# silverlight6/Ultrasound_Modeling

Measured on AMD Instinct MI355X. Metric: segmentation training images/sec at 256x256, higher is better.
Workload: dtype bf16

## Files before the change

### include/usseg.h

```cpp
#ifndef USSEG_H
#define USSEG_H

#include <stddef.h>
#include <stdint.h>

#ifdef __cplusplus
extern "C" {
#endif

typedef void* usseg_stream_t;

typedef enum UssegStatus {
  USSEG_OK = 0,
  USSEG_ERR_BAD_ARG = -1,
  USSEG_ERR_UNSUPPORTED = -2,
  USSEG_ERR_LAUNCH = -3
} UssegStatus;

typedef enum UssegAct { USSEG_ACT_NONE = 0, USSEG_ACT_LRELU = 1, USSEG_ACT_RELU = 2, USSEG_ACT_ELU = 3, USSEG_ACT_GELU = 4 } UssegAct;

enum {
  USSEG_OUT_F32 = 1,
  USSEG_ACCUMULATE = 2
};

typedef struct UssegConvDesc {
  int32_t B, H, W;
  int32_t Cin, Cout;
  int32_t ldx, ldy;
  int32_t ksize;
  int32_t dilation;
  int32_t act;
  float alpha;
  int32_t flags;
} UssegConvDesc;

const char* usseg_last_error(void);
int usseg_version(void);

int usseg_conv2d_fwd(const UssegConvDesc* d, const void* x, const void* wp_fwd, const float* bias,
                     const void* residual, int32_t ldr, void* y, usseg_stream_t stream);
int usseg_conv2d_fwd_affine(const UssegConvDesc* d, const void* x, const void* wp_fwd, const float* scale, const float* shift,
                            const void* residual, int32_t ldr, void* y, usseg_stream_t stream);
typedef struct UssegBnFoldJob {
  const float *gamma, *beta, *mean, *var;
  const float* bias;
  float *scale, *shift;
  int32_t C, Cp;
  float eps;
  int32_t reserved;
} UssegBnFoldJob;
int usseg_bn_fold_batched(const UssegBnFoldJob* jobs_dev, int32_t njobs, usseg_stream_t stream);
int usseg_conv2d_dgrad(const UssegConvDesc* d, const void* dy, const void* wp_dgrad, const void* residual,
                       int32_t ldr, void* dx, usseg_stream_t stream);
int usseg_conv2d_wgrad(const UssegConvDesc* d, const void* x, const void* dy, float* dw_scratch, float* ws,
                       int64_t ws_floats, usseg_stream_t stream);

int usseg_conv2d_dgrad_branches(const UssegConvDesc* d, int32_t nbranches, const int32_t* ksize, const int32_t* dilation,
                                const int32_t* ch_off, int32_t Cb, const void* dy, const void* wp_cat, const void* residual,
                                int32_t ldr, void* dx, usseg_stream_t stream);

typedef struct UssegWgradBlock {
  float* dst;
  int64_t sT, sI, sO;
  int32_t i_off, o_off, ni, no;
} UssegWgradBlock;
typedef struct UssegWgradDst {
  int32_t nblocks;
  int32_t reserved;
  UssegWgradBlock blk[4];
} UssegWgradDst;
int usseg_conv2d_wgrad_mapped(const UssegConvDesc* d, const void* x, const void* dy, const UssegWgradDst* dst, float* ws,
                              int64_t ws_floats, usseg_stream_t stream);
int usseg_tconv2d_wgrad_mapped(const UssegConvDesc* d, const void* x, const void* dy, const UssegWgradDst* dst, float* ws,
                               int64_t ws_floats, usseg_stream_t stream);

typedef struct UssegWgradJob {
  UssegConvDesc desc;
  const void* x;
  const void* dy;
  float* dw;
  const UssegWgradDst* dst;
} UssegWgradJob;
int usseg_conv2d_wgrad_multi(int32_t njobs, const UssegWgradJob* jobs, float* ws, int64_t ws_floats, usseg_stream_t stream);

int usseg_defer_begin(usseg_stream_t stream, float* reduce_ws, int64_t reduce_floats, float* wgrad_ws, int64_t wgrad_floats);
int usseg_defer_flush(usseg_stream_t stream);
int usseg_defer_end(usseg_stream_t stream);

typedef struct UssegConvJob {
  UssegConvDesc desc;
  const void* x;
  const void* wp;
  const float* bias;
  const void* residual;
  int32_t ldr;
  int32_t reserved;
  void* y;
  const float* scale;
} UssegConvJob;
int usseg_conv2d_fwd_multi(int32_t njobs, const UssegConvJob* jobs, usseg_stream_t stream);
int usseg_conv2d_dgrad_multi(int32_t njobs, const UssegConvJob* jobs, usseg_stream_t stream);

int usseg_tconv2d_fwd(const UssegConvDesc* d, const void* x, const void* wp_fwd, const float* bias, void* y,
                      usseg_stream_t stream);
int usseg_tconv2d_dgrad(const UssegConvDesc* d, const void* dy, const void* wp_dgrad, const void* residual,
                        int32_t ldr, void* dx, usseg_stream_t stream);
int usseg_tconv2d_wgrad(const UssegConvDesc* d, const void* x, const void* dy, float* dw_scratch,
                        usseg_stream_t stream);

int usseg_pack_weight(const float* src, int64_t sT, int64_t sN, int64_t sK, int32_t T, int32_t Nn, int32_t Kk,
                      void* dst, int32_t Kw, int32_t tap_stride, int32_t n_off, int32_t k_off,
                      usseg_stream_t stream);
typedef struct UssegPackJob {
  const float* src;
  void* dst;
  int64_t sT, sN, sK;
  int32_t T, Nn, Kk, Kw, tap_stride, n_off, k_off, reserved;
  const float* nscale;
} UssegPackJob;
int usseg_pack_weights_batched(const UssegPackJob* jobs_dev, int32_t njobs, usseg_stream_t stream);
int usseg_pack_weights_flat(const UssegPackJob* jobs_dev, const int32_t* tilemap_dev, int32_t nblocks, usseg_stream_t stream);
int usseg_unpack_wgrad(const float* scratch, int32_t Mrows, int32_t Ncols, int32_t T, int32_t Nn, int32_t Kk,
                       int32_t n_off, int32_t k_off, float* dst, int64_t sT, int64_t sN, int64_t sK,
                       float scale, int32_t accumulate, usseg_stream_t stream);
typedef struct UssegUnpackJob {
  const float* scratch;
  float* dst;
  int64_t sT, sN, sK;
  int32_t Mrows, Ncols, T, Nn, Kk, n_off, k_off, accumulate;
  float scale;
  int32_t reserved;
} UssegUnpackJob;
int usseg_unpack_wgrad_batched(const UssegUnpackJob* jobs_dev, int32_t njobs, int32_t max_elems, usseg_stream_t stream);

typedef struct UssegNormDesc {
  int64_t M;
  int32_t C, Cphys;
  int32_t ldx, ldy;
  int32_t G;
  int32_t mode;
  float eps;
  int32_t act;
  float alpha;
  int32_t lddx;
} UssegNormDesc;
int usseg_norm_act_fwd(const UssegNormDesc* d, const void* x, const float* gamma, const float* beta,
                       const float* mean, const float* var, const void* mask, int32_t ldm, void* y, usseg_stream_t stream);
int usseg_dropout_mask(void* mask, int64_t M, int32_t C, int32_t ld, uint64_t seed, float rate, usseg_stream_t stream);
int usseg_dropout_mask_step(void* mask, int64_t M, int32_t C, int32_t ld, uint64_t seed, const int32_t* step_dev, float rate,
                            usseg_stream_t stream);
int usseg_counter_add(int32_t* counter, int32_t inc, usseg_stream_t stream);
int usseg_norm_act_bwd(const UssegNormDesc* d, const void* x, const void* dy, const float* gamma, const float* beta,
                       const float* mean, const float* var, const void* mask, int32_t ldm, void* dx, float* dgamma,
                       float* dbeta, float* dbias, float* ws, usseg_stream_t stream);
int usseg_norm_act_bwd_res(const UssegNormDesc* d, const void* x, const void* dy, const float* gamma, const float* beta,
                           const void* dres, int32_t lddres, void* dx, float* dgamma, float* dbeta, float* dbias, float* ws,
                           usseg_stream_t stream);
int usseg_norm_act_fwd_gap(const UssegNormDesc* d, const void* x, const float* gamma, const float* beta, const float* mean,
                           const float* var, void* y, int32_t B, int32_t nb, float* gap_rows, usseg_stream_t stream);
int usseg_norm_act_bwd_sa(const UssegNormDesc* d, const void* x, const void* dout, const float* gamma, const float* beta,
                          const float* mean, const float* var, int32_t B, const float* sa_s, const float* sa_dg, float sa_mult,
                          void* dx, float* dgamma, float* dbeta, float* dbias, float* ws, usseg_stream_t stream);
int usseg_norm_act_bwd_pair(const UssegNormDesc* da, const void* xa, const void* dya, const float* gamma_a, const float* beta_a, void* dxa,
                            float* dgamma_a, float* dbeta_a, float* dbias_a, const UssegNormDesc* db, const void* xb, const void* doutb,
                            const float* gamma_b, const float* beta_b, int32_t B, const float* sa_s, const float* sa_dg, float sa_mult, void* dxb,
                            float* dgamma_b, float* dbeta_b, float* dbias_b, float* ws, usseg_stream_t stream);
int usseg_stem_fwd(int32_t B, int32_t H, int32_t W, const void* x, int32_t ldx, const void* w1, const float* b1, const void* w2, const float* b2,
                   const void* w3, const float* b3, const float* gamma, const float* beta, const float* mean, const float* var, float eps,
                   float alpha, void* y1, void* t1, void* c2, void* pooled, usseg_stream_t stream);
int usseg_stem_fwd_infer(int32_t B, int32_t H, int32_t W, const void* x, int32_t ldx, const void* w1, const float* b1, const void* w2,
                         const float* b2, const void* w3, const float* b3, const float* gamma, const float* beta, const float* mean,
                         const float* var, float eps, float alpha, void* pooled, usseg_stream_t stream);
int usseg_conv3_dgrad_actbwd(int32_t B, int32_t H, int32_t W, const void* dy, int32_t lddy, const void* wd, int32_t Co, const void* yact, int32_t ldy,
                             int32_t mode, const float* gamma, const float* beta, const float* var, float eps, float alpha, void* dx,
                             int32_t lddx, float* dgamma, float* dbeta, float* dbias, float* ws, usseg_stream_t stream);
typedef struct UssegCardinalDesc {
  int32_t B, H, W;
  int32_t Cin;
  int32_t P, cv11, cvkk;
  int32_t Up, Vp, Oc;
  int32_t ldx, ldu, ldv, ldsc;
  float eps, alpha;
} UssegCardinalDesc;
int32_t usseg_cardinal_supported(const UssegCardinalDesc* d);
int usseg_cardinal_fwd(const UssegCardinalDesc* d, const void* x, const void* w1, const float* b1, const float* g1, const float* be1,
                       const void* w2, const float* b2, const float* g2, const float* be2, const void* wsc, const float* bsc,
                       const float* gsc, const float* besc, void* u_raw, void* u, void* v_raw, void* y, float* gap_rows, void* sc_raw,
                       void* sc, usseg_stream_t stream);
int usseg_cardinal_fwd_infer(const UssegCardinalDesc* d, const void* x, const void* w1, const float* b1, const float* g1, const float* be1,
                             const void* w2, const float* b2, const float* g2, const float* be2, const void* wsc, const float* bsc,
                             const float* gsc, const float* besc, void* y, float* gap_rows, void* sc, usseg_stream_t stream);
int usseg_cardinal_bwd(const UssegCardinalDesc* d, const void* dout, int32_t ldo, const void* dsc, int32_t lddsc, const void* v_raw,
                       const void* u_raw, const void* sc_raw, const void* w2d, const float* g2, const float* be2, const float* g1,
                       const float* be1, const float* gsc, const float* besc, const float* sa_s, const float* sa_dg, float sa_mult, void* dv,
                       void* dcat, int32_t ldc, float* dg2, float* dbe2, float* db2, float* dg1, float* dbe1, float* db1, float* dgsc,
                       float* dbesc, float* dbsc, float* ws, usseg_stream_t stream);
int usseg_bn_act_pool_fwd(const void* x, int32_t B, int32_t H, int32_t W, int32_t C, int32_t Cphys, int32_t ldx, const float* gamma,
                          const float* beta, const float* mean, const float* var, float eps, int32_t act, float alpha, void* y,
                          int32_t ldy, usseg_stream_t stream);
int usseg_bn_act_pool_bwd(const void* x, const void* dy, int32_t B, int32_t H, int32_t W, int32_t C, int32_t Cphys, int32_t ldx,
                          int32_t lddy, const float* gamma, const float* beta, const float* mean, const float* var, float eps,
                          int32_t act, float alpha, void* dx, int32_t lddx, float* dgamma, float* dbeta, float* dbias, float* ws,
                          usseg_stream_t stream);
int64_t usseg_reduce_ws_floats(void);
int usseg_channel_stats(const void* x, int64_t M, int32_t C, int32_t ldx, float* sum, float* sumsq, float* ws,
                        usseg_stream_t stream);

int usseg_bn_finalize_stats(const float* sum, const float* sumsq, int64_t M, int32_t C, float momentum, float* mean, float* var,
                            float* moving_mean, float* moving_var, usseg_stream_t stream);
int usseg_bn_batch_stats(const void* x, int64_t M, int32_t C, int32_t ldx, float momentum, float* mean, float* var, float* moving_mean,
                         float* moving_var, float* ws, usseg_stream_t stream);
int usseg_bn_train_bwd_fix(const void* x, void* dx, int64_t M, int32_t C, int32_t Cphys, int32_t ldx, int32_t lddx, const float* gamma,
                           const float* mean, const float* var, float eps, const float* tg, const float* tb, usseg_stream_t stream);

int usseg_act_fwd(const void* x, int64_t M, int32_t C, int32_t ldx, int32_t ldy, int32_t act, float alpha, void* y,
                  usseg_stream_t stream);
int usseg_act_bwd(const void* x, const void* dy, int64_t M, int32_t C, int32_t ldx, int32_t lddy, int32_t lddx,
                  int32_t act, float alpha, void* dx, usseg_stream_t stream);
int usseg_act_bwd_colsum(const void* x, const void* dy, int64_t M, int32_t C, int32_t ldx, int32_t lddy, int32_t lddx, int32_t act,
                         float alpha, void* dx, float* db, float* ws, usseg_stream_t stream);

int usseg_avgpool2_fwd(const void* x, int32_t B, int32_t H, int32_t W, int32_t C, int32_t ldx, int32_t ldy, void* y,
                       usseg_stream_t stream);
int usseg_avgpool2_bwd(const void* dy, int32_t B, int32_t H, int32_t W, int32_t C, int32_t lddy, int32_t lddx,
                       const void* add, int32_t ldadd, void* dx, usseg_stream_t stream);
int usseg_avgpool2_bwd_colsum(const void* dy, int32_t B, int32_t H, int32_t W, int32_t C, int32_t lddy, int32_t lddx, const void* add,
                              int32_t ldadd, void* dx, float* db, float* ws, usseg_stream_t stream);

int usseg_copy_channels(const void* src, int64_t M, int32_t C, int32_t lds, void* dst, int32_t ldd, int32_t accumulate,
                        usseg_stream_t stream);
int usseg_cast_input(const void* src, int32_t src_is_f64, int64_t M, int32_t C, void* dst, int32_t Cphys,
                     usseg_stream_t stream);
int usseg_cast_bf16_to_f32(const void* src, int64_t M, int32_t C, int32_t lds, float* dst, usseg_stream_t stream);

typedef struct UssegSplitAttnDesc {
  int32_t B, HW;
  int32_t P, R, Cg, Hd;
  int32_t ldy, ldo;
  int32_t Cy_phys, Co_phys;
  float mult;
  int32_t norm_mode;
  float eps;
  int32_t act;
  float alpha;
  int32_t use_sigmoid;
} UssegSplitAttnDesc;
typedef struct UssegSplitAttnParams {
  const float *w1, *b1, *gamma, *beta, *mean, *var, *w2, *b2;
} UssegSplitAttnParams;
typedef struct UssegSplitAttnGrads {
  float *w1, *b1, *gamma, *beta, *w2, *b2;
} UssegSplitAttnGrads;
int usseg_splitattn_gap(const UssegSplitAttnDesc* d, const void* y, float* g, float* ws, usseg_stream_t stream);
int64_t usseg_splitattn_ws_floats(const UssegSplitAttnDesc* d);
int usseg_splitattn_mlp_fwd(const UssegSplitAttnDesc* d, const float* g, int32_t g_rows, int32_t g_stride,
                            const UssegSplitAttnParams* p, float* s, float* ws, usseg_stream_t stream);
int usseg_splitattn_apply_fwd(const UssegSplitAttnDesc* d, const void* y, const float* s, void* out,
                              usseg_stream_t stream);
int usseg_splitattn_apply_bwd_reduce(const UssegSplitAttnDesc* d, const void* y, const void* dout, int32_t lddo,
                                     float* ds, float* ws, usseg_stream_t stream);
int64_t usseg_splitattn_mlp_bwd_ws_floats(const UssegSplitAttnDesc* d);
int usseg_splitattn_mlp_bwd(const UssegSplitAttnDesc* d, const float* g, int32_t g_rows, int32_t g_stride,
                            const UssegSplitAttnParams* p, const float* s, const float* ws, const float* ds, float* dg,
                            const UssegSplitAttnGrads* grads, float* grad_ws, usseg_stream_t stream);
int usseg_splitattn_bwd_fused(const UssegSplitAttnDesc* d, const void* y, const void* dout, int32_t lddo, const float* g, int32_t g_rows,
                              int32_t g_stride, const UssegSplitAttnParams* p, const float* s, const float* ws, float* dg,
                              const UssegSplitAttnGrads* grads, float* reduce_ws, float* grad_ws, usseg_stream_t stream);
int usseg_splitattn_apply_bwd_dy(const UssegSplitAttnDesc* d, const void* dout, int32_t lddo, const float* s,
                                 const float* dg, void* dy, int32_t lddy, usseg_stream_t stream);

typedef struct UssegLossDesc {
  int64_t M;
  int32_t HW;
  int32_t C, ldl, lddl;
  int32_t loss_kind;
  float label_smoothing;
  float clip_eps;
  float inv_global_batch;
  int32_t quad_w;
} UssegLossDesc;
#define USSEG_ACC_FLOATS 2050
int usseg_softmax_loss_fwd_bwd(const UssegLossDesc* d, const float* logits, const float* y_true, const float* scale,
                               float* probs, float* loss, void* dlogits, usseg_stream_t stream);
int usseg_head_quad_softmax_loss(const void* x, int32_t B, int32_t h, int32_t w, int32_t Cin_phys, int32_t ldx, const void* wq, const float* bias, int32_t C,
                                 const float* y_true, float* probs, float* loss, void* dlogits, float label_smoothing, float clip_eps,
                                 float inv_global_batch, usseg_stream_t stream);
int usseg_accuracy(const float* probs, const float* y_true, int64_t M, int32_t C, float* acc, usseg_stream_t stream);
typedef struct UssegSegCountDesc {
  int32_t B, H, W, C;
  int32_t num_classes;
  int32_t round;
} UssegSegCountDesc;
#define USSEG_SEG_COUNTS 23
int usseg_seg_counts(const UssegSegCountDesc* d, const float* y_true, const float* y_pred, uint64_t* counts, usseg_stream_t stream);
int usseg_cascade_gate(const float* probs, int32_t C_mask, int64_t M, const void* x, int32_t ldx, void* x_gated, uint8_t* mask,
                       usseg_stream_t stream);
int usseg_cascade_maps(const float* probs, int32_t C, int64_t M, float* prob_map, float* bleed_prob, usseg_stream_t stream);
int usseg_loss_from_probs(const UssegLossDesc* d, const float* probs, const float* y_true, const float* scale, float* loss,
                          usseg_stream_t stream);
typedef struct UssegClassLoss {
  float w[8];
  float gamma;
  float factor;
} UssegClassLoss;
int usseg_softmax_loss_fwd_bwd_cl(const UssegLossDesc* d, const UssegClassLoss* cl, const float* logits, const float* y_true, float* probs,
                                  float* loss, void* dlogits, usseg_stream_t stream);
int usseg_head_quad_softmax_loss_cl(const void* x, int32_t B, int32_t h, int32_t w, int32_t Cin_phys, int32_t ldx, const void* wq, const float* bias,
                                    int32_t C, const float* y_true, float* probs, float* loss, void* dlogits, float label_smoothing, float clip_eps,
                                    float inv_global_batch, const UssegClassLoss* cl, usseg_stream_t stream);
int usseg_loss_from_probs_cl(const UssegLossDesc* d, const UssegClassLoss* cl, const float* probs, const float* y_true, float* loss,
                             int32_t as_map, usseg_stream_t stream);
typedef struct UssegOverlapLoss {
  float w[8];
  float alpha;
  float beta;
  float smooth;
  float power;
  float ov_weight;
  float ce_weight;
} UssegOverlapLoss;
#define USSEG_OVERLAP_ACC_FLOATS 8224
int usseg_overlap_loss_grid(int64_t M);
int usseg_overlap_loss_sums(const UssegLossDesc* d, const UssegOverlapLoss* ol, float ov_scale, const float* probs, const float* y_true,
                            float* acc, int64_t acc_floats, usseg_stream_t stream);
int usseg_overlap_loss_bwd(const UssegLossDesc* d, const UssegOverlapLoss* ol, const float* probs, const float* y_true, const float* acc,
                           int64_t acc_floats, void* dlogits, usseg_stream_t stream);
int64_t usseg_sdf_ws_bytes(int32_t B, int32_t H, int32_t W, int32_t C);
int usseg_sdf_labels(const float* y_true, int32_t B, int32_t H, int32_t W, int32_t C, float thr, float* phi, void* ws, int64_t ws_bytes,
                     usseg_stream_t stream);
int64_t usseg_surface_ws_bytes(int32_t N, int32_t H, int32_t W);
int usseg_surface_dist(const uint8_t* a, const uint8_t* b, int32_t N, int32_t H, int32_t W, int64_t* counters, double* sums, void* ws,
                       int64_t ws_bytes, usseg_stream_t stream);
int64_t usseg_surface_stats_ws_bytes(int32_t N, int32_t H, int32_t W);
int usseg_surface_stats(const uint8_t* a, const uint8_t* b, int32_t N, int32_t H, int32_t W, const double* quant, int32_t P, const int32_t* tol2,
                        int32_t T, int64_t* counters, double* sums, int32_t* sel, int64_t* within, void* ws, int64_t ws_bytes,
                        usseg_stream_t stream);
int64_t usseg_components_ws_bytes(int32_t N, int32_t H, int32_t W);
int usseg_label_components(const uint8_t* mask, int32_t N, int32_t H, int32_t W, int32_t connectivity, int32_t* labels, int32_t* count, void* ws,
                           int64_t ws_bytes, usseg_stream_t stream);
int usseg_component_stats(const int32_t* labels, const float* prob, int32_t N, int32_t H, int32_t W, int32_t cap, int64_t* stats,
                          usseg_stream_t stream);
int usseg_clean_mask(const uint8_t* mask, const float* prob, int32_t N, int32_t H, int32_t W, int32_t connectivity, int32_t min_area,
                     float min_peak, uint8_t* out, void* ws, int64_t ws_bytes, usseg_stream_t stream);
int usseg_component_overlap(const int32_t* labels_a, const int32_t* labels_b, int32_t N, int32_t H, int32_t W, int32_t cap_a, int32_t cap_b,
                            int32_t* hit_a, int32_t* hit_b, usseg_stream_t stream);
typedef struct UssegBoundaryLoss {
  float u[8];
} UssegBoundaryLoss;
int usseg_overlap_boundary_loss_sums(const UssegLossDesc* d, const UssegOverlapLoss* ol, float ov_scale, const float* probs, const float* y_true,
                                     const float* phi, const UssegBoundaryLoss* bl, const float* wb, float* acc, int64_t acc_floats,
                                     usseg_stream_t stream);
int usseg_overlap_boundary_loss_bwd(const UssegLossDesc* d, const UssegOverlapLoss* ol, const float* probs, const float* y_true, const float* phi,
                                    const UssegBoundaryLoss* bl, const float* acc, int64_t acc_floats, void* dlogits, usseg_stream_t stream);
#define USSEG_SORT_TILE 2048
#define USSEG_SORT_DIGIT_BITS 8
int64_t usseg_sort_ws_bytes(int32_t S, int64_t n);
int usseg_sort_pairs_u32(const uint32_t* keys_in, const uint32_t* vals_in, int32_t S, int64_t n, int32_t key_bits, uint32_t* keys_out,
                         uint32_t* vals_out, void* ws, int64_t ws_bytes, usseg_stream_t stream);
typedef struct UssegLovaszLoss {
  float w[8];
  float lv_weight;
  float ce_weight;
  float threshold;
  int32_t all_classes;
} UssegLovaszLoss;
int64_t usseg_lovasz_ws_bytes(int64_t M, int32_t C);
int usseg_lovasz_coeffs(const UssegLossDesc* d, UssegLovaszLoss ll, const float* probs, const float* y_true, float* g, int32_t* counts, void* ws,
                        int64_t ws_bytes, usseg_stream_t stream);
int usseg_lovasz_loss_sums(const UssegLossDesc* d, UssegLovaszLoss ll, float ov_scale, const float* probs, const float* y_true, const float* g,
                           const int32_t* counts, float* acc, int64_t acc_floats, usseg_stream_t stream);
int usseg_lovasz_loss_bwd(const UssegLossDesc* d, UssegLovaszLoss ll, const float* probs, const float* y_true, const float* g, const float* acc,
                          int64_t acc_floats, void* dlogits, usseg_stream_t stream);
int usseg_quad_bias_expand(const float* bias, int32_t C, int32_t Np, float* out , usseg_stream_t stream);
int usseg_quad_bias_fold(const float* d16 , int32_t C, float* dbias, usseg_stream_t stream);
int usseg_tconv_quad_unpack(const float* dq, int32_t Cin_phys, int32_t Cin, int32_t Cout, int32_t Np, int32_t ksize, float* grad,
                            usseg_stream_t stream);
int usseg_quad_head_fold(const float* dq, int32_t Cin_phys, int32_t Cin, int32_t Cout, int32_t Np, int32_t ksize, float* grad, const float* d16,
                         float* dbias, usseg_stream_t stream);
int usseg_space_to_depth2(const void* full, int32_t B, int32_t H, int32_t W, int32_t C, int32_t ld_full, void* quad, int32_t Np,
                          int32_t ld_quad, int32_t to_quad, usseg_stream_t stream);
int usseg_tconv_quad_fwd(const UssegConvDesc* d, int32_t ksize, int32_t Np, const void* x, const void* wq_f, const float* bias_q, void* y4,
                         usseg_stream_t stream);
int usseg_tconv_quad_dgrad(const UssegConvDesc* d, int32_t ksize, int32_t Np, const void* dy4, const void* wq_d, void* dx, usseg_stream_t stream);
int usseg_tconv_quad_wgrad(const UssegConvDesc* d, int32_t ksize, int32_t Np, const void* x, const void* dy4, float* dq, float* ws,
                           int64_t ws_floats, usseg_stream_t stream);

int usseg_loss_cat_scale(const float* y_true, int32_t B, int32_t HW, int32_t C, float* scale, usseg_stream_t stream);

int usseg_label2vec(const float* label, int64_t M, int32_t num_classes, float* out, usseg_stream_t stream);
typedef struct UssegAugSample {
  int32_t do_reduc, nclip;
  int32_t clip[2][4];
  int32_t do_shift, shift_r, shift_c, shift_dir;
  int32_t do_noise, do_flip;
  uint64_t seed;
} UssegAugSample;
typedef struct UssegAugDesc {
  int32_t B, H, W, C;
  int32_t Cphys;
  int32_t num_classes;
} UssegAugDesc;
int usseg_augment(const UssegAugDesc* d, const UssegAugSample* samples_dev, const void* x, int32_t x_is_f64, const float* y,
                  const float* noise, void* x_out_bf16, float* x_out_f32, float* y_out, float* y_vec, usseg_stream_t stream);

int usseg_reinject_hidden(void* hidden, int64_t numel, int32_t n, void* const* bufs, const int32_t* c0, const int32_t* ld,
                          int32_t backward, usseg_stream_t stream);

int usseg_patchify(const void* x, int32_t x_is_f64, int32_t B, int32_t H, int32_t W, int32_t C, int32_t patch, void* out, int32_t Cp,
                   usseg_stream_t stream);
int usseg_patch_merge(void* full, int32_t B, int32_t H, int32_t W, int32_t C, int32_t ldf, void* merged, int32_t ldm, int32_t backward,
                      usseg_stream_t stream);
int usseg_ln_wide_fwd(const void* x, int64_t M, int32_t C, int32_t ldx, const float* gamma, const float* beta, float eps, void* y,
                      int32_t ldy, usseg_stream_t stream);
int usseg_ln_wide_bwd(const void* x, const void* dy, int64_t M, int32_t C, int32_t ldx, int32_t lddy, const float* gamma, float eps,
                      void* dx, int32_t lddx, float* dgamma, float* dbeta, float* ws, int64_t ws_floats, usseg_stream_t stream);
int usseg_window_attn_fwd(const void* qkv, int32_t ldq, const float* table, int32_t B, int32_t H, int32_t W, int32_t C, int32_t heads,
                          int32_t ws, int32_t shift, void* out, int32_t ldo, usseg_stream_t stream);
int64_t usseg_window_attn_bwd_ws_floats(int32_t B, int32_t H, int32_t W, int32_t heads, int32_t ws);
int usseg_window_attn_bwd(const void* qkv, int32_t ldq, const void* dout, int32_t ldo, const float* table, int32_t B, int32_t H, int32_t W,
                          int32_t C, int32_t heads, int32_t ws, int32_t shift, void* dqkv, float* dtable, float* ws_rows,
                          usseg_stream_t stream);
int usseg_token_mean_fwd(const void* x, int32_t B, int32_t L, int32_t C, int32_t ld, float* out, usseg_stream_t stream);
int usseg_token_mean_bwd(const float* dy, int32_t B, int32_t L, int32_t C, int32_t ld, void* dx, usseg_stream_t stream);

int usseg_colsum(const void* dy, int64_t M, int32_t C, int32_t ld, float* db, float* ws, usseg_stream_t stream);

int usseg_sumsq(const float* g, int64_t n, float* out, usseg_stream_t stream);
int usseg_sum_f32(const float* x, int64_t n, float* out, usseg_stream_t stream);
int usseg_sumsq_advance(const float* g, int64_t n, float* out, int32_t* step, float* lr_t_dev, float lr, float beta1, float beta2,
                        usseg_stream_t stream);
int usseg_adam_clip_step(float* p, const float* g, float* m, float* v, int64_t n, const float* sumsq, float clip_norm,
                         const float* lr_t_dev, float beta1, float beta2, float eps, usseg_stream_t stream);
int usseg_adam_advance(int32_t* step, float* lr_t_dev, float lr, float beta1, float beta2, usseg_stream_t stream);
int usseg_fill_f32(float* p, int64_t n, float value, usseg_stream_t stream);
int usseg_scale_f32(float* p, int64_t n, const float* sumsq, float clip_norm, usseg_stream_t stream);

#define USSEG_SCHED_MAX_PIECES 16
typedef struct UssegLrSchedule {
  int32_t n;
  int32_t boundary[USSEG_SCHED_MAX_PIECES - 1];
  float lr[USSEG_SCHED_MAX_PIECES];
  float wd[USSEG_SCHED_MAX_PIECES];
} UssegLrSchedule;
int usseg_sched_advance(int32_t* step, const UssegLrSchedule* sched_dev, float* lr_t_dev, float* wd_t_dev, float beta1, float beta2,
                        usseg_stream_t stream);
int usseg_sumsq_sched_advance(const float* g, int64_t n, float* out, int32_t* step, const UssegLrSchedule* sched_dev, float* lr_t_dev,
                              float* wd_t_dev, float beta1, float beta2, usseg_stream_t stream);
int usseg_adamw_step(float* p, const float* g, float* m, float* v, int64_t n, const float* sumsq, float clip_norm, const float* lr_t_dev,
                     const float* wd_t_dev, const uint8_t* decay_mask, float beta1, float beta2, float eps, usseg_stream_t stream);

typedef struct UssegGemmDesc {
  int32_t M, N, K;
  int32_t ldx, ldw, ldy;
  int32_t nb1, nb2;
  int64_t xs1, xs2, ws1, ws2, ys1, ys2;
  int32_t flags;
} UssegGemmDesc;
int usseg_gemm_nt_batched(const UssegGemmDesc* d, const void* x, const void* w, void* y, usseg_stream_t stream);
int usseg_gemm_tn_batched(const UssegGemmDesc* d, const void* a, const void* b, float* out, usseg_stream_t stream);
int usseg_softmax_rows_fwd(const float* s, int64_t rows, int32_t n, float scale, float* p32, void* pbf, usseg_stream_t stream);
int usseg_softmax_rows_bwd(const float* p32, const float* dp, int64_t rows, int32_t n, float scale, void* ds_bf, usseg_stream_t stream);
int usseg_transpose_batched(const void* src, int32_t R, int32_t C, int32_t lds, int32_t nb1, int32_t nb2, int64_t ss1, int64_t ss2,
                            void* dst, usseg_stream_t stream);
int usseg_cast_f32_to_bf16_batched(const float* src, int32_t R, int32_t C, int32_t nb1, int32_t nb2, void* dst, int32_t ldd, int64_t ds1,
                                   int64_t ds2, usseg_stream_t stream);

typedef struct UssegFlashDesc {
  int32_t B, N, H, head_dim;
  int32_t ld_qkv, ld_o;
  float scale;
} UssegFlashDesc;
int usseg_flash_attn_fwd(const UssegFlashDesc* d, const void* q, const void* k, const void* v, void* o, float* o32, float* lse,
                         usseg_stream_t stream);
int usseg_flash_attn_bwd(const UssegFlashDesc* d, const void* q, const void* k, const void* v, const void* o, const float* o32,
                         const void* d_o, const float* lse, float* delta, void* dq, void* dk, void* dv, usseg_stream_t stream);

int usseg_prof_enable(int32_t kind_mask, int32_t capacity);
int usseg_prof_read(int32_t kind, double* total_ms, int64_t* launches);
// ... 47 lines not shown
```

### ultrasound_modeling_amd/ResNest.py

```python
from __future__ import annotations

import contextlib
from typing import List

import torch
import torch.nn as nn

from . import knobs
from . import ops
from .layers import (KERAS_LN_EPS, KERAS_LRELU_ALPHA, AveragePooling2D, BatchNormalization, Conv2D, LayerNormalization,
                     LeakyReLU, _Workspace)
from .ops import ACT_LRELU, ACT_NONE, BF16, roundup


_STAGE_LAZY_ENV = knobs.get("USSEG_ENC_LAZY")
_STAGE_LAZY = _STAGE_LAZY_ENV if _STAGE_LAZY_ENV is not None else 12
_FOLD_BN = knobs.get("USSEG_FOLD_BN")
_FUSED_CARDINAL = knobs.get("USSEG_FUSED_CARDINAL")
_FUSED_CARDINAL_BWD = knobs.get("USSEG_FUSED_CARDINAL_BWD")
_CARD_BWD_MAX_PX = knobs.get("USSEG_CARD_BWD_MAX_PX")
_LN_PAIR = knobs.get("USSEG_LN_PAIR")
_FUSED_STEM_BWD = knobs.get("USSEG_FUSED_STEM_BWD")
_STEM_WGRAD_MERGE = knobs.get("USSEG_STEM_WGRAD_MERGE")
_FUSED_STEM = knobs.get("USSEG_FUSED_STEM")
_MERGED_DGRAD = knobs.get("USSEG_MERGED_DGRAD")


def _span(t: torch.Tensor, n: int) -> torch.Tensor:
    return torch.as_strided(t, (n,), (1,))


def _make_norm(kind: str, channels: int):
    assert kind in ("ln", "bn")
    return LayerNormalization(channels) if kind == "ln" else BatchNormalization(channels)


class split_attention(nn.Module):

    def __init__(self, inchannel, radix, atrous=1, wDecay=None, norm="ln"):
        super().__init__()
        self.inchannel, self.radix, self.atrous, self.wDecay = inchannel, radix, atrous, wDecay
        self.dense1 = Conv2D(inchannel, inchannel // 2, 1)
        self.dense1_bn = _make_norm(norm, inchannel // 2)
        self.dense1_act = LeakyReLU()
        self.dense2 = Conv2D(inchannel // 2, inchannel, 1)
        for c in (self.dense1, self.dense2):
            c.on_finalize = lambda device: None

    def forward(self, inputs: List[torch.Tensor]):
        R = len(inputs)
        B, H, W, Cp, _ = ops.geom(inputs[0])
        Cg = self.inchannel
        dev = inputs[0].device
        ycat = ops.new_act(B, H, W, roundup(R * Cg, 8), dev, zero=True)
        stack = torch.cat([ops.to_f32(t, Cg) for t in inputs], dim=3)
        ycat[..., :R * Cg] = stack.to(BF16)
        out = ops.new_act(B, H, W, roundup(Cg, 8), dev)
        bn = isinstance(self.dense1_bn, BatchNormalization)
        d = ops.splitattn_desc(B, H * W, 1, R, Cg, Cg // 2, ycat.shape[3], out.shape[3], ycat.shape[3], out.shape[3], 1.0, 1 if bn else 0,
                               KERAS_LN_EPS, ACT_LRELU, KERAS_LRELU_ALPHA, R == 1)
        w2 = self.dense2.kernel.data.reshape(1, Cg // 2, Cg).repeat(R, 1, 1).contiguous()
        b2 = self.dense2.bias.data.repeat(R).contiguous()
        stats = (self.dense1_bn.moving_mean_p, self.dense1_bn.moving_variance_p) if bn else (None, None)
        params = (self.dense1.kernel.data, self.dense1.bias.data, self.dense1_bn.gamma.data, self.dense1_bn.beta.data) + stats + (w2, b2)
        ops.splitattn_fwd(d, ycat, params, out)
        return out

    def __call__(self, inputs, *args, **kwargs):
        return self.forward(inputs)


class cardinal(nn.Module):

    def __init__(self, ksize, outchannel, radix, kpaths, atrous=1, wDecay=None, in_channels=None, norm="ln"):
        super().__init__()
        self.outchannel, self.ksize, self.radix, self.kpaths, self.atrous, self.wDecay = outchannel, ksize, radix, kpaths, atrous, wDecay
        self.in_channels = in_channels if in_channels is not None else outchannel
        self.cv11 = int(outchannel / radix / kpaths)
        self.cvkk = int(outchannel / kpaths)
        self.conv1 = Conv2D(self.in_channels, self.cv11, 1, atrous)
        self.conv1_bn = _make_norm(norm, self.cv11)
        self.conv1_act = LeakyReLU()
        self.conv2 = Conv2D(self.cv11, self.cvkk, ksize, atrous)
        self.conv2_bn = _make_norm(norm, self.cvkk)
        self.conv2_act = LeakyReLU()
        self.split = split_attention(self.cvkk, radix, atrous, wDecay, norm=norm)
        for c in (self.conv1, self.conv2):
            c.on_finalize = lambda device: None
        self._solo = None

    def forward(self, x):
        if self._solo is None:
            self._solo = _CardinalGroup([self], self.radix)
            self._solo.on_finalize(x.device)
        return self._solo.forward(x)

    def backward(self, dy, dx_residual=None):
        return self._solo.backward(dy, dx_residual)

    def __call__(self, x, *args, **kwargs):
        return self.forward(x)


class _CardinalGroup:

    def __init__(self, cards: List[cardinal], radix: int):
        self.cards, self.P, self.radix = cards, len(cards), radix
        c0 = cards[0]
        self.cin, self.cv11, self.cvkk, self.k, self.dil = c0.in_channels, c0.cv11, c0.cvkk, c0.ksize, c0.atrous
        self.hid = self.cvkk // 2
        self.U, self.V = self.P * self.cv11, self.P * self.cvkk
        self.Up, self.Vp = roundup(self.U, 8), roundup(self.V, 8)
        self.cin_p = roundup(self.cin, 8)
        self.bn = isinstance(c0.conv1_bn, BatchNormalization)
        self.nmode, self.ngroups = (1, 1) if self.bn else (0, self.P)
        self.st1 = self.st2 = self.sta = (None, None)

    def adjacent_params(self):
        cs = self.cards
        groups = [[c.conv1.bias for c in cs], [c.conv1_bn.gamma for c in cs], [c.conv1_bn.beta for c in cs],
                  [c.conv2.bias for c in cs], [c.conv2_bn.gamma for c in cs], [c.conv2_bn.beta for c in cs],
                  [c.split.dense1.kernel for c in cs], [c.split.dense1.bias for c in cs],
                  [c.split.dense1_bn.gamma for c in cs], [c.split.dense1_bn.beta for c in cs],
                  [c.split.dense2.kernel for c in cs], [c.split.dense2.bias for c in cs]]
        return [(g, 0) for g in groups]

    def on_finalize(self, device):
        T = self.k * self.k
        self.w1_f = torch.zeros((roundup(self.Up, 16), self.cin_p), dtype=BF16, device=device)
        self.w1_d = torch.zeros((roundup(self.cin_p, 16), self.Up), dtype=BF16, device=device)
        self.w2_f = torch.zeros((roundup(self.Vp, 16), T * self.Up), dtype=BF16, device=device)
        self.w2_d = torch.zeros((roundup(self.Up, 16), T * self.Vp), dtype=BF16, device=device)
        c0 = self.cards[0]
        sp = lambda p, n: (_span(p.data, n), _span(p.grad, n))
        self.b1, self.db1 = sp(c0.conv1.bias, self.Up)
        self.g1, self.dg1 = sp(c0.conv1_bn.gamma, self.U)
        self.be1, self.dbe1 = sp(c0.conv1_bn.beta, self.U)
        self.b2, self.db2 = sp(c0.conv2.bias, self.Vp)
        self.g2, self.dg2 = sp(c0.conv2_bn.gamma, self.V)
        self.be2, self.dbe2 = sp(c0.conv2_bn.beta, self.V)
        s = c0.split
        names = (s.dense1.kernel, s.dense1.bias, s.dense1_bn.gamma, s.dense1_bn.beta, s.dense2.kernel, s.dense2.bias)
        self.mlp_p = tuple(p.data for p in names)
        self.mlp_g = tuple(p.grad for p in names)
        if self.bn:
            self.st1 = self._share_stats([c.conv1_bn for c in self.cards], self.Up, device)
            self.st2 = self._share_stats([c.conv2_bn for c in self.cards], self.Vp, device)
            self.sta = self._share_stats([c.split.dense1_bn for c in self.cards], roundup(self.P * self.hid, 8), device)
        for a, b in zip(self.cards[:-1], self.cards[1:]):
            assert b.conv1.bias.data_ptr() == a.conv1.bias.data_ptr() + 4 * self.cv11, "cardinal params are not adjacent"
            assert b.split.dense2.kernel.data_ptr() == a.split.dense2.kernel.data_ptr() + 4 * self.hid * self.cvkk
        self.repack()

    @staticmethod
    def _share_stats(bns, width, device):
        mean = torch.zeros(width, dtype=torch.float32, device=device)
        var = torch.ones(width, dtype=torch.float32, device=device)
        o = 0
        for bn in bns:
            mean[o:o + bn.C] = bn.moving_mean.to(device)
            var[o:o + bn.C] = bn.moving_variance.to(device)
            bn._buffers["moving_mean_p"], bn._buffers["moving_variance_p"] = mean[o:o + bn.C], var[o:o + bn.C]
            o += bn.C
        return mean, var

    def pack_jobs(self):
        T = self.k * self.k
        jobs = []
        for p, c in enumerate(self.cards):
            k1, k2 = c.conv1.kernel.data, c.conv2.kernel.data
            jobs.append(ops.pack_job(k1, 0, 1, self.cv11, 1, self.cv11, self.cin, self.w1_f, self.cin_p, self.cin_p, p * self.cv11, 0))
            jobs.append(ops.pack_job(k1, 0, self.cv11, 1, 1, self.cin, self.cv11, self.w1_d, self.Up, self.Up, 0, p * self.cv11))
            sT = self.cv11 * self.cvkk
            jobs.append(ops.pack_job(k2, sT, 1, self.cvkk, T, self.cvkk, self.cv11, self.w2_f, T * self.Up, self.Up, p * self.cvkk, p * self.cv11))
            jobs.append(ops.pack_job(k2, sT, self.cvkk, 1, T, self.cv11, self.cvkk, self.w2_d, T * self.Vp, self.Vp, p * self.cv11, p * self.cvkk))
        return jobs

    def repack(self):
        jobs = self.pack_jobs()
        ops.pack_weights_batched(ops.make_pack_table(jobs, self.w1_f.device), len(jobs))

    def _maps(self):
        key = self.cards[0].conv1.kernel.grad.data_ptr()
        if getattr(self, "_wmaps_key", None) != key:
            sT = self.cv11 * self.cvkk
            m1 = ops.wgrad_dst([(c.conv1.kernel.grad, 0, self.cv11, 1, 0, p * self.cv11, self.cin, self.cv11) for p, c in enumerate(self.cards)])
            m2 = ops.wgrad_dst([(c.conv2.kernel.grad, sT, self.cvkk, 1, p * self.cv11, p * self.cvkk, self.cv11, self.cvkk)
                                for p, c in enumerate(self.cards)])
            self._wmaps, self._wmaps_key = (m1, m2), key
        return self._wmaps

    def _sa_desc(self, B, HW):
        use_sigmoid = self.radix == 1
        return ops.splitattn_desc(B, HW, self.P, 1, self.cvkk, self.hid, self.Vp, self.Vp, self.Vp, self.Vp, float(self.radix), self.nmode,
                                  KERAS_LN_EPS, ACT_LRELU, KERAS_LRELU_ALPHA, use_sigmoid)

    def _mlp_params(self):
        return self.mlp_p[:4] + self.sta + self.mlp_p[4:]

    def fused_ok(self, sc_conv) -> bool:
        ok = getattr(self, "_fused_ok", None)
        if ok is None:
            ok = self._fused_ok = (not self.bn and self.k == 3 and self.dil == 1 and sc_conv.k == 1 and sc_conv.cout_p == sc_conv.cout and
                                   ops.cardinal_supported(self.cin_p, self.P, self.cv11, self.cvkk, self.Up, self.Vp, sc_conv.cout))
        return ok and _FUSED_CARDINAL

    def forward_fused(self, x, sc_conv, sc_norm, out=None, stash=True):
        B, H, W, _, _ = ops.geom(x)
        a = KERAS_LRELU_ALPHA
        if not stash:
            y, gap, sc = ops.cardinal_fwd_infer(x, self.w1_f, self.b1, self.g1, self.be1, self.w2_f, self.b2, self.g2, self.be2, sc_conv.wp_f,
                                                sc_conv.bias.data, sc_norm.gamma.data, sc_norm.beta.data, self.P, self.cv11, self.cvkk,
                                                self.Up, self.Vp, sc_conv.cout, KERAS_LN_EPS, a)
            out = out if out is not None else ops.new_act(B, H, W, self.Vp, x.device)
            ops.splitattn_fwd(self._sa_desc(B, H * W), y, self._mlp_params(), out, gap=gap)
            self._saved = None
            sc_conv._x = sc_norm._x = None
            return out, sc
        u_raw, u, v_raw, y, gap, sc_raw, sc = ops.cardinal_fwd(x, self.w1_f, self.b1, self.g1, self.be1, self.w2_f, self.b2, self.g2, self.be2,
                                                               sc_conv.wp_f, sc_conv.bias.data, sc_norm.gamma.data, sc_norm.beta.data,
                                                               self.P, self.cv11, self.cvkk, self.Up, self.Vp, sc_conv.cout, KERAS_LN_EPS, a)
        out = out if out is not None else ops.new_act(B, H, W, self.Vp, x.device)
        _, g, s, ws = ops.splitattn_fwd(self._sa_desc(B, H * W), y, self._mlp_params(), out, gap=gap)
        self._saved = (x, u_raw, u, v_raw, y, g, s, ws)
        sc_conv._x = x
        sc_norm._x, sc_norm._act = sc_raw, (ACT_LRELU, a)
        return out, sc

    def forward(self, x, out=None):
        B, H, W, C, _ = ops.geom(x)
        dev = x.device
        a = KERAS_LRELU_ALPHA
        u_raw = ops.conv2d_fwd(x, self.w1_f, self.b1, 1, 1, ops.new_act(B, H, W, self.Up, dev))
        u = ops.norm_act_fwd(u_raw, self.U, self.g1, self.be1, torch.empty_like(u_raw), self.nmode, self.ngroups, KERAS_LN_EPS, ACT_LRELU, a,
                             *self.st1)
        v_raw = ops.conv2d_fwd(u, self.w2_f, self.b2, self.k, self.dil, ops.new_act(B, H, W, self.Vp, dev))
        y, gap = ops.norm_act_fwd_gap(v_raw, self.V, self.g2, self.be2, torch.empty_like(v_raw), self.nmode, self.ngroups, KERAS_LN_EPS,
                                      ACT_LRELU, a, *self.st2)
        out = out if out is not None else ops.new_act(B, H, W, self.Vp, dev)
        d = self._sa_desc(B, H * W)
        _, g, s, ws = ops.splitattn_fwd(d, y, self._mlp_params(), out, gap=gap)
        self._saved = (x, u_raw, u, v_raw, y, g, s, ws)
        return out

    def backward_fused(self, dout, dsc, sc_conv, sc_norm, dcat):
        x, u_raw, u, v_raw, y, g, s, ws = self._saved
        B, H, W, _, _ = ops.geom(x)
        sa_s, sa_dg = ops.splitattn_bwd(self._sa_desc(B, H * W), y, dout, self._mlp_params(), self.mlp_g, g, s, ws, None)
        dv = torch.empty_like(v_raw)
        grads = (self.dg2, self.dbe2, self.db2, self.dg1, self.dbe1, self.db1, sc_norm.gamma.grad, sc_norm.beta.grad, sc_conv.bias.grad)
        ops.cardinal_bwd(dout, dsc, v_raw, u_raw, sc_norm._x, self.w2_d, self.g2, self.be2, self.g1, self.be1, sc_norm.gamma.data, sc_norm.beta.data,
                         sa_s, sa_dg, float(self.radix), dv, dcat, grads, self.cin_p, self.P, self.cv11, self.cvkk, self.Up, self.Vp, sc_conv.cout,
                         KERAS_LN_EPS, KERAS_LRELU_ALPHA)
        ops.wgrad_later(lambda: ops.conv2d_wgrad_mapped(u, dv, self.k, self.dil, self._maps()[1]), u, dv)

    def backward(self, dout, dx_residual=None, du_raw_out=None, shortcut=None):
        x, u_raw, u, v_raw, y, g, s, ws = self._saved
        B, H, W, _, _ = ops.geom(x)
        dev = x.device
        a = KERAS_LRELU_ALPHA
        T = self.k * self.k
        d = self._sa_desc(B, H * W)
        sa_s, sa_dg = ops.splitattn_bwd(d, y, dout, self._mlp_params(), self.mlp_g, g, s, ws, None)
        dv = torch.empty_like(v_raw)
        paired = False
        if shortcut is not None:
            scn, dsc, dx_sc, dbias_sc = shortcut
            if _LN_PAIR and not self.bn and scn._act == (ACT_LRELU, a):
                paired = ops.norm_act_bwd_pair(scn._x, dsc, scn.C, scn.gamma.data, scn.beta.data, dx_sc, scn.gamma.grad, scn.beta.grad, dbias_sc,
                                               v_raw, dout, self.V, self.ngroups, self.g2, self.be2, dv, self.dg2, self.dbe2, self.db2, sa_s, sa_dg,
                                               float(self.radix), KERAS_LN_EPS, a)
            if not paired:
                scn.backward(dsc, dx=dx_sc, dbias=dbias_sc)
        if not paired:
            ops.norm_act_bwd_sa(v_raw, dout, self.V, self.g2, self.be2, dv, self.dg2, self.dbe2, self.nmode, self.ngroups,
                                KERAS_LN_EPS, ACT_LRELU, a, sa_s, sa_dg, float(self.radix), *self.st2, dbias=self.db2)
        ops.wgrad_later(lambda: ops.conv2d_wgrad_mapped(u, dv, self.k, self.dil, self._maps()[1]), u, dv)
        du = ops.conv2d_dgrad(dv, self.w2_d, self.k, self.dil, torch.empty_like(u))
        du_raw = ops.norm_act_bwd(u_raw, du, self.U, self.g1, self.be1, du_raw_out if du_raw_out is not None else torch.empty_like(u_raw),
                                  self.dg1, self.dbe1, self.nmode, self.ngroups, KERAS_LN_EPS, ACT_LRELU, a, *self.st1, dbias=self.db1)
        if du_raw_out is not None:
            return None
        ops.wgrad_later(lambda: ops.conv2d_wgrad_mapped(x, du_raw, 1, 1, self._maps()[0]), x, du_raw)
        return ops.conv2d_dgrad(du_raw, self.w1_d, 1, 1, ops.new_act(B, H, W, self.cin_p, dev), dx_residual)


class residual_S(nn.Module):

    def __init__(self, ksize, outchannel, radix, kpaths, atrous=1, wDecay=None, in_channels=None, norm="ln"):
        super().__init__()
        self.kpaths, self.atrous, self.ksize, self.outchannel, self.radix, self.wDecay = kpaths, atrous, ksize, outchannel, radix, wDecay
        self.in_channels = in_channels if in_channels is not None else outchannel // 2
        self.cardinal_blocks = nn.ModuleList(
            [cardinal(ksize, outchannel // 2, radix, kpaths, atrous, wDecay, in_channels=self.in_channels, norm=norm) for _ in range(kpaths)])
        cvkk = self.cardinal_blocks[0].cvkk
        self.concats_2 = Conv2D(kpaths * cvkk, outchannel, ksize, atrous)
        self.convtmp_sc = Conv2D(self.in_channels, outchannel, 1, atrous)
        self.convtmp_scbn = _make_norm(norm, outchannel)
        self.convtmp_scact = LeakyReLU()
        self._group = _CardinalGroup(list(self.cardinal_blocks), radix)

    def adjacent_params(self):
        return self._group.adjacent_params()

    def on_finalize(self, device):
        g, sc = self._group, self.convtmp_sc
        self.wcat_d = (torch.zeros((roundup(g.cin_p, 16), g.Up + sc.cout_p), dtype=BF16, device=device)
                       if _MERGED_DGRAD and sc.k == 1 and g.P <= 3 else None)
        g.on_finalize(device)
        self.repack()

    def repack(self):
        jobs = self.pack_jobs()
        ops.pack_weights_batched(ops.make_pack_table(jobs, self._group.w1_f.device), len(jobs))

    def pack_jobs(self):
        g, sc = self._group, self.convtmp_sc
        jobs = g.pack_jobs()
        if self.wcat_d is not None:
            Kc = g.Up + sc.cout_p
            for p, c in enumerate(g.cards):
                jobs.append(ops.pack_job(c.conv1.kernel.data, 0, g.cv11, 1, 1, g.cin, g.cv11, self.wcat_d, Kc, Kc, 0, p * g.cv11))
            sT, sI, sO = sc._strides_tio()
            jobs.append(ops.pack_job(sc.kernel.data, sT, sI, sO, 1, sc.cin, sc.cout, self.wcat_d, Kc, Kc, 0, g.Up))
        return jobs

    def forward(self, x, out=None, stash=True):
        if self._group.fused_ok(self.convtmp_sc):
            concats_1, sc = self._group.forward_fused(x, self.convtmp_sc, self.convtmp_scbn, stash=stash)
            return self.concats_2.forward(concats_1, out=out, residual=sc)
        concats_1 = self._group.forward(x)
        sc_raw = self.convtmp_sc.forward(x)
        sc = self.convtmp_scbn.forward(sc_raw, ACT_LRELU, KERAS_LRELU_ALPHA)
        return self.concats_2.forward(concats_1, out=out, residual=sc)

    def backward(self, dout, need_dx=True, bias_done=False):
        d_c1 = self.concats_2.backward(dout, skip_bias=bias_done)
        if self.wcat_d is not None and need_dx:
            g, sc = self._group, self.convtmp_sc
            x = sc._x
            B, H, W, _, _ = ops.geom(x)
            dcat = ops.new_act(B, H, W, g.Up + sc.cout_p, x.device)
            if _FUSED_CARDINAL_BWD and g.fused_ok(sc) and B * H * W < _CARD_BWD_MAX_PX:
                g.backward_fused(d_c1, dout, sc, self.convtmp_scbn, dcat)
            else:
                g.backward(d_c1, du_raw_out=dcat[..., :g.Up], shortcut=(self.convtmp_scbn, dout, dcat[..., g.Up:], sc.bias.grad))
            ops.wgrad_later(lambda: ops.conv2d_wgrad_mapped(x, dcat, 1, 1, self._wcat_map()), x, dcat)
            return ops.conv2d_dgrad(dcat, self.wcat_d, 1, 1, ops.new_act(B, H, W, g.cin_p, x.device))
        dsc_raw = self.convtmp_scbn.backward(dout, dbias=self.convtmp_sc.bias.grad)
        dx_a = self._group.backward(d_c1)
        return self.convtmp_sc.backward(dsc_raw, need_dx=need_dx, dx_residual=dx_a, skip_bias=True)

    def _wcat_map(self):
        g, sc = self._group, self.convtmp_sc
        key = sc.kernel.grad.data_ptr()
        if getattr(self, "_wcat_key", None) != key:
            blocks = [(c.conv1.kernel.grad, 0, g.cv11, 1, 0, p * g.cv11, g.cin, g.cv11) for p, c in enumerate(g.cards)]
            blocks.append((sc.kernel.grad, 0, sc.cout, 1, 0, g.Up, sc.cin, sc.cout))
            self._wcat_m, self._wcat_key = ops.wgrad_dst(blocks), key
        return self._wcat_m

    def __call__(self, x, *args, **kwargs):
        return self.forward(x)


class ResNest(nn.Module):

    def __init__(self, height, width, channel, ksize, radix=4, kpaths=4, wDecay=None, *, norm="ln", widths=(64, 128, 256, 512)):
        super().__init__()
        self.height, self.width, self.channel = height, width, channel
        self.ksize, self.radix, self.kpaths, self.wDecay = ksize, radix, kpaths, wDecay
        self.conv1 = Conv2D(channel, 16, 3)
        self.conv1_act = LeakyReLU()
        self.convtmp_1 = Conv2D(16, 32, 3)
        self.convtmp_1bn = BatchNormalization(32)
        self.convtmp_1act = LeakyReLU()
        self.convtmp_2 = Conv2D(32, 32, 3)
        self.convtmp_2bn = BatchNormalization(32)
        self.convtmp_2act = LeakyReLU()
        self.conv1_pool = AveragePooling2D()
        self.conv2_pool = AveragePooling2D()
        self.conv3_pool = AveragePooling2D()
        self.conv4_pool = AveragePooling2D()
        w = tuple(widths)
        self.widths = w
        self.conv_1 = residual_S(ksize, w[0], radix, kpaths, wDecay=wDecay, in_channels=32, norm=norm)
        self.conv_2 = residual_S(ksize, w[1], radix, kpaths, wDecay=wDecay, in_channels=w[0], norm=norm)
        self.conv_3 = residual_S(ksize, w[2], radix, kpaths, wDecay=wDecay, in_channels=w[1], norm=norm)
        self.conv_4 = residual_S(ksize, w[3], radix, kpaths, wDecay=wDecay, in_channels=w[2], norm=norm)

    def forward(self, x, outs=None, stash=True):
        o3, o2, o1 = outs if outs is not None else (None, None, None)
        if x.dtype != BF16:
            x = ops.cast_input(x.contiguous(), roundup(self.channel, 8))
        a = KERAS_LRELU_ALPHA
        bn1, bn2 = self.convtmp_1bn, self.convtmp_2bn
        self._fold = self.convtmp_1.fold_scale() is not None
        if (_FUSED_STEM and self._fold and not bn2.training_mode and self.conv1.cin_p == 8 and x.shape[1] % 2 == 0 and x.shape[2] % 2 == 0
                and (self.conv1.cout, self.convtmp_1.cout, self.convtmp_2.cout) == (16, 32, 32)):
            if not stash:
                t = ops.stem_fwd_infer(x, self.conv1.wp_f, self.conv1.bias.data, self.convtmp_1.wp_f, bn1.fold_shift, self.convtmp_2.wp_f,
                                       self.convtmp_2.bias.data, bn2.gamma.data, bn2.beta.data, bn2.moving_mean_p, bn2.moving_variance_p, bn2.eps, a)
                self._y1 = self._t1 = self.conv1._x = self.convtmp_1._x = self.convtmp_2._x = bn2._x = None
                self._pool_fused = self._stem_fused = True
                return self._stages_forward(t, o1, o2, o3, stash=False)
            self._y1, self._t1, c2, t = ops.stem_fwd(x, self.conv1.wp_f, self.conv1.bias.data, self.convtmp_1.wp_f, bn1.fold_shift,
                                                     self.convtmp_2.wp_f, self.convtmp_2.bias.data, bn2.gamma.data, bn2.beta.data,
                                                     bn2.moving_mean_p, bn2.moving_variance_p, bn2.eps, a)
            self.conv1._x, self.convtmp_1._x, self.convtmp_2._x = x, self._y1, self._t1
            bn2._x, bn2._act = c2, (ACT_LRELU, a)
            self._pool_fused = self._stem_fused = True
            return self._stages_forward(t, o1, o2, o3)
        self._stem_fused = False
        self._y1 = self.conv1.forward(x, act=ACT_LRELU, alpha=a)
        self._pool_fused = False
        if self._fold:
            self._t1 = t = self.convtmp_1.forward(self._y1, act=ACT_LRELU, alpha=a, bias=bn1.fold_shift)
        else:
            t = self.convtmp_1.forward(self._y1)
            t = self.convtmp_1bn.forward(t, ACT_LRELU, a)
        t = self.convtmp_2.forward(t)
        self._pool_fused = not bn2.training_mode
        if self._pool_fused:
            t = self.convtmp_2bn.forward_pool(t, ACT_LRELU, a)
        else:
            t = self.conv1_pool.forward(self.convtmp_2bn.forward(t, ACT_LRELU, a))
        return self._stages_forward(t, o1, o2, o3, stash=stash)

    def _stages_forward(self, t, o1, o2, o3, stash=True):
        x_1 = self.conv_1.forward(t, out=o1, stash=stash)
        x_2 = self.conv_2.forward(self.conv2_pool.forward(x_1), out=o2, stash=stash)
        x_3 = self.conv_3.forward(self.conv3_pool.forward(x_2), out=o3, stash=stash)
        x_4 = self.conv_4.forward(self.conv4_pool.forward(x_3), stash=stash)
        return x_4, [x_3, x_2, x_1]

    def backward(self, d_x4, d_feats):
        d_x3, d_x2, d_x1 = d_feats
        mask = getattr(self, "stage_lazy", _STAGE_LAZY)
        lazy = lambda st: ops.lazy_wgrads() if (mask >> (st - 1)) & 1 else contextlib.nullcontext()
        with lazy(4):
            d = self.conv_4.backward(d_x4)
        d = self.conv4_pool.backward(d, add=d_x3, db=self.conv_3.concats_2.bias.grad)
        with lazy(3):
            d = self.conv_3.backward(d, bias_done=True)
        d = self.conv3_pool.backward(d, add=d_x2, db=self.conv_2.concats_2.bias.grad)
        with lazy(2):
            d = self.conv_2.backward(d, bias_done=True)
        d = self.conv2_pool.backward(d, add=d_x1, db=self.conv_1.concats_2.bias.grad)
        with lazy(1):
            d = self.conv_1.backward(d, bias_done=True)
        a = KERAS_LRELU_ALPHA
        if self._pool_fused:
            d = self.convtmp_2bn.backward_pool(d, dbias=self.convtmp_2.bias.grad)
        else:
            d = self.convtmp_2bn.backward(self.conv1_pool.backward(d), dbias=self.convtmp_2.bias.grad)
        bn1, c1, c2 = self.convtmp_1bn, self.convtmp_1, self.convtmp_2
        wjobs = [] if _STEM_WGRAD_MERGE else None
        def wg(conv, dy):
            if wjobs is None:
                conv.backward(dy, need_dx=False, skip_bias=True)
            else:
                wjobs.append(conv.wgrad_job(dy))
        dn = torch.empty_like(self._t1) if (_FUSED_STEM_BWD and self._fold) else None
        if dn is not None and ops.conv3_dgrad_actbwd(d, c2.wp_d, self._t1, dn, 2, a, c1.bias.grad, bn1.gamma.data, bn1.beta.data, bn1.moving_variance_p,
                                                     bn1.eps, bn1.gamma.grad, bn1.beta.grad):
            wg(c2, d)
            d = dn
        else:
            if wjobs is not None:
                wjobs.append(c2.wgrad_job(d))
            d = c2.backward(d, skip_bias=True, skip_wgrad=wjobs is not None)
            if self._fold:
                d = bn1.backward_folded(self._t1, d, ACT_LRELU, a, dbias=c1.bias.grad)
            else:
                d = bn1.backward(d, dbias=c1.bias.grad)
        dn = torch.empty_like(self._y1) if _FUSED_STEM_BWD else None
        if dn is not None and ops.conv3_dgrad_actbwd(d, c1.wp_d, self._y1, dn, 0, KERAS_LRELU_ALPHA, self.conv1.bias.grad):
            wg(c1, d)
            d = dn
        else:
            if wjobs is not None:
                wjobs.append(c1.wgrad_job(d))
            d = c1.backward(d, skip_bias=True, skip_wgrad=wjobs is not None)
            d = ops.act_bwd_colsum(self._y1, d, torch.empty_like(d), ACT_LRELU, KERAS_LRELU_ALPHA, self.conv1.bias.grad, self.conv1.cout)
        wg(self.conv1, d)
        if wjobs:
            keep = [t for job in wjobs for t in job[:2]]
            ops.wgrad_later(lambda: ops.conv2d_wgrad_multi(wjobs), *keep)
        return None

    def bn_fold_jobs(self):
        return [self.convtmp_1bn.fold_job(self.convtmp_1.bias.data), self.convtmp_2bn.fold_job(self.convtmp_2.bias.data)]

    def on_finalize(self, device):
        if getattr(self, "_fold_table", None) is None:
            jobs = self.bn_fold_jobs()
            self._fold_table = (ops.make_bn_fold_table(jobs, device), len(jobs))
        ops.bn_fold_batched(*self._fold_table)
        if _FOLD_BN:
            self.convtmp_1._fold_scale = self.convtmp_1bn.fold_scale
            self.convtmp_1._fold_bns = [self.convtmp_1bn]

    def repack(self):
        for m in self.modules():
            if m is not self and isinstance(m, (Conv2D, residual_S)) and getattr(m, "wp_f", 1) is not None:
                m.repack()
        self.on_finalize(self.conv1.kernel.device)

    def __call__(self, x, *args, **kwargs):
        return self.forward(x)
```

### ultrasound_modeling_amd/_lib.py

```python
from __future__ import annotations

import ctypes as C
import os

import torch
from . import knobs

_HERE = os.path.dirname(os.path.abspath(__file__))
LIB_PATH = knobs.get("USSEG_LIB") or os.path.join(_HERE, "libusseg_hip.so")

c_i32, c_i64, c_f32, c_vp = C.c_int32, C.c_int64, C.c_float, C.c_void_p


class UssegError(RuntimeError):
    pass


class ConvDesc(C.Structure):
    _fields_ = [("B", c_i32), ("H", c_i32), ("W", c_i32), ("Cin", c_i32), ("Cout", c_i32), ("ldx", c_i32),
                ("ldy", c_i32), ("ksize", c_i32), ("dilation", c_i32), ("act", c_i32), ("alpha", c_f32),
                ("flags", c_i32)]


class ConvJob(C.Structure):
    _fields_ = [("desc", ConvDesc), ("x", c_vp), ("wp", c_vp), ("bias", c_vp), ("residual", c_vp), ("ldr", c_i32),
                ("reserved", c_i32), ("y", c_vp), ("scale", c_vp)]


class WgradBlock(C.Structure):
    _fields_ = [("dst", c_vp), ("sT", c_i64), ("sI", c_i64), ("sO", c_i64), ("i_off", c_i32), ("o_off", c_i32), ("ni", c_i32), ("no", c_i32)]


class WgradDst(C.Structure):
    _fields_ = [("nblocks", c_i32), ("reserved", c_i32), ("blk", WgradBlock * 4)]


P_WgradDst = C.POINTER(WgradDst)


class WgradJob(C.Structure):
    _fields_ = [("desc", ConvDesc), ("x", c_vp), ("dy", c_vp), ("dw", c_vp), ("dst", P_WgradDst)]


class AugSample(C.Structure):
    _fields_ = [("do_reduc", c_i32), ("nclip", c_i32), ("clip", (c_i32 * 4) * 2), ("do_shift", c_i32), ("shift_r", c_i32),
                ("shift_c", c_i32), ("shift_dir", c_i32), ("do_noise", c_i32), ("do_flip", c_i32), ("seed", C.c_uint64)]


class AugDesc(C.Structure):
    _fields_ = [("B", c_i32), ("H", c_i32), ("W", c_i32), ("C", c_i32), ("Cphys", c_i32), ("num_classes", c_i32)]


class PrepAugSample(C.Structure):
    _fields_ = [("do_flip", c_i32), ("do_reduc", c_i32), ("do_contrast", c_i32), ("do_clip", c_i32), ("clip", c_i32 * 4), ("do_rotate", c_i32),
                ("rot_slot", c_i32), ("do_shift", c_i32), ("shift_r", c_i32), ("shift_c", c_i32), ("shift_dir", c_i32), ("do_noise", c_i32),
                ("reserved", c_i32), ("seed", C.c_uint64), ("rot", C.c_double * 6)]


class PrepAugDesc(C.Structure):
    _fields_ = [("N", c_i32), ("H", c_i32), ("W", c_i32), ("C", c_i32), ("n_rot", c_i32), ("k_lo", c_i32), ("k_hi", c_i32),
                ("g_lo", C.c_double), ("g_hi", C.c_double), ("zH", C.c_double), ("zW", C.c_double)]


class NormDesc(C.Structure):
    _fields_ = [("M", c_i64), ("C", c_i32), ("Cphys", c_i32), ("ldx", c_i32), ("ldy", c_i32), ("G", c_i32),
                ("mode", c_i32), ("eps", c_f32), ("act", c_i32), ("alpha", c_f32), ("lddx", c_i32)]


class CardinalDesc(C.Structure):
    _fields_ = [("B", c_i32), ("H", c_i32), ("W", c_i32), ("Cin", c_i32), ("P", c_i32), ("cv11", c_i32), ("cvkk", c_i32), ("Up", c_i32),
                ("Vp", c_i32), ("Oc", c_i32), ("ldx", c_i32), ("ldu", c_i32), ("ldv", c_i32), ("ldsc", c_i32), ("eps", c_f32), ("alpha", c_f32)]


class SplitAttnDesc(C.Structure):
    _fields_ = [("B", c_i32), ("HW", c_i32), ("P", c_i32), ("R", c_i32), ("Cg", c_i32), ("Hd", c_i32),
                ("ldy", c_i32), ("ldo", c_i32), ("Cy_phys", c_i32), ("Co_phys", c_i32), ("mult", c_f32),
                ("norm_mode", c_i32), ("eps", c_f32), ("act", c_i32), ("alpha", c_f32), ("use_sigmoid", c_i32)]


class SplitAttnParams(C.Structure):
    _fields_ = [(n, c_vp) for n in ("w1", "b1", "gamma", "beta", "mean", "var", "w2", "b2")]


class SplitAttnGrads(C.Structure):
    _fields_ = [(n, c_vp) for n in ("w1", "b1", "gamma", "beta", "w2", "b2")]


class GemmDesc(C.Structure):
    _fields_ = [("M", c_i32), ("N", c_i32), ("K", c_i32), ("ldx", c_i32), ("ldw", c_i32), ("ldy", c_i32), ("nb1", c_i32), ("nb2", c_i32),
                ("xs1", c_i64), ("xs2", c_i64), ("ws1", c_i64), ("ws2", c_i64), ("ys1", c_i64), ("ys2", c_i64), ("flags", c_i32)]


class ClassLoss(C.Structure):
    _fields_ = [("w", c_f32 * 8), ("gamma", c_f32), ("factor", c_f32)]


class OverlapLoss(C.Structure):
    _fields_ = [("w", c_f32 * 8), ("alpha", c_f32), ("beta", c_f32), ("smooth", c_f32), ("power", c_f32), ("ov_weight", c_f32),
                ("ce_weight", c_f32)]


class LovaszLoss(C.Structure):
    _fields_ = [("w", c_f32 * 8), ("lv_weight", c_f32), ("ce_weight", c_f32), ("threshold", c_f32), ("all_classes", c_i32)]


class BoundaryLoss(C.Structure):
    _fields_ = [("u", c_f32 * 8)]


class FlashDesc(C.Structure):
    _fields_ = [("B", c_i32), ("N", c_i32), ("H", c_i32), ("head_dim", c_i32), ("ld_qkv", c_i32), ("ld_o", c_i32), ("scale", c_f32)]


class LossDesc(C.Structure):
    _fields_ = [("M", c_i64), ("HW", c_i32), ("C", c_i32), ("ldl", c_i32), ("lddl", c_i32), ("loss_kind", c_i32),
                ("label_smoothing", c_f32), ("clip_eps", c_f32), ("inv_global_batch", c_f32), ("quad_w", c_i32)]


class SegCountDesc(C.Structure):
    _fields_ = [("B", c_i32), ("H", c_i32), ("W", c_i32), ("C", c_i32), ("num_classes", c_i32), ("round", c_i32)]


SEG_COUNTS = 23

ACT_NONE, ACT_LRELU, ACT_RELU, ACT_ELU, ACT_GELU = 0, 1, 2, 3, 4
OUT_F32, ACCUMULATE = 1, 2

P = C.POINTER
_PROTOS = {
    "usseg_last_error": (C.c_char_p, []),
    "usseg_version": (C.c_int, []),
    "usseg_conv2d_fwd": (C.c_int, [P(ConvDesc), c_vp, c_vp, c_vp, c_vp, c_i32, c_vp, c_vp]),
    "usseg_conv2d_fwd_affine": (C.c_int, [P(ConvDesc), c_vp, c_vp, c_vp, c_vp, c_vp, c_i32, c_vp, c_vp]),
    "usseg_bn_fold_batched": (C.c_int, [c_vp, c_i32, c_vp]),
    "usseg_conv2d_dgrad": (C.c_int, [P(ConvDesc), c_vp, c_vp, c_vp, c_i32, c_vp, c_vp]),
    "usseg_conv2d_wgrad": (C.c_int, [P(ConvDesc), c_vp, c_vp, c_vp, c_vp, c_i64, c_vp]),
    "usseg_conv2d_wgrad_mapped": (C.c_int, [P(ConvDesc), c_vp, c_vp, P(WgradDst), c_vp, c_i64, c_vp]),
    "usseg_tconv2d_wgrad_mapped": (C.c_int, [P(ConvDesc), c_vp, c_vp, P(WgradDst), c_vp, c_i64, c_vp]),
    "usseg_conv2d_dgrad_branches": (C.c_int, [P(ConvDesc), c_i32, c_vp, c_vp, c_vp, c_i32, c_vp, c_vp, c_vp, c_i32, c_vp, c_vp]),
    "usseg_conv2d_wgrad_multi": (C.c_int, [c_i32, c_vp, c_vp, c_i64, c_vp]),
    "usseg_conv2d_fwd_multi": (C.c_int, [c_i32, c_vp, c_vp]),
    "usseg_conv2d_dgrad_multi": (C.c_int, [c_i32, c_vp, c_vp]),
    "usseg_tconv2d_fwd": (C.c_int, [P(ConvDesc), c_vp, c_vp, c_vp, c_vp, c_vp]),
    "usseg_tconv2d_dgrad": (C.c_int, [P(ConvDesc), c_vp, c_vp, c_vp, c_i32, c_vp, c_vp]),
    "usseg_tconv2d_wgrad": (C.c_int, [P(ConvDesc), c_vp, c_vp, c_vp, c_vp]),
    "usseg_pack_weight": (C.c_int, [c_vp, c_i64, c_i64, c_i64, c_i32, c_i32, c_i32, c_vp, c_i32, c_i32, c_i32, c_i32, c_vp]),
    "usseg_pack_weights_batched": (C.c_int, [c_vp, c_i32, c_vp]),
    "usseg_pack_weights_flat": (C.c_int, [c_vp, c_vp, c_i32, c_vp]),
    "usseg_unpack_wgrad": (C.c_int, [c_vp, c_i32, c_i32, c_i32, c_i32, c_i32, c_i32, c_i32, c_vp, c_i64, c_i64, c_i64,
                                     c_f32, c_i32, c_vp]),
    "usseg_unpack_wgrad_batched": (C.c_int, [c_vp, c_i32, c_i32, c_vp]),
    "usseg_norm_act_fwd": (C.c_int, [P(NormDesc), c_vp, c_vp, c_vp, c_vp, c_vp, c_vp, c_i32, c_vp, c_vp]),
    "usseg_dropout_mask": (C.c_int, [c_vp, c_i64, c_i32, c_i32, C.c_uint64, c_f32, c_vp]),
    "usseg_dropout_mask_step": (C.c_int, [c_vp, c_i64, c_i32, c_i32, C.c_uint64, c_vp, c_f32, c_vp]),
    "usseg_counter_add": (C.c_int, [c_vp, c_i32, c_vp]),
    "usseg_norm_act_bwd": (C.c_int, [P(NormDesc), c_vp, c_vp, c_vp, c_vp, c_vp, c_vp, c_vp, c_i32, c_vp, c_vp, c_vp, c_vp, c_vp, c_vp]),
    "usseg_bn_act_pool_fwd": (C.c_int, [c_vp, c_i32, c_i32, c_i32, c_i32, c_i32, c_i32, c_vp, c_vp, c_vp, c_vp, c_f32, c_i32, c_f32, c_vp, c_i32, c_vp]),
    "usseg_bn_act_pool_bwd": (C.c_int, [c_vp, c_vp, c_i32, c_i32, c_i32, c_i32, c_i32, c_i32, c_i32, c_vp, c_vp, c_vp, c_vp, c_f32, c_i32, c_f32,
                                        c_vp, c_i32, c_vp, c_vp, c_vp, c_vp, c_vp]),
    "usseg_reduce_ws_floats": (c_i64, []),
    "usseg_channel_stats": (C.c_int, [c_vp, c_i64, c_i32, c_i32, c_vp, c_vp, c_vp, c_vp]),
    "usseg_bn_finalize_stats": (C.c_int, [c_vp, c_vp, c_i64, c_i32, c_f32, c_vp, c_vp, c_vp, c_vp, c_vp]),
    "usseg_bn_batch_stats": (C.c_int, [c_vp, c_i64, c_i32, c_i32, c_f32, c_vp, c_vp, c_vp, c_vp, c_vp, c_vp]),
    "usseg_bn_train_bwd_fix": (C.c_int, [c_vp, c_vp, c_i64, c_i32, c_i32, c_i32, c_i32, c_vp, c_vp, c_vp, c_f32, c_vp, c_vp, c_vp]),
    "usseg_act_fwd": (C.c_int, [c_vp, c_i64, c_i32, c_i32, c_i32, c_i32, c_f32, c_vp, c_vp]),
    "usseg_act_bwd": (C.c_int, [c_vp, c_vp, c_i64, c_i32, c_i32, c_i32, c_i32, c_i32, c_f32, c_vp, c_vp]),
    "usseg_act_bwd_colsum": (C.c_int, [c_vp, c_vp, c_i64, c_i32, c_i32, c_i32, c_i32, c_i32, c_f32, c_vp, c_vp, c_vp, c_vp]),
    "usseg_avgpool2_fwd": (C.c_int, [c_vp, c_i32, c_i32, c_i32, c_i32, c_i32, c_i32, c_vp, c_vp]),
    "usseg_avgpool2_bwd": (C.c_int, [c_vp, c_i32, c_i32, c_i32, c_i32, c_i32, c_i32, c_vp, c_i32, c_vp, c_vp]),
    "usseg_avgpool2_bwd_colsum": (C.c_int, [c_vp, c_i32, c_i32, c_i32, c_i32, c_i32, c_i32, c_vp, c_i32, c_vp, c_vp, c_vp, c_vp]),
    "usseg_copy_channels": (C.c_int, [c_vp, c_i64, c_i32, c_i32, c_vp, c_i32, c_i32, c_vp]),
    "usseg_cast_input": (C.c_int, [c_vp, c_i32, c_i64, c_i32, c_vp, c_i32, c_vp]),
    "usseg_cast_bf16_to_f32": (C.c_int, [c_vp, c_i64, c_i32, c_i32, c_vp, c_vp]),
    "usseg_splitattn_gap": (C.c_int, [P(SplitAttnDesc), c_vp, c_vp, c_vp, c_vp]),
    "usseg_splitattn_ws_floats": (c_i64, [P(SplitAttnDesc)]),
    "usseg_splitattn_mlp_fwd": (C.c_int, [P(SplitAttnDesc), c_vp, c_i32, c_i32, P(SplitAttnParams), c_vp, c_vp, c_vp]),
    "usseg_norm_act_fwd_gap": (C.c_int, [P(NormDesc), c_vp, c_vp, c_vp, c_vp, c_vp, c_vp, c_i32, c_i32, c_vp, c_vp]),
    "usseg_stem_fwd": (C.c_int, [c_i32, c_i32, c_i32, c_vp, c_i32, c_vp, c_vp, c_vp, c_vp, c_vp, c_vp, c_vp, c_vp, c_vp, c_vp, c_f32, c_f32,
                                 c_vp, c_vp, c_vp, c_vp, c_vp]),
    "usseg_stem_fwd_infer": (C.c_int, [c_i32, c_i32, c_i32, c_vp, c_i32, c_vp, c_vp, c_vp, c_vp, c_vp, c_vp, c_vp, c_vp, c_vp, c_vp, c_f32, c_f32,
                                       c_vp, c_vp]),
    "usseg_conv3_dgrad_actbwd": (C.c_int, [c_i32, c_i32, c_i32, c_vp, c_i32, c_vp, c_i32, c_vp, c_i32, c_i32, c_vp, c_vp, c_vp, c_f32, c_f32, c_vp, c_i32,
                                           c_vp, c_vp, c_vp, c_vp, c_vp]),
    "usseg_cardinal_supported": (c_i32, [P(CardinalDesc)]),
    "usseg_cardinal_fwd": (C.c_int, [P(CardinalDesc)] + [c_vp] * 21),
    "usseg_cardinal_fwd_infer": (C.c_int, [P(CardinalDesc)] + [c_vp] * 17),
    "usseg_cardinal_bwd": (C.c_int, [P(CardinalDesc), c_vp, c_i32, c_vp, c_i32] + [c_vp] * 12 + [c_f32, c_vp, c_vp, c_i32] + [c_vp] * 11),
    "usseg_accuracy": (C.c_int, [c_vp, c_vp, c_i64, c_i32, c_vp, c_vp]),
    "usseg_seg_counts": (C.c_int, [P(SegCountDesc), c_vp, c_vp, c_vp, c_vp]),
    "usseg_cascade_gate": (C.c_int, [c_vp, c_i32, c_i64, c_vp, c_i32, c_vp, c_vp, c_vp]),
    "usseg_cascade_maps": (C.c_int, [c_vp, c_i32, c_i64, c_vp, c_vp, c_vp]),
    "usseg_norm_act_bwd_res": (C.c_int, [P(NormDesc), c_vp, c_vp, c_vp, c_vp, c_vp, c_i32, c_vp, c_vp, c_vp, c_vp, c_vp, c_vp]),
    "usseg_norm_act_bwd_sa": (C.c_int, [P(NormDesc), c_vp, c_vp, c_vp, c_vp, c_vp, c_vp, c_i32, c_vp, c_vp, c_f32, c_vp, c_vp, c_vp, c_vp, c_vp, c_vp]),
    "usseg_norm_act_bwd_pair": (C.c_int, [P(NormDesc)] + [c_vp] * 8 + [P(NormDesc)] + [c_vp] * 4 + [c_i32, c_vp, c_vp, c_f32] + [c_vp] * 6),
    "usseg_splitattn_apply_fwd": (C.c_int, [P(SplitAttnDesc), c_vp, c_vp, c_vp, c_vp]),
    "usseg_splitattn_apply_bwd_reduce": (C.c_int, [P(SplitAttnDesc), c_vp, c_vp, c_i32, c_vp, c_vp, c_vp]),
    "usseg_splitattn_mlp_bwd_ws_floats": (c_i64, [P(SplitAttnDesc)]),
    "usseg_splitattn_bwd_fused": (C.c_int, [P(SplitAttnDesc), c_vp, c_vp, c_i32, c_vp, c_i32, c_i32, P(SplitAttnParams), c_vp, c_vp, c_vp,
                                            P(SplitAttnGrads), c_vp, c_vp, c_vp]),
    "usseg_splitattn_mlp_bwd": (C.c_int, [P(SplitAttnDesc), c_vp, c_i32, c_i32, P(SplitAttnParams), c_vp, c_vp, c_vp, c_vp,
                                          P(SplitAttnGrads), c_vp, c_vp]),
    "usseg_splitattn_apply_bwd_dy": (C.c_int, [P(SplitAttnDesc), c_vp, c_i32, c_vp, c_vp, c_vp, c_i32, c_vp]),
    "usseg_softmax_loss_fwd_bwd": (C.c_int, [P(LossDesc), c_vp, c_vp, c_vp, c_vp, c_vp, c_vp, c_vp]),
    "usseg_head_quad_softmax_loss": (C.c_int, [c_vp, c_i32, c_i32, c_i32, c_i32, c_i32, c_vp, c_vp, c_i32, c_vp, c_vp, c_vp, c_vp, c_f32, c_f32, c_f32, c_vp]),
    "usseg_loss_from_probs": (C.c_int, [P(LossDesc), c_vp, c_vp, c_vp, c_vp, c_vp]),
    "usseg_softmax_loss_fwd_bwd_cl": (C.c_int, [P(LossDesc), P(ClassLoss), c_vp, c_vp, c_vp, c_vp, c_vp, c_vp]),
    "usseg_head_quad_softmax_loss_cl": (C.c_int, [c_vp, c_i32, c_i32, c_i32, c_i32, c_i32, c_vp, c_vp, c_i32, c_vp, c_vp, c_vp, c_vp, c_f32, c_f32, c_f32,
                                                  P(ClassLoss), c_vp]),
    "usseg_loss_from_probs_cl": (C.c_int, [P(LossDesc), P(ClassLoss), c_vp, c_vp, c_vp, c_i32, c_vp]),
    "usseg_overlap_loss_grid": (C.c_int, [c_i64]),
    "usseg_overlap_loss_sums": (C.c_int, [P(LossDesc), P(OverlapLoss), c_f32, c_vp, c_vp, c_vp, c_i64, c_vp]),
    "usseg_overlap_loss_bwd": (C.c_int, [P(LossDesc), P(OverlapLoss), c_vp, c_vp, c_vp, c_i64, c_vp, c_vp]),
    "usseg_sdf_ws_bytes": (c_i64, [c_i32, c_i32, c_i32, c_i32]),
    "usseg_sdf_labels": (C.c_int, [c_vp, c_i32, c_i32, c_i32, c_i32, c_f32, c_vp, c_vp, c_i64, c_vp]),
    "usseg_surface_ws_bytes": (c_i64, [c_i32, c_i32, c_i32]),
    "usseg_surface_dist": (C.c_int, [c_vp, c_vp, c_i32, c_i32, c_i32, c_vp, c_vp, c_vp, c_i64, c_vp]),
    "usseg_surface_stats_ws_bytes": (c_i64, [c_i32, c_i32, c_i32]),
    "usseg_surface_stats": (C.c_int, [c_vp, c_vp, c_i32, c_i32, c_i32, c_vp, c_i32, c_vp, c_i32, c_vp, c_vp, c_vp, c_vp, c_vp, c_i64, c_vp]),
    "usseg_components_ws_bytes": (c_i64, [c_i32, c_i32, c_i32]),
    "usseg_label_components": (C.c_int, [c_vp, c_i32, c_i32, c_i32, c_i32, c_vp, c_vp, c_vp, c_i64, c_vp]),
    "usseg_component_stats": (C.c_int, [c_vp, c_vp, c_i32, c_i32, c_i32, c_i32, c_vp, c_vp]),
    "usseg_clean_mask": (C.c_int, [c_vp, c_vp, c_i32, c_i32, c_i32, c_i32, c_i32, c_f32, c_vp, c_vp, c_i64, c_vp]),
    "usseg_component_overlap": (C.c_int, [c_vp, c_vp, c_i32, c_i32, c_i32, c_i32, c_i32, c_vp, c_vp, c_vp]),
    "usseg_overlap_boundary_loss_sums": (C.c_int, [P(LossDesc), P(OverlapLoss), c_f32, c_vp, c_vp, c_vp, P(BoundaryLoss), c_vp, c_vp, c_i64, c_vp]),
    "usseg_overlap_boundary_loss_bwd": (C.c_int, [P(LossDesc), P(OverlapLoss), c_vp, c_vp, c_vp, P(BoundaryLoss), c_vp, c_i64, c_vp, c_vp]),
    "usseg_sort_ws_bytes": (c_i64, [c_i32, c_i64]),
    "usseg_sort_pairs_u32": (C.c_int, [c_vp, c_vp, c_i32, c_i64, c_i32, c_vp, c_vp, c_vp, c_i64, c_vp]),
    "usseg_lovasz_ws_bytes": (c_i64, [c_i64, c_i32]),
    "usseg_lovasz_coeffs": (C.c_int, [P(LossDesc), LovaszLoss, c_vp, c_vp, c_vp, c_vp, c_vp, c_i64, c_vp]),
    "usseg_lovasz_loss_sums": (C.c_int, [P(LossDesc), LovaszLoss, c_f32, c_vp, c_vp, c_vp, c_vp, c_vp, c_i64, c_vp]),
    "usseg_lovasz_loss_bwd": (C.c_int, [P(LossDesc), LovaszLoss, c_vp, c_vp, c_vp, c_vp, c_i64, c_vp, c_vp]),
    "usseg_quad_bias_expand": (C.c_int, [c_vp, c_i32, c_i32, c_vp, c_vp]),
    "usseg_space_to_depth2": (C.c_int, [c_vp, c_i32, c_i32, c_i32, c_i32, c_i32, c_vp, c_i32, c_i32, c_i32, c_vp]),
    "usseg_tconv_quad_fwd": (C.c_int, [P(ConvDesc), c_i32, c_i32, c_vp, c_vp, c_vp, c_vp, c_vp]),
    "usseg_tconv_quad_dgrad": (C.c_int, [P(ConvDesc), c_i32, c_i32, c_vp, c_vp, c_vp, c_vp]),
    "usseg_tconv_quad_wgrad": (C.c_int, [P(ConvDesc), c_i32, c_i32, c_vp, c_vp, c_vp, c_vp, c_i64, c_vp]),
    "usseg_quad_bias_fold": (C.c_int, [c_vp, c_i32, c_vp, c_vp]),
    "usseg_tconv_quad_unpack": (C.c_int, [c_vp, c_i32, c_i32, c_i32, c_i32, c_i32, c_vp, c_vp]),
    "usseg_quad_head_fold": (C.c_int, [c_vp, c_i32, c_i32, c_i32, c_i32, c_i32, c_vp, c_vp, c_vp, c_vp]),
    "usseg_label2vec": (C.c_int, [c_vp, c_i64, c_i32, c_vp, c_vp]),
    "usseg_augment": (C.c_int, [P(AugDesc), c_vp, c_vp, c_i32, c_vp, c_vp, c_vp, c_vp, c_vp, c_vp, c_vp]),
    "usseg_loss_cat_scale": (C.c_int, [c_vp, c_i32, c_i32, c_i32, c_vp, c_vp]),
    "usseg_patchify": (C.c_int, [c_vp, c_i32, c_i32, c_i32, c_i32, c_i32, c_i32, c_vp, c_i32, c_vp]),
    "usseg_patch_merge": (C.c_int, [c_vp, c_i32, c_i32, c_i32, c_i32, c_i32, c_vp, c_i32, c_i32, c_vp]),
    "usseg_ln_wide_fwd": (C.c_int, [c_vp, c_i64, c_i32, c_i32, c_vp, c_vp, c_f32, c_vp, c_i32, c_vp]),
    "usseg_ln_wide_bwd": (C.c_int, [c_vp, c_vp, c_i64, c_i32, c_i32, c_i32, c_vp, c_f32, c_vp, c_i32, c_vp, c_vp, c_vp, c_i64, c_vp]),
    "usseg_window_attn_fwd": (C.c_int, [c_vp, c_i32, c_vp, c_i32, c_i32, c_i32, c_i32, c_i32, c_i32, c_i32, c_vp, c_i32, c_vp]),
    "usseg_window_attn_bwd_ws_floats": (c_i64, [c_i32, c_i32, c_i32, c_i32, c_i32]),
    "usseg_window_attn_bwd": (C.c_int, [c_vp, c_i32, c_vp, c_i32, c_vp, c_i32, c_i32, c_i32, c_i32, c_i32, c_i32, c_i32, c_vp, c_vp, c_vp, c_vp]),
    "usseg_token_mean_fwd": (C.c_int, [c_vp, c_i32, c_i32, c_i32, c_i32, c_vp, c_vp]),
    "usseg_token_mean_bwd": (C.c_int, [c_vp, c_i32, c_i32, c_i32, c_i32, c_vp, c_vp]),
    "usseg_colsum": (C.c_int, [c_vp, c_i64, c_i32, c_i32, c_vp, c_vp, c_vp]),
    "usseg_sumsq": (C.c_int, [c_vp, c_i64, c_vp, c_vp]),
    "usseg_sum_f32": (C.c_int, [c_vp, c_i64, c_vp, c_vp]),
    "usseg_sumsq_advance": (C.c_int, [c_vp, c_i64, c_vp, c_vp, c_vp, c_f32, c_f32, c_f32, c_vp]),
    "usseg_reinject_hidden": (C.c_int, [c_vp, c_i64, c_i32, c_vp, c_vp, c_vp, c_i32, c_vp]),
    "usseg_adam_clip_step": (C.c_int, [c_vp, c_vp, c_vp, c_vp, c_i64, c_vp, c_f32, c_vp, c_f32, c_f32, c_f32, c_vp]),
    "usseg_adam_advance": (C.c_int, [c_vp, c_vp, c_f32, c_f32, c_f32, c_vp]),
    "usseg_fill_f32": (C.c_int, [c_vp, c_i64, c_f32, c_vp]),
    "usseg_scale_f32": (C.c_int, [c_vp, c_i64, c_vp, c_f32, c_vp]),
    "usseg_sched_advance": (C.c_int, [c_vp, c_vp, c_vp, c_vp, c_f32, c_f32, c_vp]),
    "usseg_sumsq_sched_advance": (C.c_int, [c_vp, c_i64, c_vp, c_vp, c_vp, c_vp, c_vp, c_f32, c_f32, c_vp]),
    "usseg_adamw_step": (C.c_int, [c_vp, c_vp, c_vp, c_vp, c_i64, c_vp, c_f32, c_vp, c_vp, c_vp, c_f32, c_f32, c_f32, c_vp]),
    "usseg_gemm_nt_batched": (C.c_int, [P(GemmDesc), c_vp, c_vp, c_vp, c_vp]),
    "usseg_gemm_tn_batched": (C.c_int, [P(GemmDesc), c_vp, c_vp, c_vp, c_vp]),
    "usseg_flash_attn_fwd": (C.c_int, [P(FlashDesc), c_vp, c_vp, c_vp, c_vp, c_vp, c_vp, c_vp]),
    "usseg_flash_attn_bwd": (C.c_int, [P(FlashDesc), c_vp, c_vp, c_vp, c_vp, c_vp, c_vp, c_vp, c_vp, c_vp, c_vp, c_vp, c_vp]),
    "usseg_softmax_rows_fwd": (C.c_int, [c_vp, c_i64, c_i32, c_f32, c_vp, c_vp, c_vp]),
    "usseg_softmax_rows_bwd": (C.c_int, [c_vp, c_vp, c_i64, c_i32, c_f32, c_vp, c_vp]),
    "usseg_transpose_batched": (C.c_int, [c_vp, c_i32, c_i32, c_i32, c_i32, c_i32, c_i64, c_i64, c_vp, c_vp]),
    "usseg_cast_f32_to_bf16_batched": (C.c_int, [c_vp, c_i32, c_i32, c_i32, c_i32, c_vp, c_i32, c_i64, c_i64, c_vp]),
    "usseg_defer_begin": (C.c_int, [c_vp, c_vp, c_i64, c_vp, c_i64]),
    "usseg_defer_flush": (C.c_int, [c_vp]),
    "usseg_defer_end": (C.c_int, [c_vp]),
    "usseg_prof_enable": (C.c_int, [c_i32, c_i32]),
    "usseg_prof_read": (C.c_int, [c_i32, P(C.c_double), P(c_i64)]),
    "usseg_prof_disable": (C.c_int, []),
    "usseg_prep_cycle_stats": (C.c_int, [c_vp, c_i32, c_i32, c_i32, c_vp, c_vp, c_vp]),
    "usseg_prep_label": (C.c_int, [c_vp, c_i32, c_i32, c_vp, c_vp, c_i32, c_i32, c_i32, c_vp, c_vp, c_vp, c_vp]),
    "usseg_prep_label_thick": (C.c_int, [c_vp, c_i32, c_i32, c_vp, c_i32, c_i32, c_i32, c_vp, c_vp, c_vp]),
    "usseg_prep_assemble": (C.c_int, [c_vp, c_vp, c_i32, c_i32, c_i32, c_vp, c_i32, c_i32, c_i32, c_vp, c_vp, c_i32, c_vp, c_vp]),
    "usseg_select_ranks_f64": (C.c_int, [c_vp, c_i32, c_i64, P(c_i32), c_i32, c_vp, c_vp, c_vp]),
    "usseg_prep_aug_ws_doubles": (c_i64, [c_i32, c_i32, c_i32, c_i32, c_i32]),
    "usseg_prep_aug": (C.c_int, [P(PrepAugDesc), c_vp, c_vp, c_vp, c_vp, c_vp, c_i64, c_vp, c_vp, c_vp]),
    "usseg_cone_index": (C.c_int, [c_vp, c_vp, c_i32, c_i32, C.c_double, C.c_double, C.c_double, c_i32, c_i32, c_vp, c_vp]),
    "usseg_cone_range": (C.c_int, [c_vp, c_i32, c_i32, c_vp, c_vp, c_vp]),
    "usseg_cone_render": (C.c_int, [c_vp, c_i32, c_i32, c_i32, c_vp, c_vp, c_vp, c_vp, c_i32, c_i32, c_i32, P(C.c_double), c_vp, c_vp, c_vp,
                                    c_vp]),
}
EXPORTED_SYMBOLS = tuple(_PROTOS)

_lib = None


def load() -> C.CDLL:
    global _lib
    if _lib is not None:
        return _lib
    if not os.path.exists(LIB_PATH):
        raise UssegError(f"{LIB_PATH} not found: build the HIP extension first (python -c 'import __graft_entry__ as g; "
                         f"g.build()'). There is no CPU fallback.")
    lib = C.CDLL(LIB_PATH)
    for name, (res, args) in _PROTOS.items():
        fn = getattr(lib, name)
        fn.restype = res
        fn.argtypes = args
    _lib = lib
    return lib


def check(rc: int, what: str = "") -> None:
    if rc != 0:
        msg = load().usseg_last_error().decode("utf-8", "replace")
        raise UssegError(f"{what}: usseg error {rc}: {msg}")
```

### ultrasound_modeling_amd/csrc/stem.hip

```cpp
#include "common.h"

namespace {

struct StemFwd {
  const bf16_t* x;
  const bf16_t *w1, *w2, *w3;
  const float *b1, *b2, *b3, *gamma, *beta, *mean, *var;
  bf16_t *y1, *t1, *c2, *pooled;
  int32_t B, H, W, ldx, tiles_x, ntiles;
  float alpha, eps;
};

#ifndef STEM_TH
#define STEM_TH 16
#endif
constexpr int T = 16, TH = STEM_TH;
constexpr int XW = T + 6, Y1W = T + 4, T1W = T + 2;
constexpr int XH = TH + 6, Y1H = TH + 4, T1H = TH + 2;
constexpr int XS = 8, Y1S = 16 + 8, T1S = 32 + 8, C2S = 32 + 8;
constexpr int XS_B = XW * XH * XS * 2, Y1_B = Y1W * Y1H * Y1S * 2, T1_B = T1W * T1H * T1S * 2;
constexpr int LDS_B = XS_B + Y1_B + T1_B;
static_assert(T * TH * C2S * 2 <= XS_B + Y1_B, "staging tile must fit the dead x / y1 region");
static_assert(XW * XH <= 512 && (T / 2) * (TH / 2) * 4 <= 256, "thread mappings");

__device__ __forceinline__ bf16x8_t zfrag() {
  bf16x8_t z;
#pragma unroll
  for (int i = 0; i < 8; ++i) z[i] = (__bf16)0.f;
  return z;
}

template <int CPT, int NT>
struct WFrag {
  static constexpr int NCH = 9 * CPT, KS = (NCH + 3) / 4;
  bf16x8_t a[KS][NT];
  __device__ __forceinline__ void load(const bf16_t* w, int r, int q) {
#pragma unroll
    for (int ks = 0; ks < KS; ++ks)
#pragma unroll
      for (int nt = 0; nt < NT; ++nt) {
        const int chunk = 4 * ks + q;
        const bf16x8_t v = *reinterpret_cast<const bf16x8_t*>(w + (int64_t)(nt * 16 + r) * (NCH * 8) + (chunk < NCH ? chunk : 0) * 8);
        a[ks][nt] = chunk < NCH ? v : zfrag();
      }
  }
};

template <int CPT, int NT, int OW, int OH, int SRC_S, int DST_S, bool LRELU, bool ZERO_OUT>
__device__ __forceinline__ void conv_phase(const bf16_t* src, bf16_t* dst, const WFrag<CPT, NT>& wf, const float* bias, float alpha, int gy0, int gx0,
                                           int H, int W, int wv, int r, int q) {
  constexpr int IW = OW + 2, NPIX = OW * OH, MT = (NPIX + 15) / 16, NCH = 9 * CPT, KS = (NCH + 3) / 4;
  float4 bb[NT];
#pragma unroll
  for (int nt = 0; nt < NT; ++nt) bb[nt] = *reinterpret_cast<const float4*>(bias + nt * 16 + 4 * q);
  int toff[KS];
#pragma unroll
  for (int ks = 0; ks < KS; ++ks) {
    const int chunk = 4 * ks + q;
    const int cc = chunk < NCH ? chunk : 0;
    const int tap = cc / CPT, choff = cc - tap * CPT;
    const int dy = tap / 3, dx = tap - dy * 3;
    toff[ks] = (dy * IW + dx) * SRC_S + choff * 8;
  }
  for (int mt = wv; mt < MT; mt += 4) {
    const int pp = mt * 16 + r;
    const int pc = pp < NPIX ? pp : NPIX - 1;
    const int py = pc / OW, px = pc - py * OW;
    const int base = (py * IW + px) * SRC_S;
    f32x4_t acc[NT];
#pragma unroll
    for (int nt = 0; nt < NT; ++nt) acc[nt] = f32x4_t{0.f, 0.f, 0.f, 0.f};
#pragma unroll
    for (int ks = 0; ks < KS; ++ks) {
      const bf16x8_t b = *reinterpret_cast<const bf16x8_t*>(src + base + toff[ks]);
#pragma unroll
      for (int nt = 0; nt < NT; ++nt) acc[nt] = __builtin_amdgcn_mfma_f32_16x16x32_bf16(wf.a[ks][nt], b, acc[nt], 0, 0, 0);
    }
    if (pp < NPIX) {
      const int gy = gy0 + py, gx = gx0 + px;
      const bool in = !ZERO_OUT || (gy >= 0 && gy < H && gx >= 0 && gx < W);
#pragma unroll
      for (int nt = 0; nt < NT; ++nt) {
        float v0 = acc[nt][0] + bb[nt].x, v1 = acc[nt][1] + bb[nt].y, v2 = acc[nt][2] + bb[nt].z, v3 = acc[nt][3] + bb[nt].w;
        if (LRELU) {
          v0 = v0 >= 0.f ? v0 : alpha * v0; v1 = v1 >= 0.f ? v1 : alpha * v1;
          v2 = v2 >= 0.f ? v2 : alpha * v2; v3 = v3 >= 0.f ? v3 : alpha * v3;
        }
        uint2 o;
        o.x = in ? pack2bf(v0, v1) : 0u;
        o.y = in ? pack2bf(v2, v3) : 0u;
        *reinterpret_cast<uint2*>(dst + pp * DST_S + nt * 16 + 4 * q) = o;
      }
    }
  }
}

template <int GW, int OFF, int NCHK, int S>
__device__ __forceinline__ void store_interior(const bf16_t* tile, bf16_t* out, int64_t img, int ld, int ty0, int tx0, int H, int W, int tid) {
  for (int it = tid; it < T * TH * NCHK; it += 256) {
    const int pp = it / NCHK, c = it - pp * NCHK;
    const int iy = pp / T, ix = pp - iy * T;
    const int gy = ty0 + iy, gx = tx0 + ix;
    if (gy < H && gx < W)
      *reinterpret_cast<uint4*>(out + (img + (int64_t)gy * W + gx) * ld + c * 8) =
          *reinterpret_cast<const uint4*>(tile + ((iy + OFF) * GW + ix + OFF) * S + c * 8);
  }
}

__global__ __launch_bounds__(256) void stem_fwd_kernel(const StemFwd p) {
  constexpr bool STASH = true;
#include "stem_fwd_body.inc"
}

__global__ __launch_bounds__(256) void stem_fwd_infer_kernel(const StemFwd p) {
  constexpr bool STASH = false;
#include "stem_fwd_body.inc"
}

struct DgAct {
  const bf16_t *dy, *wd, *yact;
  bf16_t* dx;
  const float *gamma, *beta, *var;
  float* ws;
  int32_t B, H, W, lddy, ldy, lddx, tiles_x, ntiles;
  float eps, alpha;
};
[[maybe_unused]] constexpr int DG_S = 40;

template <int CO, int MODE>
__global__ __launch_bounds__(256, 2) void dgrad_actbwd_kernel(const DgAct p) {
#if defined(__HIP_DEVICE_COMPILE__)
  constexpr int TW = 16, HWD = TW + 2, NT = CO / 16, NIT = (HWD * HWD * 4 + 255) / 256, CL = 4 * NT;
  __shared__ __attribute__((aligned(16))) bf16_t DT[2][HWD * HWD * DG_S];
  __shared__ float RED[4][4][NT * 4 * 3];
  const int tid = threadIdx.x, lane = tid & 63, wv = tid >> 6, r = lane & 15, q = lane >> 4;
  constexpr bool WREG = NT == 1;
  __shared__ __attribute__((aligned(16))) bf16_t WL[WREG ? 8 : 9 * NT * 64 * 8];
  __shared__ __attribute__((aligned(16))) float CST[3][CO];
  auto wrow = [&](int t, int nt) { return p.wd + (int64_t)(CL * (r >> 2) + 4 * nt + (r & 3)) * 288 + (8 - t) * 32 + q * 8; };
  bf16x8_t a[WREG ? 9 : 1][NT];
  if constexpr (WREG) {
#pragma unroll
    for (int t = 0; t < 9; ++t) a[t][0] = *reinterpret_cast<const bf16x8_t*>(wrow(t, 0));
  } else if (wv == 0) {
#pragma unroll
    for (int t = 0; t < 9; ++t)
#pragma unroll
      for (int nt = 0; nt < NT; ++nt) *reinterpret_cast<bf16x8_t*>(WL + ((t * NT + nt) * 64 + lane) * 8) = *reinterpret_cast<const bf16x8_t*>(wrow(t, nt));
  }
  if (MODE == 2 && tid < CO) {
    const float g = p.gamma[tid];
    CST[0][tid] = g * rsqrtf(p.var[tid] + p.eps);
    CST[1][tid] = p.beta[tid];
    CST[2][tid] = fabsf(g) > 1e-20f ? 1.f / g : 0.f;
  }
  const float inv_neg = p.alpha != 0.f ? 1.f / p.alpha : 1.f;
  float sga[NT][4], sbe[NT][4], sbi[NT][4];
#pragma unroll
  for (int nt = 0; nt < NT; ++nt)
#pragma unroll
    for (int j = 0; j < 4; ++j) sga[nt][j] = sbe[nt][j] = sbi[nt][j] = 0.f;
  const int tiles_img = p.tiles_x * ((p.H + TW - 1) / TW);
  uint4 dv[NIT];
  auto load_dy = [&](int t) -> uint32_t {
    const int b = t / tiles_img, tile = t - b * tiles_img;
    const int tyi = tile / p.tiles_x, txi = tile - tyi * p.tiles_x;
    const int64_t img = (int64_t)b * p.H * p.W;
    uint32_t m = 0;
#pragma unroll
    for (int i = 0; i < NIT; ++i) {
      const int it = tid + i * 256;
      const int hp = min(it >> 2, HWD * HWD - 1), c = it & 3;
      const int hy = hp / HWD, hx = hp - hy * HWD;
      const int gy = tyi * TW - 1 + hy, gx = txi * TW - 1 + hx;
      m |= (uint32_t)(gy >= 0 && gy < p.H && gx >= 0 && gx < p.W) << i;
      const int cy = min(max(gy, 0), p.H - 1), cx = min(max(gx, 0), p.W - 1);
      dv[i] = *reinterpret_cast<const uint4*>(p.dy + (img + (int64_t)cy * p.W + cx) * p.lddy + c * 8);
    }
    return m;
  };
  auto stage = [&](int buf, uint32_t m) {
#pragma unroll
    for (int i = 0; i < NIT; ++i) {
      const int it = tid + i * 256;
      const uint4 v = (m >> i) & 1u ? dv[i] : make_uint4(0, 0, 0, 0);
      if (it < HWD * HWD * 4) *reinterpret_cast<uint4*>(DT[buf] + (it >> 2) * DG_S + (it & 3) * 8) = v;
    }
  };
  int t = blockIdx.x, buf = 0;
  if (t < p.ntiles) {
    const uint32_t m = load_dy(t);
    stage(0, m);
  }
  __syncthreads();
  for (; t < p.ntiles; t += gridDim.x) {
    const int b = t / tiles_img, tile = t - b * tiles_img;
    const int tyi = tile / p.tiles_x, txi = tile - tyi * p.tiles_x;
    const int ty0 = tyi * TW, tx0 = txi * TW;
    const int64_t img = (int64_t)b * p.H * p.W;
    uint32_t yv[4][CL / 2];
#pragma unroll
    for (int i = 0; i < 4; ++i) {
      const int gy = min(ty0 + wv + 4 * i, p.H - 1), gx = min(tx0 + r, p.W - 1);
      const bf16_t* yp = p.yact + (img + (int64_t)gy * p.W + gx) * p.ldy + CL * q;
      if constexpr (NT == 2) {
        const uint4 v = *reinterpret_cast<const uint4*>(yp);
        yv[i][0] = v.x; yv[i][1] = v.y; yv[i][CL / 2 - 2] = v.z; yv[i][CL / 2 - 1] = v.w;
      } else {
        const uint2 v = *reinterpret_cast<const uint2*>(yp);
        yv[i][0] = v.x; yv[i][1] = v.y;
      }
    }
    const int tn = t + (int)gridDim.x;
    const uint32_t mnext = load_dy(tn < p.ntiles ? tn : t);
    f32x4_t acc[4][NT];
#pragma unroll
    for (int i = 0; i < 4; ++i)
#pragma unroll
      for (int nt = 0; nt < NT; ++nt) acc[i][nt] = f32x4_t{0.f, 0.f, 0.f, 0.f};
#pragma unroll
    for (int tp = 0; tp < 9; ++tp) {
      const int ty = tp / 3, tx = tp - ty * 3;
      bf16x8_t at[NT];
#pragma unroll
      for (int nt = 0; nt < NT; ++nt) {
        if constexpr (WREG) at[nt] = a[tp][nt];
        else at[nt] = *reinterpret_cast<const bf16x8_t*>(WL + ((tp * NT + nt) * 64 + lane) * 8);
      }
#pragma unroll
      for (int i = 0; i < 4; ++i) {
        const bf16x8_t bx = *reinterpret_cast<const bf16x8_t*>(DT[buf] + ((wv + 4 * i + ty) * HWD + (r + tx)) * DG_S + q * 8);
#pragma unroll
        for (int nt = 0; nt < NT; ++nt) acc[i][nt] = __builtin_amdgcn_mfma_f32_16x16x32_bf16(at[nt], bx, acc[i][nt], 0, 0, 0);
      }
    }
#pragma unroll
    for (int i = 0; i < 4; ++i) {
      const int gy = ty0 + wv + 4 * i, gx = tx0 + r;
      const bool ok = gy < p.H && gx < p.W;
      uint32_t o2[CL / 2];
#pragma unroll
      for (int nt = 0; nt < NT; ++nt) {
        const uint32_t y01 = yv[i][2 * nt], y23 = yv[i][2 * nt + 1];
        const float y[4] = {__uint_as_float(y01 << 16), __uint_as_float(y01 & 0xffff0000u), __uint_as_float(y23 << 16), __uint_as_float(y23 & 0xffff0000u)};
        float o[4];
        float4 gr = make_float4(1.f, 1.f, 1.f, 1.f), be = gr, ig = gr;
        if (MODE == 2) {
          gr = *reinterpret_cast<const float4*>(&CST[0][CL * q + 4 * nt]);
          be = *reinterpret_cast<const float4*>(&CST[1][CL * q + 4 * nt]);
          ig = *reinterpret_cast<const float4*>(&CST[2][CL * q + 4 * nt]);
        }
        const float grj[4] = {gr.x, gr.y, gr.z, gr.w}, bej[4] = {be.x, be.y, be.z, be.w}, igj[4] = {ig.x, ig.y, ig.z, ig.w};
#pragma unroll
        for (int j = 0; j < 4; ++j) {
          const float d = ok ? acc[i][nt][j] : 0.f;
          if (MODE == 2) {
            const float xh = ((y[j] >= 0.f ? y[j] : y[j] * inv_neg) - bej[j]) * igj[j];
            const float dh = d * (y[j] > 0.f ? 1.f : p.alpha);
            sga[nt][j] = fmaf(dh, xh, sga[nt][j]);
            sbe[nt][j] += dh;
            o[j] = dh * grj[j];
            sbi[nt][j] += o[j];
          } else {
            o[j] = d * (y[j] >= 0.f ? 1.f : p.alpha);
          }
        }
        o2[2 * nt] = pack2bf(o[0], o[1]); o2[2 * nt + 1] = pack2bf(o[2], o[3]);
        if (MODE == 0) {
          sbi[nt][0] += __uint_as_float(o2[2 * nt] << 16); sbi[nt][1] += __uint_as_float(o2[2 * nt] & 0xffff0000u);
          sbi[nt][2] += __uint_as_float(o2[2 * nt + 1] << 16); sbi[nt][3] += __uint_as_float(o2[2 * nt + 1] & 0xffff0000u);
        }
      }
      if (ok) {
        bf16_t* xp = p.dx + (img + (int64_t)gy * p.W + gx) * p.lddx + CL * q;
        if constexpr (NT == 2) *reinterpret_cast<uint4*>(xp) = make_uint4(o2[0], o2[1], o2[CL / 2 - 2], o2[CL / 2 - 1]);
        else *reinterpret_cast<uint2*>(xp) = make_uint2(o2[0], o2[1]);
      }
    }
    stage(buf ^ 1, mnext);
    __syncthreads();
    buf ^= 1;
  }
#pragma unroll
  for (int nt = 0; nt < NT; ++nt)
#pragma unroll
    for (int j = 0; j < 4; ++j) {
      float v0 = sga[nt][j], v1 = sbe[nt][j], v2 = sbi[nt][j];
#pragma unroll
      for (int msk = 1; msk < 16; msk <<= 1) {
        v0 += __shfl_xor(v0, msk, 64); v1 += __shfl_xor(v1, msk, 64); v2 += __shfl_xor(v2, msk, 64);
      }
      if (r == 0) { RED[wv][q][(nt * 4 + j) * 3 + 0] = v0; RED[wv][q][(nt * 4 + j) * 3 + 1] = v1; RED[wv][q][(nt * 4 + j) * 3 + 2] = v2; }
    }
  __syncthreads();
  if (tid < CO * 3) {
    const int k = tid / CO, c = tid - k * CO;
    const int qq = c / CL, nt = (c % CL) >> 2, j = c & 3;
    float s = 0.f;
#pragma unroll
    for (int w = 0; w < 4; ++w) s += RED[w][qq][(nt * 4 + j) * 3 + k];
    p.ws[((int64_t)blockIdx.x * 3 + k) * CO + c] = s;
  }
#endif
}

}

extern "C" int usseg_stem_fwd(int32_t B, int32_t H, int32_t W, const void* x, int32_t ldx, const void* w1, const float* b1, const void* w2,
                              const float* b2, const void* w3, const float* b3, const float* gamma, const float* beta, const float* mean,
                              const float* var, float eps, float alpha, void* y1, void* t1, void* c2, void* pooled, usseg_stream_t stream) {
  USSEG_CHECK_ARG(x && w1 && b1 && w2 && b2 && w3 && b3 && gamma && beta && mean && var && y1 && t1 && c2 && pooled, "stem_fwd: null pointer");
  USSEG_CHECK_ARG(B > 0 && H > 0 && W > 0 && H % 2 == 0 && W % 2 == 0 && ldx >= 8 && ldx % 8 == 0, "stem_fwd: bad geometry (H, W even; 8 physical input channels)");
  USSEG_CHECK_ARG(((((uintptr_t)b1) | ((uintptr_t)b2) | ((uintptr_t)b3) | ((uintptr_t)gamma) | ((uintptr_t)beta) | ((uintptr_t)mean) | ((uintptr_t)var)) & 15) == 0,
                  "stem_fwd: per-channel vectors must be 16-byte aligned");
  StemFwd p = {};
  p.x = (const bf16_t*)x; p.w1 = (const bf16_t*)w1; p.w2 = (const bf16_t*)w2; p.w3 = (const bf16_t*)w3;
  p.b1 = b1; p.b2 = b2; p.b3 = b3; p.gamma = gamma; p.beta = beta; p.mean = mean; p.var = var;
  p.y1 = (bf16_t*)y1; p.t1 = (bf16_t*)t1; p.c2 = (bf16_t*)c2; p.pooled = (bf16_t*)pooled;
  p.B = B; p.H = H; p.W = W; p.ldx = ldx; p.alpha = alpha; p.eps = eps;
  p.tiles_x = (W + T - 1) / T;
  p.ntiles = p.tiles_x * ((H + TH - 1) / TH);
  if (usseg_lds_opt_in((const void*)stem_fwd_kernel, LDS_B)) return usseg_check_launch("stem_fwd");
  hipStream_t s = (hipStream_t)stream;
  const int slot = usseg_prof_start(4, s);
  hipLaunchKernelGGL(stem_fwd_kernel, dim3(p.ntiles, B), dim3(256), LDS_B, s, p);
  usseg_prof_stop(4, slot, s);
  return usseg_check_launch("stem_fwd");
}

extern "C" int usseg_stem_fwd_infer(int32_t B, int32_t H, int32_t W, const void* x, int32_t ldx, const void* w1, const float* b1, const void* w2,
                                    const float* b2, const void* w3, const float* b3, const float* gamma, const float* beta, const float* mean,
                                    const float* var, float eps, float alpha, void* pooled, usseg_stream_t stream) {
  USSEG_CHECK_ARG(x && w1 && b1 && w2 && b2 && w3 && b3 && gamma && beta && mean && var && pooled, "stem_fwd_infer: null pointer");
  USSEG_CHECK_ARG(B > 0 && H > 0 && W > 0 && H % 2 == 0 && W % 2 == 0 && ldx >= 8 && ldx % 8 == 0, "stem_fwd_infer: bad geometry (H, W even; 8 physical input channels)");
  USSEG_CHECK_ARG(((((uintptr_t)b1) | ((uintptr_t)b2) | ((uintptr_t)b3) | ((uintptr_t)gamma) | ((uintptr_t)beta) | ((uintptr_t)mean) | ((uintptr_t)var)) & 15) == 0,
                  "stem_fwd_infer: per-channel vectors must be 16-byte aligned");
  StemFwd p = {};
  p.x = (const bf16_t*)x; p.w1 = (const bf16_t*)w1; p.w2 = (const bf16_t*)w2; p.w3 = (const bf16_t*)w3;
  p.b1 = b1; p.b2 = b2; p.b3 = b3; p.gamma = gamma; p.beta = beta; p.mean = mean; p.var = var;
  p.pooled = (bf16_t*)pooled;
  p.B = B; p.H = H; p.W = W; p.ldx = ldx; p.alpha = alpha; p.eps = eps;
  p.tiles_x = (W + T - 1) / T;
  p.ntiles = p.tiles_x * ((H + TH - 1) / TH);
  if (usseg_lds_opt_in((const void*)stem_fwd_infer_kernel, LDS_B)) return usseg_check_launch("stem_fwd_infer");
  hipStream_t s = (hipStream_t)stream;
  const int slot = usseg_prof_start(4, s);
  hipLaunchKernelGGL(stem_fwd_infer_kernel, dim3(p.ntiles, B), dim3(256), LDS_B, s, p);
  usseg_prof_stop(4, slot, s);
  return usseg_check_launch("stem_fwd_infer");
}

extern "C" int usseg_conv3_dgrad_actbwd(int32_t B, int32_t H, int32_t W, const void* dy, int32_t lddy, const void* wd, int32_t Co, const void* yact,
                                        int32_t ldy, int32_t mode, const float* gamma, const float* beta, const float* var, float eps, float alpha,
                                        void* dx, int32_t lddx, float* dgamma, float* dbeta, float* dbias, float* ws, usseg_stream_t stream) {
  USSEG_CHECK_ARG(dy && wd && yact && dx && dbias && ws && B > 0 && H > 0 && W > 0, "conv3_dgrad_actbwd: null pointer / bad geometry");
  USSEG_CHECK_ARG(lddy >= 32 && lddy % 8 == 0 && ldy >= Co && ldy % 4 == 0 && lddx >= Co && lddx % 4 == 0, "conv3_dgrad_actbwd: bad strides");
  USSEG_CHECK_ARG(mode == 0 || (mode == 2 && gamma && beta && var && dgamma && dbeta), "conv3_dgrad_actbwd: mode 0 (activation) or 2 (folded BatchNorm)");
  if (!((Co == 32 && mode == 2) || (Co == 16 && mode == 0))) {
    usseg_set_error("conv3_dgrad_actbwd: no fused kernel for %d channels / mode %d", Co, mode);
    return USSEG_ERR_UNSUPPORTED;
  }
  DgAct p = {};
  p.dy = (const bf16_t*)dy; p.wd = (const bf16_t*)wd; p.yact = (const bf16_t*)yact; p.dx = (bf16_t*)dx;
  p.gamma = gamma; p.beta = beta; p.var = var;
  p.B = B; p.H = H; p.W = W; p.lddy = lddy; p.ldy = ldy; p.lddx = lddx; p.eps = eps; p.alpha = alpha;
  p.tiles_x = (W + 15) / 16;
  const int64_t total = (int64_t)p.tiles_x * ((H + 15) / 16) * B;
  USSEG_CHECK_ARG(total < (1ll << 31), "conv3_dgrad_actbwd: too many tiles");
  p.ntiles = (int)total;
  constexpr int DG_GRID = 512;
  static_assert(DG_GRID <= USSEG_REDUCE_MAX_BLOCKS, "one partial row per workgroup");
  const int grid = p.ntiles < DG_GRID ? p.ntiles : DG_GRID;
  hipStream_t s = (hipStream_t)stream;
  p.ws = usseg_defer_reduce_ws(s, ws, (int64_t)grid * 3 * Co);
  const int slot = usseg_prof_start(4, s);
  if (mode == 2) hipLaunchKernelGGL((dgrad_actbwd_kernel<32, 2>), dim3(grid), dim3(256), 0, s, p);
  else hipLaunchKernelGGL((dgrad_actbwd_kernel<16, 0>), dim3(grid), dim3(256), 0, s, p);
  usseg_prof_stop(4, slot, s);
  if (mode == 2) usseg_launch_reduce_finish(p.ws, 1, grid, 3, Co, Co, 1.f, dgamma, dbeta, dbias, s, 0);
  else usseg_launch_reduce_finish(p.ws + 2 * Co, 1, grid, 1, 3 * Co, Co, 1.f, dbias, nullptr, nullptr, s, 0);
  return usseg_check_launch("conv3_dgrad_actbwd");
}
```

### ultrasound_modeling_amd/csrc/stem_fwd_body.inc

```
#if defined(__HIP_DEVICE_COMPILE__)
  extern __shared__ __attribute__((aligned(16))) char lds[];
  bf16_t* const XT = reinterpret_cast<bf16_t*>(lds);
  bf16_t* const Y1T = reinterpret_cast<bf16_t*>(lds + XS_B);
  bf16_t* const T1T = reinterpret_cast<bf16_t*>(lds + XS_B + Y1_B);
  bf16_t* const C2T = reinterpret_cast<bf16_t*>(lds);
  const int tid = threadIdx.x, lane = tid & 63, wv = __builtin_amdgcn_readfirstlane(tid >> 6);
  const int r = lane & 15, q = lane >> 4;
  WFrag<1, 1> wf1;
  WFrag<2, 2> wf2;
  wf1.load(p.w1, r, q);
  wf2.load(p.w2, r, q);
  {
  const int b = blockIdx.y, tile = blockIdx.x;
  const int tyi = tile / p.tiles_x, txi = tile - tyi * p.tiles_x;
  const int ty0 = tyi * TH, tx0 = txi * T;
  const int64_t img = (int64_t)b * p.H * p.W;
  {
    uint4 v[2];
#pragma unroll
    for (int i = 0; i < 2; ++i) {
      const int hp = tid + 256 * i;
      const int hy = hp / XW, hx = hp - hy * XW;
      const int gy = ty0 - 3 + hy, gx = tx0 - 3 + hx;
      v[i] = (hp < XW * XH && gy >= 0 && gy < p.H && gx >= 0 && gx < p.W)
                 ? *reinterpret_cast<const uint4*>(p.x + (img + (int64_t)gy * p.W + gx) * p.ldx) : make_uint4(0, 0, 0, 0);
    }
#pragma unroll
    for (int i = 0; i < 2; ++i) {
      const int hp = tid + 256 * i;
      if (hp < XW * XH) *reinterpret_cast<uint4*>(XT + hp * XS) = v[i];
    }
  }
  __syncthreads();
  conv_phase<1, 1, Y1W, Y1H, XS, Y1S, true, true>(XT, Y1T, wf1, p.b1, p.alpha, ty0 - 2, tx0 - 2, p.H, p.W, wv, r, q);
  WFrag<4, 2> wf3;
  wf3.load(p.w3, r, q);
  __syncthreads();
  if constexpr (STASH) store_interior<Y1W, 2, 2, Y1S>(Y1T, p.y1, img, 16, ty0, tx0, p.H, p.W, tid);
  conv_phase<2, 2, T1W, T1H, Y1S, T1S, true, true>(Y1T, T1T, wf2, p.b2, p.alpha, ty0 - 1, tx0 - 1, p.H, p.W, wv, r, q);
  __syncthreads();
  if constexpr (STASH) store_interior<T1W, 1, 4, T1S>(T1T, p.t1, img, 32, ty0, tx0, p.H, p.W, tid);
  conv_phase<4, 2, T, TH, T1S, C2S, false, false>(T1T, C2T, wf3, p.b3, 0.f, ty0, tx0, p.H, p.W, wv, r, q);
  __syncthreads();
  if constexpr (STASH) store_interior<T, 0, 4, C2S>(C2T, p.c2, img, 32, ty0, tx0, p.H, p.W, tid);
  if (tid < (T / 2) * (TH / 2) * 4) {
    const int pp = tid >> 2, c = tid & 3;
    const int oy = pp >> 3, ox = pp & 7;
    const int gy = (ty0 >> 1) + oy, gx = (tx0 >> 1) + ox;
    float ga[8], be[8], mu[8], rs[8];
    *reinterpret_cast<float4*>(ga) = *reinterpret_cast<const float4*>(p.gamma + c * 8);
    *reinterpret_cast<float4*>(ga + 4) = *reinterpret_cast<const float4*>(p.gamma + c * 8 + 4);
    *reinterpret_cast<float4*>(be) = *reinterpret_cast<const float4*>(p.beta + c * 8);
    *reinterpret_cast<float4*>(be + 4) = *reinterpret_cast<const float4*>(p.beta + c * 8 + 4);
    *reinterpret_cast<float4*>(mu) = *reinterpret_cast<const float4*>(p.mean + c * 8);
    *reinterpret_cast<float4*>(mu + 4) = *reinterpret_cast<const float4*>(p.mean + c * 8 + 4);
    *reinterpret_cast<float4*>(rs) = *reinterpret_cast<const float4*>(p.var + c * 8);
    *reinterpret_cast<float4*>(rs + 4) = *reinterpret_cast<const float4*>(p.var + c * 8 + 4);
#pragma unroll
    for (int j = 0; j < 8; ++j) rs[j] = rsqrtf(rs[j] + p.eps);
    float acc[8];
#pragma unroll
    for (int j = 0; j < 8; ++j) acc[j] = 0.f;
#pragma unroll
    for (int s = 0; s < 4; ++s) {
      const int iy = 2 * oy + (s >> 1), ix = 2 * ox + (s & 1);
      float xv[8], o[8], r8[8];
      unpack8(*reinterpret_cast<const uint4*>(C2T + (iy * T + ix) * C2S + c * 8), xv);
#pragma unroll
      for (int j = 0; j < 8; ++j) {
        const float v = ga[j] * ((xv[j] - mu[j]) * rs[j]) + be[j];
        o[j] = v >= 0.f ? v : p.alpha * v;
      }
      unpack8(pack8(o), r8);
#pragma unroll
      for (int j = 0; j < 8; ++j) acc[j] += r8[j];
    }
#pragma unroll
    for (int j = 0; j < 8; ++j) acc[j] *= 0.25f;
    if (gy < (p.H >> 1) && gx < (p.W >> 1))
      *reinterpret_cast<uint4*>(p.pooled + ((int64_t)b * (p.H >> 1) * (p.W >> 1) + (int64_t)gy * (p.W >> 1) + gx) * 32 + c * 8) = pack8(acc);
  }
  }
#endif
```

### ultrasound_modeling_amd/knobs.py

```python
from __future__ import annotations

import os

KNOBS = {
    "USSEG_LIB":                ("str",    None,  "path of a diagnostic build of the same sources to load instead of the in-tree library"),
    "USSEG_SIDE_STREAM":        ("flag",   0,     "weight gradients fork to a side stream per launch inside an overlap region"),
    "USSEG_DEFER":              ("flag",   1,     "defer the finishing reductions to the end of the region (0: finish after each producer)"),
    "USSEG_LAZY_WGRAD":         ("flag",   1,     "lazy weight gradients: queued and run on the side stream beside the backward-data chain"),
    "USSEG_FUSE_LN_RES":        ("flag",   1,     "LayerNorm backward + residual add in one pass (transformer blocks)"),
    "USSEG_ENC_LAZY":           ("optint", None,  "bit mask of the ResNest stages whose weight gradients are lazy (unset: 12, or 0 in front of a ViT)"),
    "USSEG_FOLD_BN":            ("flag",   1,     "inference BatchNorm folded into the producing conv's packed weights"),
    "USSEG_FUSED_CARDINAL":     ("flag",   1,     "cardinal group + shortcut of a stage as one launch"),
    "USSEG_FUSED_CARDINAL_BWD": ("flag",   1,     "its backward chain + the shortcut norm's backward as one launch"),
    "USSEG_CARD_BWD_MAX_PX":    ("int",    32768, "most pixels of a stage for the fused cardinal backward"),
    "USSEG_LN_PAIR":            ("flag",   1,     "shortcut norm backward + conv2_bn backward of the large stages in one launch"),
    "USSEG_FUSED_STEM_BWD":     ("flag",   1,     "stem backward-data fused with the norm / activation backward in front"),
    "USSEG_STEM_WGRAD_MERGE":   ("flag",   1,     "the stem's three weight gradients in one multi-job launch"),
    "USSEG_FUSED_STEM":         ("flag",   1,     "the stem (three convs, two norms, pool) as one launch"),
    "USSEG_MERGED_DGRAD":       ("flag",   1,     "one backward-data GEMM for a stage's grouped 1x1 and shortcut 1x1"),
    "USSEG_FUSED_DGRAD":        ("flag",   1,     "the DecoderBlock's four branch backward-data passes as one launch"),
    "USSEG_BRANCH4":            ("flag",   1,     "the DecoderBlock's 1x1 branch as a fourth job of the dilated branches' launch"),
    "USSEG_QUAD_UP":            ("flag",   0,     "the decoder's transposed convs in quad (parity-class) form"),
    "USSEG_QUAD_HEAD":          ("flag",   1,     "the <= 4-class head's transposed conv in quad form (read at construction)"),
    "USSEG_QUAD_TCONV":         ("flag",   0,     "Arch A's inner transposed convs in quad form (read at construction)"),
    "USSEG_STAGE_LAZY":         ("flag",   1,     "Arch A: per-stage lazy weight gradients"),
    "USSEG_FUSED_HEAD":         ("flag",   1,     "head conv + softmax + loss as one launch"),
    "USSEG_VIT_LAZY":           ("str",    "enc", "lazy weight gradients of the ViT: whole encoder (enc), per block (block), or 0"),
    "USSEG_FUSED_ATTN":         ("flag",   1,     "train-step attention on the fused kernels (head size 128)"),
    "USSEG_SWIN_LAZY":          ("flag",   1,     "Swin: per-block lazy weight gradients"),
    "USSEG_DIST_BACKEND":       ("str",    None,  "torch.distributed backend (unset: nccl with a GPU, else gloo)"),
    "USSEG_DP_CHUNKS":          ("int",    0,     "chunks of the pipelined gradient exchange (0 or 1: one exchange)"),
}


def get(name: str):
    rule, default, _ = KNOBS[name]
    v = os.environ.get(name)
    if rule == "flag":
        return bool(default) if v is None else v != "0"
    if v is None:
        return default
    return v if rule == "str" else int(v)
```

### ultrasound_modeling_amd/ops.py

```python
from __future__ import annotations

import contextlib
import ctypes as C
import math
import os
from typing import Optional, Tuple

import torch

from . import _lib as L
from . import knobs
from ._lib import (ACCUMULATE, ACT_ELU, ACT_GELU, ACT_LRELU, ACT_NONE, ACT_RELU, OUT_F32, CardinalDesc, ConvDesc, GemmDesc, LossDesc, NormDesc,
                   SplitAttnDesc, SplitAttnGrads, SplitAttnParams)

BF16 = torch.bfloat16
ACC_FLOATS = 2050


def roundup(a: int, b: int) -> int:
    return (a + b - 1) // b * b


def _stream() -> int:
    return torch.cuda.current_stream().cuda_stream
# ... 446 lines not shown
    B, H, W, Cphys, _ = geom(x)
    d = _norm_desc(x, C_logical, geom(out)[4], G, mode, eps, act, alpha)
    gamma, beta, mean, var = (_readable(t, Cphys) for t in (gamma, beta, mean, var))
    nb = max(1, min(32, (H * W) // 32))
    rows = torch.empty((B, nb, Cphys), dtype=torch.float32, device=x.device)
    L.check(L.load().usseg_norm_act_fwd_gap(C.byref(d), x.data_ptr(), gamma.data_ptr(), beta.data_ptr(), _ptr(mean), _ptr(var), out.data_ptr(),
                                            B, nb, rows.data_ptr(), _stream()), "norm_act_fwd_gap")
    return out, (rows, nb, Cphys)


def norm_act_bwd_sa(x, dout, C_logical, gamma, beta, dx, dgamma, dbeta, mode, G, eps, act, alpha, sa_s, sa_dg, sa_mult, mean=None, var=None,
                    dbias=None):
    B, H, W, Cphys, ldx = geom(x)
    d = NormDesc(B * H * W, C_logical, Cphys, ldx, geom(dout)[4], G, mode, eps, act, alpha, geom(dx)[4])
    gamma, beta, mean, var = (_readable(t, Cphys) for t in (gamma, beta, mean, var))
    L.check(L.load().usseg_norm_act_bwd_sa(C.byref(d), x.data_ptr(), dout.data_ptr(), gamma.data_ptr(), beta.data_ptr(), _ptr(mean), _ptr(var), B,
                                           sa_s.data_ptr(), sa_dg.data_ptr(), sa_mult, dx.data_ptr(), dgamma.data_ptr(), dbeta.data_ptr(),
                                           _ptr(dbias), reduce_ws(x.device).data_ptr(), _stream()), "norm_act_bwd_sa")
    return dx


def norm_act_bwd_pair(xa, dya, Ca, gamma_a, beta_a, dxa, dgamma_a, dbeta_a, dbias_a, xb, doutb, Cb, Gb, gamma_b, beta_b, dxb, dgamma_b, dbeta_b,
                      dbias_b, sa_s, sa_dg, sa_mult, eps, alpha) -> bool:
    Ba, Ha, Wa, Cpa, ldxa = geom(xa)
    Bb, Hb, Wb, Cpb, ldxb = geom(xb)
    da = NormDesc(Ba * Ha * Wa, Ca, Cpa, ldxa, geom(dya)[4], 1, 0, eps, ACT_LRELU, alpha, geom(dxa)[4])
    db = NormDesc(Bb * Hb * Wb, Cb, Cpb, ldxb, geom(doutb)[4], Gb, 0, eps, ACT_LRELU, alpha, geom(dxb)[4])
    gamma_a, beta_a, gamma_b, beta_b = (_readable(t, n) for t, n in ((gamma_a, Cpa), (beta_a, Cpa), (gamma_b, Cpb), (beta_b, Cpb)))
    rc = L.load().usseg_norm_act_bwd_pair(C.byref(da), xa.data_ptr(), dya.data_ptr(), gamma_a.data_ptr(), beta_a.data_ptr(), dxa.data_ptr(),
                                          dgamma_a.data_ptr(), dbeta_a.data_ptr(), dbias_a.data_ptr(), C.byref(db), xb.data_ptr(), doutb.data_ptr(),
                                          gamma_b.data_ptr(), beta_b.data_ptr(), Bb, sa_s.data_ptr(), sa_dg.data_ptr(), float(sa_mult), dxb.data_ptr(),
                                          dgamma_b.data_ptr(), dbeta_b.data_ptr(), dbias_b.data_ptr(), reduce_ws(xa.device).data_ptr(), _stream())
    if rc == -2:
        return False
    L.check(rc, "norm_act_bwd_pair")
    return True


def norm_act_bwd(x, dy, C_logical, gamma, beta, dx, dgamma, dbeta, mode, G=1, eps=1e-3, act=ACT_NONE, alpha=0.0, mean=None,
                 var=None, dbias=None, mask=None):
    B, H, W, Cphys, ldx = geom(x)
    lddy = geom(dy)[4]
    d = NormDesc(B * H * W, C_logical, Cphys, ldx, lddy, G, mode, eps, act, alpha, geom(dx)[4])
    gamma, beta, mean, var = (_readable(t, Cphys) for t in (gamma, beta, mean, var))
    ldm = geom(mask)[4] if mask is not None else 0
    L.check(L.load().usseg_norm_act_bwd(C.byref(d), x.data_ptr(), dy.data_ptr(), gamma.data_ptr(), beta.data_ptr(), _ptr(mean),
                                        _ptr(var), _ptr(mask), ldm, dx.data_ptr(), dgamma.data_ptr(), dbeta.data_ptr(), _ptr(dbias),
                                        reduce_ws(x.device).data_ptr(), _stream()), "norm_act_bwd")
    return dx


def accuracy(probs, y_true, acc):
    assert acc.numel() >= ACC_FLOATS and probs.is_contiguous() and y_true.is_contiguous() and probs.dtype == y_true.dtype == torch.float32
    C_ = probs.shape[-1]
    L.check(L.load().usseg_accuracy(probs.data_ptr(), y_true.data_ptr(), probs.numel() // C_, C_, acc.data_ptr(), _stream()), "accuracy")
    return acc[0]


def seg_counts(y_true, probs, counts, round=True, num_classes=3):
    assert y_true.shape == probs.shape and y_true.dim() == 4, (tuple(y_true.shape), tuple(probs.shape))
    assert y_true.dtype == probs.dtype == torch.float32 and y_true.is_contiguous() and probs.is_contiguous()
    assert counts.dtype == torch.int64 and counts.is_contiguous() and counts.numel() >= L.SEG_COUNTS
    if not (y_true.is_cuda and probs.is_cuda and counts.is_cuda):
        raise RuntimeError("seg_counts: device tensors only (there is no CPU fallback)")
    B, H, W, C_ = y_true.shape
    d = L.SegCountDesc(B, H, W, C_, int(num_classes), int(bool(round)))
    L.check(L.load().usseg_seg_counts(C.byref(d), y_true.data_ptr(), probs.data_ptr(), counts.data_ptr(), _stream()), "seg_counts")
    return counts


def cascade_gate(probs, x, out=None, mask=None):
    B, H, W, Cm = probs.shape
    assert probs.dtype == torch.float32 and probs.is_contiguous() and probs.is_cuda
    assert x.dtype == BF16 and x.is_contiguous() and tuple(x.shape[:3]) == (B, H, W), (tuple(x.shape), tuple(probs.shape))
    out = torch.empty_like(x) if out is None else out
    assert out.dtype == BF16 and out.is_contiguous() and out.shape == x.shape
    if mask is not None:
        assert mask.dtype == torch.uint8 and mask.is_contiguous() and tuple(mask.shape) == (B, H, W)
    L.check(L.load().usseg_cascade_gate(probs.data_ptr(), Cm, B * H * W, x.data_ptr(), x.shape[3], out.data_ptr(), _ptr(mask), _stream()),
            "cascade_gate")
    return out


def cascade_maps(probs, prob_map=None, bleed_prob=None):
    B, H, W, Cc = probs.shape
    assert probs.dtype == torch.float32 and probs.is_contiguous() and probs.is_cuda
    prob_map = torch.empty((B, H, W), dtype=torch.float32, device=probs.device) if prob_map is None else prob_map
    bleed_prob = torch.empty((B, H, W), dtype=torch.float32, device=probs.device) if bleed_prob is None else bleed_prob
    for t in (prob_map, bleed_prob):
        assert t.dtype == torch.float32 and t.is_contiguous() and tuple(t.shape) == (B, H, W)
    L.check(L.load().usseg_cascade_maps(probs.data_ptr(), Cc, B * H * W, prob_map.data_ptr(), bleed_prob.data_ptr(), _stream()),
            "cascade_maps")
    return prob_map, bleed_prob


def norm_act_bwd_res(x, dy, C_logical, gamma, beta, dres, dx, dgamma, dbeta, eps, dbias=None):
    B, H, W, Cphys, ldx = geom(x)
    d = NormDesc(B * H * W, C_logical, Cphys, ldx, geom(dy)[4], 1, 0, eps, ACT_NONE, 0.0, geom(dx)[4])
    L.check(L.load().usseg_norm_act_bwd_res(C.byref(d), x.data_ptr(), dy.data_ptr(), gamma.data_ptr(), beta.data_ptr(), dres.data_ptr(),
                                            geom(dres)[4], dx.data_ptr(), dgamma.data_ptr(), dbeta.data_ptr(), _ptr(dbias),
                                            reduce_ws(x.device).data_ptr(), _stream()), "norm_act_bwd_res")
    return dx


def bn_act_pool_fwd(x, C_logical, gamma, beta, mean, var, eps, act, alpha, out=None):
    B, H, W, Cp, ldx = geom(x)
    out = out if out is not None else new_act(B, H // 2, W // 2, Cp, x.device)
    L.check(L.load().usseg_bn_act_pool_fwd(x.data_ptr(), B, H, W, C_logical, Cp, ldx, gamma.data_ptr(), beta.data_ptr(), mean.data_ptr(), var.data_ptr(),
                                           eps, act, alpha, out.data_ptr(), geom(out)[4], _stream()), "bn_act_pool_fwd")
    return out


def bn_act_pool_bwd(x, dy, C_logical, gamma, beta, mean, var, eps, act, alpha, dx, dgamma, dbeta, dbias=None):
    B, H, W, Cp, ldx = geom(x)
    L.check(L.load().usseg_bn_act_pool_bwd(x.data_ptr(), dy.data_ptr(), B, H, W, C_logical, Cp, ldx, geom(dy)[4], gamma.data_ptr(), beta.data_ptr(),
                                           mean.data_ptr(), var.data_ptr(), eps, act, alpha, dx.data_ptr(), geom(dx)[4], dgamma.data_ptr(),
                                           dbeta.data_ptr(), _ptr(dbias), reduce_ws(x.device).data_ptr(), _stream()), "bn_act_pool_bwd")
    return dx


def dropout_mask(mask, seed: int, rate: float, step_dev=None):
    B, H, W, Cc, ld = geom(mask)
    if step_dev is not None:
        L.check(L.load().usseg_dropout_mask_step(mask.data_ptr(), B * H * W, Cc, ld, seed, step_dev.data_ptr(), rate, _stream()), "dropout_mask_step")
        return mask
    L.check(L.load().usseg_dropout_mask(mask.data_ptr(), B * H * W, Cc, ld, seed, rate, _stream()), "dropout_mask")
    return mask


def counter_add(counter, inc: int = 1):
    assert counter.dtype == torch.int32
    L.check(L.load().usseg_counter_add(counter.data_ptr(), inc, _stream()), "counter_add")


def channel_stats(x, C_logical, s, s2):
    B, H, W, _, ldx = geom(x)
    L.check(L.load().usseg_channel_stats(x.data_ptr(), B * H * W, C_logical, ldx, s.data_ptr(), s2.data_ptr(),
                                         reduce_ws(x.device).data_ptr(), _stream()), "channel_stats")


def bn_finalize_stats(s, s2, M, C_logical, momentum, mean, var, moving_mean=None, moving_var=None):
    L.check(L.load().usseg_bn_finalize_stats(s.data_ptr(), s2.data_ptr(), M, C_logical, momentum, mean.data_ptr(), var.data_ptr(),
                                             _ptr(moving_mean), _ptr(moving_var), _stream()), "bn_finalize_stats")


def bn_batch_stats(x, C_logical, momentum, mean, var, moving_mean=None, moving_var=None):
    B, H, W, _, ldx = geom(x)
    L.check(L.load().usseg_bn_batch_stats(x.data_ptr(), B * H * W, C_logical, ldx, momentum, mean.data_ptr(), var.data_ptr(), _ptr(moving_mean),
                                          _ptr(moving_var), reduce_ws(x.device).data_ptr(), _stream()), "bn_batch_stats")


def bn_train_bwd_fix(x, dx, C_logical, gamma, mean, var, eps, tg, tb):
    B, H, W, Cphys, ldx = geom(x)
    L.check(L.load().usseg_bn_train_bwd_fix(x.data_ptr(), dx.data_ptr(), B * H * W, C_logical, Cphys, ldx, geom(dx)[4], gamma.data_ptr(),
                                            mean.data_ptr(), var.data_ptr(), eps, tg.data_ptr(), tb.data_ptr(), _stream()), "bn_train_bwd_fix")


def act_fwd(x, out, act, alpha):
    B, H, W, Cc, ldx = geom(x)
    L.check(L.load().usseg_act_fwd(x.data_ptr(), B * H * W, Cc, ldx, geom(out)[4], act, alpha, out.data_ptr(), _stream()), "act_fwd")
    return out


def act_bwd(x, dy, dx, act, alpha):
    B, H, W, Cc, ldx = geom(x)
    L.check(L.load().usseg_act_bwd(x.data_ptr(), dy.data_ptr(), B * H * W, Cc, ldx, geom(dy)[4], geom(dx)[4], act, alpha,
                                   dx.data_ptr(), _stream()), "act_bwd")
    return dx


def act_bwd_colsum(x, dy, dx, act, alpha, db, C_logical):
    B, H, W, Cc, ldx = geom(x)
    L.check(L.load().usseg_act_bwd_colsum(x.data_ptr(), dy.data_ptr(), B * H * W, C_logical, ldx, geom(dy)[4], geom(dx)[4], act, alpha, dx.data_ptr(),
                                          db.data_ptr(), reduce_ws(x.device).data_ptr(), _stream()), "act_bwd_colsum")
    return dx


def avgpool2_fwd(x, out):
    B, H, W, Cc, ldx = geom(x)
    L.check(L.load().usseg_avgpool2_fwd(x.data_ptr(), B, H, W, Cc, ldx, geom(out)[4], out.data_ptr(), _stream()), "avgpool2_fwd")
    return out


def avgpool2_bwd(dy, dx, add=None, db=None):
    B, H, W, Cc, lddx = geom(dx)
    ldadd = geom(add)[4] if add is not None else 0
    if db is not None and Cc <= 512:
        L.check(L.load().usseg_avgpool2_bwd_colsum(dy.data_ptr(), B, H, W, Cc, geom(dy)[4], lddx, _ptr(add), ldadd, dx.data_ptr(), db.data_ptr(),
                                                   reduce_ws(dx.device).data_ptr(), _stream()), "avgpool2_bwd_colsum")
        return dx
    L.check(L.load().usseg_avgpool2_bwd(dy.data_ptr(), B, H, W, Cc, geom(dy)[4], lddx, _ptr(add), ldadd, dx.data_ptr(),
                                        _stream()), "avgpool2_bwd")
    if db is not None:
        colsum(dx, db)
    return dx


def copy_channels(src, dst, accumulate=False):
    B, H, W, Cc, lds = geom(src)
    Bd, Hd, Wd, Cd, ldd = geom(dst)
    assert B * H * W == Bd * Hd * Wd and Cc == Cd
    L.check(L.load().usseg_copy_channels(src.data_ptr(), B * H * W, Cc, lds, dst.data_ptr(), ldd, 1 if accumulate else 0,
                                         _stream()), "copy_channels")
    return dst


def cast_input(x: torch.Tensor, Cphys: int) -> torch.Tensor:
    assert x.is_cuda and x.is_contiguous() and x.dtype in (torch.float32, torch.float64)
    B, H, W, Cc = x.shape
    out = new_act(B, H, W, Cphys, x.device)
    L.check(L.load().usseg_cast_input(x.data_ptr(), 1 if x.dtype == torch.float64 else 0, B * H * W, Cc, out.data_ptr(), Cphys,
                                      _stream()), "cast_input")
    return out


def to_f32(x: torch.Tensor, C_logical: Optional[int] = None) -> torch.Tensor:
    B, H, W, Cc, ld = geom(x)
    Cl = C_logical or Cc
    out = torch.empty((B, H, W, Cl), dtype=torch.float32, device=x.device)
    L.check(L.load().usseg_cast_bf16_to_f32(x.data_ptr(), B * H * W, Cl, ld, out.data_ptr(), _stream()), "cast_bf16_to_f32")
    return out


def colsum(dy, db: torch.Tensor, C_logical: Optional[int] = None):
    B, H, W, Cc, ld = geom(dy)
    L.check(L.load().usseg_colsum(dy.data_ptr(), B * H * W, C_logical or Cc, ld, db.data_ptr(), reduce_ws(dy.device).data_ptr(),
                                  _stream()), "colsum")


def fill_f32(t: torch.Tensor, value: float = 0.0):
    assert t.dtype == torch.float32 and t.is_contiguous()
    L.check(L.load().usseg_fill_f32(t.data_ptr(), t.numel(), value, _stream()), "fill_f32")


def sumsq(g: torch.Tensor, out: torch.Tensor):
    assert out.numel() >= ACC_FLOATS, "sumsq accumulates through a USSEG_ACC_FLOATS buffer"
    L.check(L.load().usseg_sumsq(g.data_ptr(), g.numel(), out.data_ptr(), _stream()), "sumsq")


def sum_f32(x: torch.Tensor, out: torch.Tensor):
    assert out.numel() >= ACC_FLOATS and x.dtype == torch.float32 and x.is_contiguous()
    L.check(L.load().usseg_sum_f32(x.data_ptr(), x.numel(), out.data_ptr(), _stream()), "sum_f32")
    return out[0]


def sumsq_advance(g: torch.Tensor, out: torch.Tensor, step_dev, lr_t_dev, lr, b1, b2):
    assert out.numel() >= ACC_FLOATS
    L.check(L.load().usseg_sumsq_advance(g.data_ptr(), g.numel(), out.data_ptr(), step_dev.data_ptr(), lr_t_dev.data_ptr(), lr, b1, b2, _stream()),
            "sumsq_advance")


def reinject_hidden(hidden: torch.Tensor, views, backward: bool):
    assert hidden.is_contiguous() and hidden.dtype == BF16 and 1 <= len(views) <= 4
    n = len(views)
    bufs = (C.c_void_p * n)(*[v.data_ptr() for v in views])
    c0 = (C.c_int32 * n)(*[v.shape[3] for v in views])
    ld = (C.c_int32 * n)(*[geom(v)[4] for v in views])
    for v in views:
        assert v.numel() == hidden.numel()
    L.check(L.load().usseg_reinject_hidden(hidden.data_ptr(), hidden.numel(), n, bufs, c0, ld, 1 if backward else 0, _stream()), "reinject_hidden")


def scale_by_clip(g: torch.Tensor, sumsq_t: torch.Tensor, clip_norm: float):
    L.check(L.load().usseg_scale_f32(g.data_ptr(), g.numel(), sumsq_t.data_ptr(), clip_norm, _stream()), "scale_f32")


def adam_clip_step(p, g, m, v, sumsq_t, clip_norm, lr_t_dev, b1, b2, eps):
    L.check(L.load().usseg_adam_clip_step(p.data_ptr(), g.data_ptr(), m.data_ptr(), v.data_ptr(), p.numel(), _ptr(sumsq_t),
                                          clip_norm, lr_t_dev.data_ptr(), b1, b2, eps, _stream()), "adam_clip_step")


def adam_advance(step_dev, lr_t_dev, lr, b1, b2):
    L.check(L.load().usseg_adam_advance(step_dev.data_ptr(), lr_t_dev.data_ptr(), lr, b1, b2, _stream()), "adam_advance")


def sched_advance(step_dev, sched_dev, lr_t_dev, wd_t_dev, b1, b2):
    L.check(L.load().usseg_sched_advance(step_dev.data_ptr(), sched_dev.data_ptr(), lr_t_dev.data_ptr(), wd_t_dev.data_ptr(), b1, b2, _stream()),
            "sched_advance")


def sumsq_sched_advance(g: torch.Tensor, out: torch.Tensor, step_dev, sched_dev, lr_t_dev, wd_t_dev, b1, b2):
    assert out.numel() >= ACC_FLOATS
    L.check(L.load().usseg_sumsq_sched_advance(g.data_ptr(), g.numel(), out.data_ptr(), step_dev.data_ptr(), sched_dev.data_ptr(), lr_t_dev.data_ptr(),
                                               wd_t_dev.data_ptr(), b1, b2, _stream()), "sumsq_sched_advance")


def adamw_step(p, g, m, v, sumsq_t, clip_norm, lr_t_dev, wd_t_dev, decay_mask, b1, b2, eps):
    L.check(L.load().usseg_adamw_step(p.data_ptr(), g.data_ptr(), m.data_ptr(), v.data_ptr(), p.numel(), _ptr(sumsq_t), clip_norm,
                                      lr_t_dev.data_ptr(), wd_t_dev.data_ptr(), _ptr(decay_mask), b1, b2, eps, _stream()), "adamw_step")


def stem_fwd(x, w1, b1, w2, b2, w3, b3, gamma, beta, mean, var, eps, alpha):
    B, H, W, Cin, ldx = geom(x)
    assert Cin == 8 and x.dtype == BF16
    dev = x.device
    y1, t1, c2 = new_act(B, H, W, 16, dev), new_act(B, H, W, 32, dev), new_act(B, H, W, 32, dev)
    pooled = new_act(B, H // 2, W // 2, 32, dev)
    L.check(L.load().usseg_stem_fwd(B, H, W, x.data_ptr(), ldx, w1.data_ptr(), b1.data_ptr(), w2.data_ptr(), b2.data_ptr(), w3.data_ptr(),
                                    b3.data_ptr(), gamma.data_ptr(), beta.data_ptr(), mean.data_ptr(), var.data_ptr(), eps, alpha,
                                    y1.data_ptr(), t1.data_ptr(), c2.data_ptr(), pooled.data_ptr(), _stream()), "stem_fwd")
    return y1, t1, c2, pooled


def stem_fwd_infer(x, w1, b1, w2, b2, w3, b3, gamma, beta, mean, var, eps, alpha):
    B, H, W, Cin, ldx = geom(x)
    assert Cin == 8 and x.dtype == BF16
    pooled = new_act(B, H // 2, W // 2, 32, x.device)
    L.check(L.load().usseg_stem_fwd_infer(B, H, W, x.data_ptr(), ldx, w1.data_ptr(), b1.data_ptr(), w2.data_ptr(), b2.data_ptr(), w3.data_ptr(),
                                          b3.data_ptr(), gamma.data_ptr(), beta.data_ptr(), mean.data_ptr(), var.data_ptr(), eps, alpha,
                                          pooled.data_ptr(), _stream()), "stem_fwd_infer")
    return pooled


def conv3_dgrad_actbwd(dy, wd, yact, dx, mode, alpha, dbias, gamma=None, beta=None, var=None, eps=1e-3, dgamma=None, dbeta=None) -> bool:
    B, H, W, Cdy, lddy = geom(dy)
    Co = yact.shape[-1]
    if Cdy != 32 or tuple(wd.shape) != (roundup(Co, 16), 9 * 32):
        return False
    rc = L.load().usseg_conv3_dgrad_actbwd(B, H, W, dy.data_ptr(), lddy, wd.data_ptr(), Co, yact.data_ptr(), geom(yact)[4], mode, _ptr(gamma), _ptr(beta),
                                           _ptr(var), eps, alpha, dx.data_ptr(), geom(dx)[4], _ptr(dgamma), _ptr(dbeta), dbias.data_ptr(),
                                           reduce_ws(dy.device).data_ptr(), _stream())
    if rc == -2:
        return False
    L.check(rc, "conv3_dgrad_actbwd")
    return True


def cardinal_desc(B, H, W, Cin, P, cv11, cvkk, Up, Vp, Oc, ldx, ldu, ldv, ldsc, eps, alpha) -> CardinalDesc:
    return CardinalDesc(B, H, W, Cin, P, cv11, cvkk, Up, Vp, Oc, ldx, ldu, ldv, ldsc, eps, alpha)


def cardinal_supported(Cin, P, cv11, cvkk, Up, Vp, Oc) -> bool:
    d = cardinal_desc(1, 8, 8, Cin, P, cv11, cvkk, Up, Vp, Oc, Cin, Up, Vp, Oc, 1e-3, 0.3)
    return bool(L.load().usseg_cardinal_supported(C.byref(d)))


def cardinal_fwd(x, w1, b1, g1, be1, w2, b2, g2, be2, wsc, bsc, gsc, besc, P, cv11, cvkk, Up, Vp, Oc, eps, alpha):
    B, H, W, Cin, ldx = geom(x)
    dev = x.device
    u_raw, u = new_act(B, H, W, Up, dev), new_act(B, H, W, Up, dev)
    v_raw, y = new_act(B, H, W, Vp, dev), new_act(B, H, W, Vp, dev)
    sc_raw, sc = new_act(B, H, W, Oc, dev), new_act(B, H, W, Oc, dev)
    tiles = ((H + 7) // 8) * ((W + 7) // 8)
    rows = torch.empty((B, tiles, Vp), dtype=torch.float32, device=dev)
    d = cardinal_desc(B, H, W, Cin, P, cv11, cvkk, Up, Vp, Oc, ldx, Up, Vp, Oc, eps, alpha)
    g1, be1, g2, be2, gsc, besc = (_readable(t, n) for t, n in ((g1, P * cv11), (be1, P * cv11), (g2, P * cvkk), (be2, P * cvkk), (gsc, Oc), (besc, Oc)))
    L.check(L.load().usseg_cardinal_fwd(C.byref(d), x.data_ptr(), w1.data_ptr(), b1.data_ptr(), g1.data_ptr(), be1.data_ptr(), w2.data_ptr(),
                                        b2.data_ptr(), g2.data_ptr(), be2.data_ptr(), wsc.data_ptr(), bsc.data_ptr(), gsc.data_ptr(), besc.data_ptr(),
                                        u_raw.data_ptr(), u.data_ptr(), v_raw.data_ptr(), y.data_ptr(), rows.data_ptr(), sc_raw.data_ptr(),
                                        sc.data_ptr(), _stream()), "cardinal_fwd")
    return u_raw, u, v_raw, y, (rows, tiles, Vp), sc_raw, sc


def cardinal_fwd_infer(x, w1, b1, g1, be1, w2, b2, g2, be2, wsc, bsc, gsc, besc, P, cv11, cvkk, Up, Vp, Oc, eps, alpha):
    B, H, W, Cin, ldx = geom(x)
    dev = x.device
    y, sc = new_act(B, H, W, Vp, dev), new_act(B, H, W, Oc, dev)
    tiles = ((H + 7) // 8) * ((W + 7) // 8)
    rows = torch.empty((B, tiles, Vp), dtype=torch.float32, device=dev)
    d = cardinal_desc(B, H, W, Cin, P, cv11, cvkk, Up, Vp, Oc, ldx, Up, Vp, Oc, eps, alpha)
    g1, be1, g2, be2, gsc, besc = (_readable(t, n) for t, n in ((g1, P * cv11), (be1, P * cv11), (g2, P * cvkk), (be2, P * cvkk), (gsc, Oc), (besc, Oc)))
    L.check(L.load().usseg_cardinal_fwd_infer(C.byref(d), x.data_ptr(), w1.data_ptr(), b1.data_ptr(), g1.data_ptr(), be1.data_ptr(), w2.data_ptr(),
                                              b2.data_ptr(), g2.data_ptr(), be2.data_ptr(), wsc.data_ptr(), bsc.data_ptr(), gsc.data_ptr(),
                                              besc.data_ptr(), y.data_ptr(), rows.data_ptr(), sc.data_ptr(), _stream()), "cardinal_fwd_infer")
    return y, (rows, tiles, Vp), sc


def cardinal_bwd(dout, dsc, v_raw, u_raw, sc_raw, w2d, g2, be2, g1, be1, gsc, besc, sa_s, sa_dg, sa_mult, dv, dcat, grads, Cin, P, cv11, cvkk, Up,
                 Vp, Oc, eps, alpha):
    B, H, W, _, ldo = geom(dout)
    d = cardinal_desc(B, H, W, Cin, P, cv11, cvkk, Up, Vp, Oc, Cin, geom(u_raw)[4], geom(v_raw)[4], geom(sc_raw)[4], eps, alpha)
    assert geom(dv)[4] == d.ldv and dcat.shape[-1] >= Up + Oc
    g2, be2, g1, be1, gsc, besc = (_readable(t, n) for t, n in ((g2, P * cvkk), (be2, P * cvkk), (g1, P * cv11), (be1, P * cv11), (gsc, Oc), (besc, Oc)))
    L.check(L.load().usseg_cardinal_bwd(C.byref(d), dout.data_ptr(), ldo, dsc.data_ptr(), geom(dsc)[4], v_raw.data_ptr(), u_raw.data_ptr(),
                                        sc_raw.data_ptr(), w2d.data_ptr(), g2.data_ptr(), be2.data_ptr(), g1.data_ptr(), be1.data_ptr(),
                                        gsc.data_ptr(), besc.data_ptr(), sa_s.data_ptr(), sa_dg.data_ptr(), float(sa_mult), dv.data_ptr(),
                                        dcat.data_ptr(), geom(dcat)[4], *[t.data_ptr() for t in grads], reduce_ws(dout.device).data_ptr(),
                                        _stream()), "cardinal_bwd")
    return dv, dcat


def splitattn_desc(B, HW, P, R, Cg, Hd, ldy, ldo, Cy_phys, Co_phys, mult, norm_mode, eps, act, alpha, use_sigmoid) -> SplitAttnDesc:
    return SplitAttnDesc(B, HW, P, R, Cg, Hd, ldy, ldo, Cy_phys, Co_phys, mult, norm_mode, eps, act, alpha, 1 if use_sigmoid else 0)


def _sa_params(w1, b1, gamma, beta, mean, var, w2, b2) -> SplitAttnParams:
    return SplitAttnParams(_ptr(w1), _ptr(b1), _ptr(gamma), _ptr(beta), _ptr(mean), _ptr(var), _ptr(w2), _ptr(b2))


def splitattn_fwd(d: SplitAttnDesc, y, params, out, gap=None):
    dev = y.device
    Cy = d.P * d.R * d.Cg
    s = torch.empty((d.B, Cy), dtype=torch.float32, device=dev)
    ws = torch.empty(d.B * d.P * (d.Cg + 2 * d.Hd), dtype=torch.float32, device=dev)
    lib = L.load()
    if gap is None:
        g = torch.empty((d.B, Cy), dtype=torch.float32, device=dev)
        L.check(lib.usseg_splitattn_gap(C.byref(d), y.data_ptr(), g.data_ptr(), reduce_ws(dev).data_ptr(), _stream()), "splitattn_gap")
        gap = (g, 1, Cy)
    sp = _sa_params(*params)
    L.check(lib.usseg_splitattn_mlp_fwd(C.byref(d), gap[0].data_ptr(), gap[1], gap[2], C.byref(sp), s.data_ptr(), ws.data_ptr(), _stream()),
            "splitattn_mlp_fwd")
    L.check(lib.usseg_splitattn_apply_fwd(C.byref(d), y.data_ptr(), s.data_ptr(), out.data_ptr(), _stream()), "splitattn_apply_fwd")
    return out, gap, s, ws


def splitattn_bwd(d: SplitAttnDesc, y, dout, params, grads, g, s, ws, dy):
    dev = y.device
    Cy = d.P * d.R * d.Cg
    dg = torch.empty((d.B, Cy), dtype=torch.float32, device=dev)
    lib = L.load()
    lddo = geom(dout)[4]
    if not isinstance(g, tuple):
        g = (g, 1, Cy)
    sp = _sa_params(*params)
    sg = SplitAttnGrads(*[_ptr(t) for t in grads])
    gws = torch.empty(int(lib.usseg_splitattn_mlp_bwd_ws_floats(C.byref(d))), dtype=torch.float32, device=dev)
    L.check(lib.usseg_splitattn_bwd_fused(C.byref(d), y.data_ptr(), dout.data_ptr(), lddo, g[0].data_ptr(), g[1], g[2], C.byref(sp), s.data_ptr(),
                                          ws.data_ptr(), dg.data_ptr(), C.byref(sg), reduce_ws(dev).data_ptr(), gws.data_ptr(), _stream()),
            "splitattn_bwd_fused")
    if dy is None:
        assert d.R == 1, "the fused re-weighting backward needs identical radix branches (R == 1)"
        return s, dg
    L.check(lib.usseg_splitattn_apply_bwd_dy(C.byref(d), dout.data_ptr(), lddo, s.data_ptr(), dg.data_ptr(), dy.data_ptr(), geom(dy)[4],
                                             _stream()), "splitattn_apply_bwd_dy")
    return dy


def class_loss(w, gamma=0.0, factor=1.0) -> L.ClassLoss:
    w = [float(v) for v in w]
    gamma, factor = float(gamma), float(factor)
    if not 1 <= len(w) <= 8:
        raise ValueError(f"class loss: 1 to 8 class weights, got {len(w)}")
    if not (gamma == 0.0 or 1.0 <= gamma <= 8.0):
        raise ValueError(f"class loss: gamma must be 0 or lie in [1, 8], got {gamma}")
    if not all(math.isfinite(v) and v >= 0.0 for v in w + [factor]):
        raise ValueError(f"class loss: weights and factor must be finite and >= 0, got {w}, {factor}")
    return L.ClassLoss((L.c_f32 * 8)(*w), gamma, factor)


def softmax_loss(logits, y_true, probs, loss, dlogits, *, HW, C_classes, loss_kind=0, label_smoothing=0.1, clip_eps=1e-7,
                 inv_global_batch=1.0, scale=None, quad_w=0, class_loss=None):
    M = probs.numel() // C_classes
    ldl = logits.shape[-1]
    if class_loss is not None:
        assert scale is None and (loss is None or loss.numel() >= ACC_FLOATS)
        d = LossDesc(M, HW, C_classes, ldl, 16 if quad_w else 8, 2, label_smoothing, clip_eps, inv_global_batch, quad_w)
        L.check(L.load().usseg_softmax_loss_fwd_bwd_cl(C.byref(d), C.byref(class_loss), logits.data_ptr(), _ptr(y_true), probs.data_ptr(), _ptr(loss),
                                                       _ptr(dlogits), _stream()), "softmax_loss_cl")
        return
    assert loss is None or loss_kind == 1 or loss.numel() >= ACC_FLOATS, "the scalar loss accumulates through a USSEG_ACC_FLOATS buffer"
    d = LossDesc(M, HW, C_classes, ldl, 16 if quad_w else 8, loss_kind, label_smoothing, clip_eps, inv_global_batch, quad_w)
    L.check(L.load().usseg_softmax_loss_fwd_bwd(C.byref(d), logits.data_ptr(), _ptr(y_true), _ptr(scale), probs.data_ptr(), _ptr(loss),
                                                _ptr(dlogits), _stream()), "softmax_loss")


def head_quad_softmax_loss(x, wq, bias, C_classes, y_true, probs, loss, dlogits, *, label_smoothing=0.1, clip_eps=1e-7, inv_global_batch=1.0,
                           class_loss=None) -> bool:
    B, h, w, Cx, ldx = geom(x)
    assert tuple(wq.shape) == (16, 9 * Cx) and (loss is None or loss.numel() >= ACC_FLOATS)
    if class_loss is not None:
        rc = L.load().usseg_head_quad_softmax_loss_cl(x.data_ptr(), B, h, w, Cx, ldx, wq.data_ptr(), bias.data_ptr(), C_classes, _ptr(y_true),
                                                      probs.data_ptr(), _ptr(loss), _ptr(dlogits), label_smoothing, clip_eps, inv_global_batch,
                                                      C.byref(class_loss), _stream())
    else:
        rc = L.load().usseg_head_quad_softmax_loss(x.data_ptr(), B, h, w, Cx, ldx, wq.data_ptr(), bias.data_ptr(), C_classes, _ptr(y_true), probs.data_ptr(),
                                                   _ptr(loss), _ptr(dlogits), label_smoothing, clip_eps, inv_global_batch, _stream())
    if rc == -2:
        return False
    L.check(rc, "head_quad_softmax_loss")
    return True


def loss_from_probs(probs, y_true, loss, *, HW, C_classes, loss_kind=0, label_smoothing=0.1, clip_eps=1e-7, inv_global_batch=1.0, scale=None,
                    class_loss=None, as_map=False):
    assert probs.dtype == torch.float32 and y_true.dtype == torch.float32 and probs.is_contiguous() and y_true.is_contiguous()
    M = probs.numel() // C_classes
    if class_loss is not None:
        assert scale is None and loss.numel() >= (HW if as_map else ACC_FLOATS)
        d = LossDesc(M, HW, C_classes, C_classes, 8, 2, label_smoothing, clip_eps, inv_global_batch, 0)
        L.check(L.load().usseg_loss_from_probs_cl(C.byref(d), C.byref(class_loss), probs.data_ptr(), y_true.data_ptr(), loss.data_ptr(), int(as_map),
                                                  _stream()), "loss_from_probs_cl")
        return
    assert loss_kind == 1 or loss.numel() >= ACC_FLOATS
    d = LossDesc(M, HW, C_classes, C_classes, 8, loss_kind, label_smoothing, clip_eps, inv_global_batch, 0)
    L.check(L.load().usseg_loss_from_probs(C.byref(d), probs.data_ptr(), y_true.data_ptr(), _ptr(scale), loss.data_ptr(), _stream()),
            "loss_from_probs")


OVERLAP_ACC_FLOATS = 8224
OVERLAP_KEYS = ("alpha", "beta", "smooth", "power", "class_weight", "ce_weight", "ov_weight")


def overlap_loss(class_weight, alpha=0.5, beta=0.5, smooth=1.0, power=1.0, ov_weight=1.0, ce_weight=0.0) -> L.OverlapLoss:
    w = [float(v) for v in class_weight]
    alpha, beta, smooth, power, ov_weight, ce_weight = (float(v) for v in (alpha, beta, smooth, power, ov_weight, ce_weight))
    if not 1 <= len(w) <= 4:
        raise ValueError(f"overlap loss: 1 to 4 class weights, got {len(w)}")
    if not 1.0 <= power <= 4.0:
        raise ValueError(f"overlap loss: power must lie in [1, 4], got {power}")
    if not (math.isfinite(smooth) and smooth > 0.0):
        raise ValueError(f"overlap loss: smooth must be finite and > 0, got {smooth}")
    if not all(math.isfinite(v) and v >= 0.0 for v in w + [alpha, beta, ov_weight, ce_weight]):
        raise ValueError(f"overlap loss: weights, alpha and beta must be finite and >= 0, got {w}, {alpha}, {beta}, {ov_weight}, {ce_weight}")
    if ov_weight == 0.0 and ce_weight == 0.0:
        raise ValueError("overlap loss: ov_weight and ce_weight are both zero")
    return L.OverlapLoss((L.c_f32 * 8)(*w), alpha, beta, smooth, power, ov_weight, ce_weight)


def overlap_loss_grid(M: int) -> int:
    return int(L.load().usseg_overlap_loss_grid(int(M)))


def _overlap_desc(probs, y_true, HW, C_classes, lddl, label_smoothing, clip_eps, inv_global_batch, quad_w):
    assert probs.dtype == torch.float32 and y_true.dtype == torch.float32 and probs.is_contiguous() and y_true.is_contiguous()
    assert probs.shape == y_true.shape
    return LossDesc(probs.numel() // C_classes, HW, C_classes, C_classes, lddl, 0, label_smoothing, clip_eps, inv_global_batch, quad_w)


def overlap_loss_sums(probs, y_true, acc, *, overlap, HW, C_classes, ov_scale=1.0, label_smoothing=0.1, clip_eps=1e-7, inv_global_batch=1.0):
    d = _overlap_desc(probs, y_true, HW, C_classes, 8, label_smoothing, clip_eps, inv_global_batch, 0)
    L.check(L.load().usseg_overlap_loss_sums(C.byref(d), C.byref(overlap), ov_scale, probs.data_ptr(), y_true.data_ptr(), acc.data_ptr(), acc.numel(),
                                             _stream()), "overlap_loss_sums")


def overlap_loss_bwd(probs, y_true, acc, dlogits, *, overlap, HW, C_classes, label_smoothing=0.1, clip_eps=1e-7, inv_global_batch=1.0, quad_w=0):
    d = _overlap_desc(probs, y_true, HW, C_classes, 16 if quad_w else 8, label_smoothing, clip_eps, inv_global_batch, quad_w)
    L.check(L.load().usseg_overlap_loss_bwd(C.byref(d), C.byref(overlap), probs.data_ptr(), y_true.data_ptr(), acc.data_ptr(), acc.numel(),
                                            dlogits.data_ptr(), _stream()), "overlap_loss_bwd")


BOUNDARY_KEYS = ("weight", "class_weight", "threshold")


def boundary_loss(class_weight) -> L.BoundaryLoss:
    u = [float(v) for v in class_weight]
    if not 1 <= len(u) <= 4:
        raise ValueError(f"boundary loss: 1 to 4 class weights, got {len(u)}")
    if not all(math.isfinite(v) and v >= 0.0 for v in u):
        raise ValueError(f"boundary loss: class weights must be finite and >= 0, got {u}")
    return L.BoundaryLoss((L.c_f32 * 8)(*u))


def sdf_ws_bytes(B: int, H: int, W: int, C_classes: int) -> int:
    n = int(L.load().usseg_sdf_ws_bytes(B, H, W, C_classes))
    if n < 0:
        raise ValueError(f"sdf_labels: H and W must lie in [1, 8192] and C in [1, 4], got {B}x{H}x{W}x{C_classes}")
    return n


def sdf_labels(y_true, phi=None, ws=None, *, threshold=0.5):
    assert y_true.dtype == torch.float32 and y_true.is_contiguous() and y_true.dim() == 4
    B, H, W, Cc = y_true.shape
    need = sdf_ws_bytes(B, H, W, Cc)
    if phi is None:
        phi = torch.empty_like(y_true)
    if ws is None:
        ws = torch.empty(max(need, 16), dtype=torch.uint8, device=y_true.device)
    assert phi.dtype == torch.float32 and phi.is_contiguous() and phi.shape == y_true.shape and ws.dtype == torch.uint8
    L.check(L.load().usseg_sdf_labels(y_true.data_ptr(), B, H, W, Cc, float(threshold), phi.data_ptr(), ws.data_ptr(), ws.numel(), _stream()), "sdf_labels")
    return phi


def surface_dist(a, b, ws=None):
    assert a.dtype == torch.uint8 and b.dtype == torch.uint8 and a.is_contiguous() and b.is_contiguous() and a.dim() == 3 and a.shape == b.shape
    N, H, W = a.shape
    need = int(L.load().usseg_surface_ws_bytes(N, H, W))
    if need < 0:
        raise ValueError(f"surface_dist: H and W must lie in [1, 8192], got {N}x{H}x{W}")
    if ws is None:
        ws = torch.empty(max(need, 16), dtype=torch.uint8, device=a.device)
    counters = torch.empty((N, 4), dtype=torch.int64, device=a.device)
    sums = torch.empty((N, 2), dtype=torch.float64, device=a.device)
    L.check(L.load().usseg_surface_dist(a.data_ptr(), b.data_ptr(), N, H, W, counters.data_ptr(), sums.data_ptr(), ws.data_ptr(), ws.numel(), _stream()),
            "surface_dist")
    return counters, sums


def surface_stats_ws_bytes(N: int, H: int, W: int) -> int:
    n = int(L.load().usseg_surface_stats_ws_bytes(N, H, W))
    if n < 0:
        raise ValueError(f"surface_stats: H and W must lie in [1, 8192], got {N}x{H}x{W}")
    return n


def surface_stats(a, b, percentiles=(), tol2=(), *, ws=None, out=None):
    assert a.dtype == torch.uint8 and b.dtype == torch.uint8 and a.is_contiguous() and b.is_contiguous() and a.dim() == 3 and a.shape == b.shape
    N, H, W = a.shape
    quant = [float(q) / 100 for q in percentiles]
    t2 = [int(t) for t in tol2]
    P, T = len(quant), len(t2)
    if P > 4 or T > 4:
        raise ValueError(f"surface_stats: at most 4 percentiles and 4 tolerances, got {P} and {T}")
    if not all(math.isfinite(q) and 0.0 <= q <= 1.0 for q in quant):
        raise ValueError(f"surface_stats: percentiles must lie in [0, 100], got {list(percentiles)}")
    if not all(0 <= t < 2 ** 31 and t == v for t, v in zip(t2, tol2)):
        raise ValueError(f"surface_stats: squared tolerances must be integers in [0, 2^31), got {list(tol2)}")
    need = surface_stats_ws_bytes(N, H, W)
    if ws is None:
        ws = torch.empty(max(need, 16), dtype=torch.uint8, device=a.device)
    if out is None:
        out = (torch.empty((N, 4), dtype=torch.int64, device=a.device), torch.empty((N, 2), dtype=torch.float64, device=a.device),
               torch.empty((N, 3, P, 2), dtype=torch.int32, device=a.device), torch.empty((N, T, 2), dtype=torch.int64, device=a.device))
    counters, sums, sel, within = out
    for t, dt, shape in ((counters, torch.int64, (N, 4)), (sums, torch.float64, (N, 2)), (sel, torch.int32, (N, 3, P, 2)), (within, torch.int64, (N, T, 2))):
        assert t.dtype == dt and tuple(t.shape) == shape and t.is_contiguous() and t.device == a.device and ws.dtype == torch.uint8
    if N == 0:
        return counters, sums, sel, within
    L.check(L.load().usseg_surface_stats(a.data_ptr(), b.data_ptr(), N, H, W, (C.c_double * max(P, 1))(*quant), P, (C.c_int32 * max(T, 1))(*t2), T,
                                         counters.data_ptr(), sums.data_ptr(), sel.data_ptr() if P else None, within.data_ptr() if T else None,
                                         ws.data_ptr(), ws.numel(), _stream()), "surface_stats")
    return counters, sums, sel, within


COMPONENT_STAT_FIELDS = ("area", "y_min", "x_min", "y_max", "x_max", "sum_y", "sum_x", "peak_bits")


def components_ws_bytes(N: int, H: int, W: int) -> int:
    n = int(L.load().usseg_components_ws_bytes(N, H, W))
    if n < 0:
        raise ValueError(f"components: H and W must lie in [1, 8192], N in [0, 65535] and N*H*W <= 2^29, got {N}x{H}x{W}")
    return n


def _component_mask(mask, what):
    assert mask.dtype == torch.uint8 and mask.is_contiguous() and mask.dim() == 3, f"{what}: a contiguous uint8 [N,H,W] mask"
    return mask.shape
# ... 494 lines not shown
```

Baseline: 5814.

## Fuse one-channel stem conv1 weight gradient into dgrad epilogue, read f32 input directly

For a single-channel f32 input, the stem forward gets a variant that reads the fp32 image directly, so the separate cast/pad-to-8-channel launch is skipped. In backward, the first conv's activation-backward kernel now also accumulates conv1's 3x3x1x16 weight gradient from the staged input tile. It no longer writes the 16-channel input gradient, which is not needed for the network input. This removes a cast kernel, a 16-channel gradient write and a separate wgrad pass, at the cost of extra register accumulators and an LDS reduction in the dgrad kernel.

```diff
diff --git a/include/usseg.h b/include/usseg.h
--- a/include/usseg.h
+++ b/include/usseg.h
@@ -169,12 +169,18 @@
 int usseg_stem_fwd(int32_t B, int32_t H, int32_t W, const void* x, int32_t ldx, const void* w1, const float* b1, const void* w2, const float* b2,
                    const void* w3, const float* b3, const float* gamma, const float* beta, const float* mean, const float* var, float eps,
                    float alpha, void* y1, void* t1, void* c2, void* pooled, usseg_stream_t stream);
+int usseg_stem_fwd_f32(int32_t B, int32_t H, int32_t W, const float* x, const void* w1, const float* b1, const void* w2, const float* b2,
+                       const void* w3, const float* b3, const float* gamma, const float* beta, const float* mean, const float* var, float eps,
+                       float alpha, void* y1, void* t1, void* c2, void* pooled, usseg_stream_t stream);
 int usseg_stem_fwd_infer(int32_t B, int32_t H, int32_t W, const void* x, int32_t ldx, const void* w1, const float* b1, const void* w2,
                          const float* b2, const void* w3, const float* b3, const float* gamma, const float* beta, const float* mean,
                          const float* var, float eps, float alpha, void* pooled, usseg_stream_t stream);
 int usseg_conv3_dgrad_actbwd(int32_t B, int32_t H, int32_t W, const void* dy, int32_t lddy, const void* wd, int32_t Co, const void* yact, int32_t ldy,
                              int32_t mode, const float* gamma, const float* beta, const float* var, float eps, float alpha, void* dx,
                              int32_t lddx, float* dgamma, float* dbeta, float* dbias, float* ws, usseg_stream_t stream);
+int usseg_conv3_dgrad_actbwd_wgrad1(int32_t B, int32_t H, int32_t W, const void* dy, int32_t lddy, const void* wd, const void* yact, int32_t ldy,
+                                    const void* x, int32_t ldx, int32_t x_is_f32, float alpha, void* dx, int32_t lddx, float* dbias, float* dw,
+                                    float* ws, usseg_stream_t stream);
 typedef struct UssegCardinalDesc {
   int32_t B, H, W;
   int32_t Cin;
diff --git a/ultrasound_modeling_amd/ResNest.py b/ultrasound_modeling_amd/ResNest.py
--- a/ultrasound_modeling_amd/ResNest.py
+++ b/ultrasound_modeling_amd/ResNest.py
@@ -22,6 +22,7 @@
 _LN_PAIR = knobs.get("USSEG_LN_PAIR")
 _FUSED_STEM_BWD = knobs.get("USSEG_FUSED_STEM_BWD")
 _STEM_WGRAD_MERGE = knobs.get("USSEG_STEM_WGRAD_MERGE")
+_STEM_LEAN_BWD = knobs.get("USSEG_STEM_LEAN_BWD")
 _FUSED_STEM = knobs.get("USSEG_FUSED_STEM")
 _MERGED_DGRAD = knobs.get("USSEG_MERGED_DGRAD")
 
@@ -391,13 +392,24 @@
 
     def forward(self, x, outs=None, stash=True):
         o3, o2, o1 = outs if outs is not None else (None, None, None)
-        if x.dtype != BF16:
-            x = ops.cast_input(x.contiguous(), roundup(self.channel, 8))
         a = KERAS_LRELU_ALPHA
         bn1, bn2 = self.convtmp_1bn, self.convtmp_2bn
         self._fold = self.convtmp_1.fold_scale() is not None
-        if (_FUSED_STEM and self._fold and not bn2.training_mode and self.conv1.cin_p == 8 and x.shape[1] % 2 == 0 and x.shape[2] % 2 == 0
-                and (self.conv1.cout, self.convtmp_1.cout, self.convtmp_2.cout) == (16, 32, 32)):
+        fused = (_FUSED_STEM and self._fold and not bn2.training_mode and self.conv1.cin_p == 8 and x.shape[1] % 2 == 0 and x.shape[2] % 2 == 0
+                 and (self.conv1.cout, self.convtmp_1.cout, self.convtmp_2.cout) == (16, 32, 32))
+        lean = _STEM_LEAN_BWD and _FUSED_STEM_BWD and stash and x.dtype == torch.float32 and self.channel == 1 and x.shape[3] == 1
+        self._x_f32 = x.contiguous() if lean else None
+        if lean and fused:
+            self._y1, self._t1, c2, t = ops.stem_fwd_f32(self._x_f32, self.conv1.wp_f, self.conv1.bias.data, self.convtmp_1.wp_f, bn1.fold_shift,
+                                                         self.convtmp_2.wp_f, self.convtmp_2.bias.data, bn2.gamma.data, bn2.beta.data,
+                                                         bn2.moving_mean_p, bn2.moving_variance_p, bn2.eps, a)
+            self.conv1._x, self.convtmp_1._x, self.convtmp_2._x = self._x_f32, self._y1, self._t1
+            bn2._x, bn2._act = c2, (ACT_LRELU, a)
+            self._pool_fused = self._stem_fused = True
+            return self._stages_forward(t, o1, o2, o3)
+        if x.dtype != BF16:
+            x = ops.cast_input(x.contiguous(), roundup(self.channel, 8))
+        if fused:
             if not stash:
                 t = ops.stem_fwd_infer(x, self.conv1.wp_f, self.conv1.bias.data, self.convtmp_1.wp_f, bn1.fold_shift, self.convtmp_2.wp_f,
                                        self.convtmp_2.bias.data, bn2.gamma.data, bn2.beta.data, bn2.moving_mean_p, bn2.moving_variance_p, bn2.eps, a)
@@ -474,8 +486,13 @@
                 d = bn1.backward_folded(self._t1, d, ACT_LRELU, a, dbias=c1.bias.grad)
             else:
                 d = bn1.backward(d, dbias=c1.bias.grad)
-        dn = torch.empty_like(self._y1) if _FUSED_STEM_BWD else None
-        if dn is not None and ops.conv3_dgrad_actbwd(d, c1.wp_d, self._y1, dn, 0, KERAS_LRELU_ALPHA, self.conv1.bias.grad):
+        x1 = self._x_f32 if getattr(self, "_x_f32", None) is not None else self.conv1._x
+        lean = (_STEM_LEAN_BWD and _FUSED_STEM_BWD and self.conv1.cin == 1 and x1 is not None
+                and ops.conv3_dgrad_actbwd_wgrad1(d, c1.wp_d, self._y1, x1, KERAS_LRELU_ALPHA, self.conv1.bias.grad, self.conv1.kernel.grad))
+        dn = torch.empty_like(self._y1) if (_FUSED_STEM_BWD and not lean) else None
+        if lean:
+            wg(c1, d)
+        elif dn is not None and ops.conv3_dgrad_actbwd(d, c1.wp_d, self._y1, dn, 0, KERAS_LRELU_ALPHA, self.conv1.bias.grad):
             wg(c1, d)
             d = dn
         else:
@@ -483,7 +500,8 @@
                 wjobs.append(c1.wgrad_job(d))
             d = c1.backward(d, skip_bias=True, skip_wgrad=wjobs is not None)
             d = ops.act_bwd_colsum(self._y1, d, torch.empty_like(d), ACT_LRELU, KERAS_LRELU_ALPHA, self.conv1.bias.grad, self.conv1.cout)
-        wg(self.conv1, d)
+        if not lean:
+            wg(self.conv1, d)
         if wjobs:
             keep = [t for job in wjobs for t in job[:2]]
             ops.wgrad_later(lambda: ops.conv2d_wgrad_multi(wjobs), *keep)
diff --git a/ultrasound_modeling_amd/_lib.py b/ultrasound_modeling_amd/_lib.py
--- a/ultrasound_modeling_amd/_lib.py
+++ b/ultrasound_modeling_amd/_lib.py
@@ -178,10 +178,14 @@
     "usseg_norm_act_fwd_gap": (C.c_int, [P(NormDesc), c_vp, c_vp, c_vp, c_vp, c_vp, c_vp, c_i32, c_i32, c_vp, c_vp]),
     "usseg_stem_fwd": (C.c_int, [c_i32, c_i32, c_i32, c_vp, c_i32, c_vp, c_vp, c_vp, c_vp, c_vp, c_vp, c_vp, c_vp, c_vp, c_vp, c_f32, c_f32,
                                  c_vp, c_vp, c_vp, c_vp, c_vp]),
+    "usseg_stem_fwd_f32": (C.c_int, [c_i32, c_i32, c_i32, c_vp, c_vp, c_vp, c_vp, c_vp, c_vp, c_vp, c_vp, c_vp, c_vp, c_vp, c_f32, c_f32,
+                                     c_vp, c_vp, c_vp, c_vp, c_vp]),
     "usseg_stem_fwd_infer": (C.c_int, [c_i32, c_i32, c_i32, c_vp, c_i32, c_vp, c_vp, c_vp, c_vp, c_vp, c_vp, c_vp, c_vp, c_vp, c_vp, c_f32, c_f32,
                                        c_vp, c_vp]),
     "usseg_conv3_dgrad_actbwd": (C.c_int, [c_i32, c_i32, c_i32, c_vp, c_i32, c_vp, c_i32, c_vp, c_i32, c_i32, c_vp, c_vp, c_vp, c_f32, c_f32, c_vp, c_i32,
                                            c_vp, c_vp, c_vp, c_vp, c_vp]),
+    "usseg_conv3_dgrad_actbwd_wgrad1": (C.c_int, [c_i32, c_i32, c_i32, c_vp, c_i32, c_vp, c_vp, c_i32, c_vp, c_i32, c_i32, c_f32, c_vp, c_i32,
+                                                  c_vp, c_vp, c_vp, c_vp]),
     "usseg_cardinal_supported": (c_i32, [P(CardinalDesc)]),
     "usseg_cardinal_fwd": (C.c_int, [P(CardinalDesc)] + [c_vp] * 21),
     "usseg_cardinal_fwd_infer": (C.c_int, [P(CardinalDesc)] + [c_vp] * 17),
diff --git a/ultrasound_modeling_amd/csrc/stem.hip b/ultrasound_modeling_amd/csrc/stem.hip
--- a/ultrasound_modeling_amd/csrc/stem.hip
+++ b/ultrasound_modeling_amd/csrc/stem.hip
@@ -4,6 +4,7 @@
 
 struct StemFwd {
   const bf16_t* x;
+  const float* xf;
   const bf16_t *w1, *w2, *w3;
   const float *b1, *b2, *b3, *gamma, *beta, *mean, *var;
   bf16_t *y1, *t1, *c2, *pooled;
@@ -108,12 +109,17 @@
 }
 
 __global__ __launch_bounds__(256) void stem_fwd_kernel(const StemFwd p) {
-  constexpr bool STASH = true;
+  constexpr bool STASH = true, XF32 = false;
 #include "stem_fwd_body.inc"
 }
 
 __global__ __launch_bounds__(256) void stem_fwd_infer_kernel(const StemFwd p) {
-  constexpr bool STASH = false;
+  constexpr bool STASH = false, XF32 = false;
+#include "stem_fwd_body.inc"
+}
+
+__global__ __launch_bounds__(256) void stem_fwd_f32_kernel(const StemFwd p) {
+  constexpr bool STASH = true, XF32 = true;
 #include "stem_fwd_body.inc"
 }
 
@@ -124,184 +130,22 @@
   float* ws;
   int32_t B, H, W, lddy, ldy, lddx, tiles_x, ntiles;
   float eps, alpha;
+  const void* x;
+  float* wws;
+  int32_t ldx, x_f32;
 };
 [[maybe_unused]] constexpr int DG_S = 40;
 
 template <int CO, int MODE>
 __global__ __launch_bounds__(256, 2) void dgrad_actbwd_kernel(const DgAct p) {
-#if defined(__HIP_DEVICE_COMPILE__)
-  constexpr int TW = 16, HWD = TW + 2, NT = CO / 16, NIT = (HWD * HWD * 4 + 255) / 256, CL = 4 * NT;
-  __shared__ __attribute__((aligned(16))) bf16_t DT[2][HWD * HWD * DG_S];
-  __shared__ float RED[4][4][NT * 4 * 3];
-  const int tid = threadIdx.x, lane = tid & 63, wv = tid >> 6, r = lane & 15, q = lane >> 4;
-  constexpr bool WREG = NT == 1;
-  __shared__ __attribute__((aligned(16))) bf16_t WL[WREG ? 8 : 9 * NT * 64 * 8];
-  __shared__ __attribute__((aligned(16))) float CST[3][CO];
-  auto wrow = [&](int t, int nt) { return p.wd + (int64_t)(CL * (r >> 2) + 4 * nt + (r & 3)) * 288 + (8 - t) * 32 + q * 8; };
-  bf16x8_t a[WREG ? 9 : 1][NT];
-  if constexpr (WREG) {
-#pragma unroll
-    for (int t = 0; t < 9; ++t) a[t][0] = *reinterpret_cast<const bf16x8_t*>(wrow(t, 0));
-  } else if (wv == 0) {
-#pragma unroll
-    for (int t = 0; t < 9; ++t)
-#pragma unroll
-      for (int nt = 0; nt < NT; ++nt) *reinterpret_cast<bf16x8_t*>(WL + ((t * NT + nt) * 64 + lane) * 8) = *reinterpret_cast<const bf16x8_t*>(wrow(t, nt));
-  }
-  if (MODE == 2 && tid < CO) {
-    const float g = p.gamma[tid];
-    CST[0][tid] = g * rsqrtf(p.var[tid] + p.eps);
-    CST[1][tid] = p.beta[tid];
-    CST[2][tid] = fabsf(g) > 1e-20f ? 1.f / g : 0.f;
-  }
-  const float inv_neg = p.alpha != 0.f ? 1.f / p.alpha : 1.f;
-  float sga[NT][4], sbe[NT][4], sbi[NT][4];
-#pragma unroll
-  for (int nt = 0; nt < NT; ++nt)
-#pragma unroll
-    for (int j = 0; j < 4; ++j) sga[nt][j] = sbe[nt][j] = sbi[nt][j] = 0.f;
-  const int tiles_img = p.tiles_x * ((p.H + TW - 1) / TW);
-  uint4 dv[NIT];
-  auto load_dy = [&](int t) -> uint32_t {
-    const int b = t / tiles_img, tile = t - b * tiles_img;
-    const int tyi = tile / p.tiles_x, txi = tile - tyi * p.tiles_x;
-    const int64_t img = (int64_t)b * p.H * p.W;
-    uint32_t m = 0;
-#pragma unroll
-    for (int i = 0; i < NIT; ++i) {
-      const int it = tid + i * 256;
-      const int hp = min(it >> 2, HWD * HWD - 1), c = it & 3;
-      const int hy = hp / HWD, hx = hp - hy * HWD;
-      const int gy = tyi * TW - 1 + hy, gx = txi * TW - 1 + hx;
-      m |= (uint32_t)(gy >= 0 && gy < p.H && gx >= 0 && gx < p.W) << i;
-      const int cy = min(max(gy, 0), p.H - 1), cx = min(max(gx, 0), p.W - 1);
-      dv[i] = *reinterpret_cast<const uint4*>(p.dy + (img + (int64_t)cy * p.W + cx) * p.lddy + c * 8);
-    }
-    return m;
-  };
-  auto stage = [&](int buf, uint32_t m) {
-#pragma unroll
-    for (int i = 0; i < NIT; ++i) {
-      const int it = tid + i * 256;
-      const uint4 v = (m >> i) & 1u ? dv[i] : make_uint4(0, 0, 0, 0);
-      if (it < HWD * HWD * 4) *reinterpret_cast<uint4*>(DT[buf] + (it >> 2) * DG_S + (it & 3) * 8) = v;
-    }
-  };
-  int t = blockIdx.x, buf = 0;
-  if (t < p.ntiles) {
-    const uint32_t m = load_dy(t);
-    stage(0, m);
-  }
-  __syncthreads();
-  for (; t < p.ntiles; t += gridDim.x) {
-    const int b = t / tiles_img, tile = t - b * tiles_img;
-    const int tyi = tile / p.tiles_x, txi = tile - tyi * p.tiles_x;
-    const int ty0 = tyi * TW, tx0 = txi * TW;
-    const int64_t img = (int64_t)b * p.H * p.W;
-    uint32_t yv[4][CL / 2];
-#pragma unroll
-    for (int i = 0; i < 4; ++i) {
-      const int gy = min(ty0 + wv + 4 * i, p.H - 1), gx = min(tx0 + r, p.W - 1);
-      const bf16_t* yp = p.yact + (img + (int64_t)gy * p.W + gx) * p.ldy + CL * q;
-      if constexpr (NT == 2) {
-        const uint4 v = *reinterpret_cast<const uint4*>(yp);
-        yv[i][0] = v.x; yv[i][1] = v.y; yv[i][CL / 2 - 2] = v.z; yv[i][CL / 2 - 1] = v.w;
-      } else {
-        const uint2 v = *reinterpret_cast<const uint2*>(yp);
-        yv[i][0] = v.x; yv[i][1] = v.y;
-      }
-    }
-    const int tn = t + (int)gridDim.x;
-    const uint32_t mnext = load_dy(tn < p.ntiles ? tn : t);
-    f32x4_t acc[4][NT];
-#pragma unroll
-    for (int i = 0; i < 4; ++i)
-#pragma unroll
-      for (int nt = 0; nt < NT; ++nt) acc[i][nt] = f32x4_t{0.f, 0.f, 0.f, 0.f};
-#pragma unroll
-    for (int tp = 0; tp < 9; ++tp) {
-      const int ty = tp / 3, tx = tp - ty * 3;
-      bf16x8_t at[NT];
-#pragma unroll
-      for (int nt = 0; nt < NT; ++nt) {
-        if constexpr (WREG) at[nt] = a[tp][nt];
-        else at[nt] = *reinterpret_cast<const bf16x8_t*>(WL + ((tp * NT + nt) * 64 + lane) * 8);
-      }
-#pragma unroll
-      for (int i = 0; i < 4; ++i) {
-        const bf16x8_t bx = *reinterpret_cast<const bf16x8_t*>(DT[buf] + ((wv + 4 * i + ty) * HWD + (r + tx)) * DG_S + q * 8);
-#pragma unroll
-        for (int nt = 0; nt < NT; ++nt) acc[i][nt] = __builtin_amdgcn_mfma_f32_16x16x32_bf16(at[nt], bx, acc[i][nt], 0, 0, 0);
-      }
-    }
-#pragma unroll
-    for (int i = 0; i < 4; ++i) {
-      const int gy = ty0 + wv + 4 * i, gx = tx0 + r;
-      const bool ok = gy < p.H && gx < p.W;
-      uint32_t o2[CL / 2];
-#pragma unroll
-      for (int nt = 0; nt < NT; ++nt) {
-        const uint32_t y01 = yv[i][2 * nt], y23 = yv[i][2 * nt + 1];
-        const float y[4] = {__uint_as_float(y01 << 16), __uint_as_float(y01 & 0xffff0000u), __uint_as_float(y23 << 16), __uint_as_float(y23 & 0xffff0000u)};
-        float o[4];
-        float4 gr = make_float4(1.f, 1.f, 1.f, 1.f), be = gr, ig = gr;
-        if (MODE == 2) {
-          gr = *reinterpret_cast<const float4*>(&CST[0][CL * q + 4 * nt]);
-          be = *reinterpret_cast<const float4*>(&CST[1][CL * q + 4 * nt]);
-          ig = *reinterpret_cast<const float4*>(&CST[2][CL * q + 4 * nt]);
-        }
-        const float grj[4] = {gr.x, gr.y, gr.z, gr.w}, bej[4] = {be.x, be.y, be.z, be.w}, igj[4] = {ig.x, ig.y, ig.z, ig.w};
-#pragma unroll
-        for (int j = 0; j < 4; ++j) {
-          const float d = ok ? acc[i][nt][j] : 0.f;
-          if (MODE == 2) {
-            const float xh = ((y[j] >= 0.f ? y[j] : y[j] * inv_neg) - bej[j]) * igj[j];
-            const float dh = d * (y[j] > 0.f ? 1.f : p.alpha);
-            sga[nt][j] = fmaf(dh, xh, sga[nt][j]);
-            sbe[nt][j] += dh;
-            o[j] = dh * grj[j];
-            sbi[nt][j] += o[j];
-          } else {
-            o[j] = d * (y[j] >= 0.f ? 1.f : p.alpha);
-          }
-        }
-        o2[2 * nt] = pack2bf(o[0], o[1]); o2[2 * nt + 1] = pack2bf(o[2], o[3]);
-        if (MODE == 0) {
-          sbi[nt][0] += __uint_as_float(o2[2 * nt] << 16); sbi[nt][1] += __uint_as_float(o2[2 * nt] & 0xffff0000u);
-          sbi[nt][2] += __uint_as_float(o2[2 * nt + 1] << 16); sbi[nt][3] += __uint_as_float(o2[2 * nt + 1] & 0xffff0000u);
-        }
-      }
-      if (ok) {
-        bf16_t* xp = p.dx + (img + (int64_t)gy * p.W + gx) * p.lddx + CL * q;
-        if constexpr (NT == 2) *reinterpret_cast<uint4*>(xp) = make_uint4(o2[0], o2[1], o2[CL / 2 - 2], o2[CL / 2 - 1]);
-        else *reinterpret_cast<uint2*>(xp) = make_uint2(o2[0], o2[1]);
-      }
-    }
-    stage(buf ^ 1, mnext);
-    __syncthreads();
-    buf ^= 1;
-  }
-#pragma unroll
-  for (int nt = 0; nt < NT; ++nt)
-#pragma unroll
-    for (int j = 0; j < 4; ++j) {
-      float v0 = sga[nt][j], v1 = sbe[nt][j], v2 = sbi[nt][j];
-#pragma unroll
-      for (int msk = 1; msk < 16; msk <<= 1) {
-        v0 += __shfl_xor(v0, msk, 64); v1 += __shfl_xor(v1, msk, 64); v2 += __shfl_xor(v2, msk, 64);
-      }
-      if (r == 0) { RED[wv][q][(nt * 4 + j) * 3 + 0] = v0; RED[wv][q][(nt * 4 + j) * 3 + 1] = v1; RED[wv][q][(nt * 4 + j) * 3 + 2] = v2; }
-    }
-  __syncthreads();
-  if (tid < CO * 3) {
-    const int k = tid / CO, c = tid - k * CO;
-    const int qq = c / CL, nt = (c % CL) >> 2, j = c & 3;
-    float s = 0.f;
-#pragma unroll
-    for (int w = 0; w < 4; ++w) s += RED[w][qq][(nt * 4 + j) * 3 + k];
-    p.ws[((int64_t)blockIdx.x * 3 + k) * CO + c] = s;
-  }
-#endif
+  constexpr bool WG1 = false;
+#include "stem_dgrad_body.inc"
+}
+
+__global__ __launch_bounds__(256, 2) void dgrad_actbwd_wgrad1_kernel(const DgAct p) {
+  constexpr int CO = 16, MODE = 0;
+  constexpr bool WG1 = true;
+#include "stem_dgrad_body.inc"
 }
 
 }
@@ -328,6 +172,28 @@
   return usseg_check_launch("stem_fwd");
 }
 
+extern "C" int usseg_stem_fwd_f32(int32_t B, int32_t H, int32_t W, const float* x, const void* w1, const float* b1, const void* w2, const float* b2,
+                                  const void* w3, const float* b3, const float* gamma, const float* beta, const float* mean, const float* var,
+                                  float eps, float alpha, void* y1, void* t1, void* c2, void* pooled, usseg_stream_t stream) {
+  USSEG_CHECK_ARG(x && w1 && b1 && w2 && b2 && w3 && b3 && gamma && beta && mean && var && y1 && t1 && c2 && pooled, "stem_fwd_f32: null pointer");
+  USSEG_CHECK_ARG(B > 0 && H > 0 && W > 0 && H % 2 == 0 && W % 2 == 0, "stem_fwd_f32: bad geometry (H, W even)");
+  USSEG_CHECK_ARG(((((uintptr_t)b1) | ((uintptr_t)b2) | ((uintptr_t)b3) | ((uintptr_t)gamma) | ((uintptr_t)beta) | ((uintptr_t)mean) | ((uintptr_t)var)) & 15) == 0,
+                  "stem_fwd_f32: per-channel vectors must be 16-byte aligned");
+  StemFwd p = {};
+  p.xf = x; p.w1 = (const bf16_t*)w1; p.w2 = (const bf16_t*)w2; p.w3 = (const bf16_t*)w3;
+  p.b1 = b1; p.b2 = b2; p.b3 = b3; p.gamma = gamma; p.beta = beta; p.mean = mean; p.var = var;
+  p.y1 = (bf16_t*)y1; p.t1 = (bf16_t*)t1; p.c2 = (bf16_t*)c2; p.pooled = (bf16_t*)pooled;
+  p.B = B; p.H = H; p.W = W; p.ldx = 1; p.alpha = alpha; p.eps = eps;
+  p.tiles_x = (W + T - 1) / T;
+  p.ntiles = p.tiles_x * ((H + TH - 1) / TH);
+  if (usseg_lds_opt_in((const void*)stem_fwd_f32_kernel, LDS_B)) return usseg_check_launch("stem_fwd_f32");
+  hipStream_t s = (hipStream_t)stream;
+  const int slot = usseg_prof_start(4, s);
+  hipLaunchKernelGGL(stem_fwd_f32_kernel, dim3(p.ntiles, B), dim3(256), LDS_B, s, p);
+  usseg_prof_stop(4, slot, s);
+  return usseg_check_launch("stem_fwd_f32");
+}
+
 extern "C" int usseg_stem_fwd_infer(int32_t B, int32_t H, int32_t W, const void* x, int32_t ldx, const void* w1, const float* b1, const void* w2,
                                     const float* b2, const void* w3, const float* b3, const float* gamma, const float* beta, const float* mean,
                                     const float* var, float eps, float alpha, void* pooled, usseg_stream_t stream) {
@@ -381,3 +247,35 @@
   else usseg_launch_reduce_finish(p.ws + 2 * Co, 1, grid, 1, 3 * Co, Co, 1.f, dbias, nullptr, nullptr, s, 0);
   return usseg_check_launch("conv3_dgrad_actbwd");
 }
+
+extern "C" int usseg_conv3_dgrad_actbwd_wgrad1(int32_t B, int32_t H, int32_t W, const void* dy, int32_t lddy, const void* wd, const void* yact,
+                                               int32_t ldy, const void* x, int32_t ldx, int32_t x_is_f32, float alpha, void* dx, int32_t lddx,
+                                               float* dbias, float* dw, float* ws, usseg_stream_t stream) {
+  constexpr int Co = 16, WN = 9 * Co;
+  USSEG_CHECK_ARG(dy && wd && yact && x && dbias && dw && ws && B > 0 && H > 0 && W > 0, "conv3_dgrad_actbwd_wgrad1: null pointer / bad geometry");
+  USSEG_CHECK_ARG(lddy >= 32 && lddy % 8 == 0 && ldy >= Co && ldy % 4 == 0 && ldx >= 1 && (!dx || (lddx >= Co && lddx % 4 == 0)),
+                  "conv3_dgrad_actbwd_wgrad1: bad strides");
+  USSEG_CHECK_ARG(((uintptr_t)x & 3) == 0 && (x_is_f32 || ldx % 2 == 0), "conv3_dgrad_actbwd_wgrad1: x must be 4-byte aligned, a bf16 x of even pixel stride");
+  DgAct p = {};
+  p.dy = (const bf16_t*)dy; p.wd = (const bf16_t*)wd; p.yact = (const bf16_t*)yact; p.dx = (bf16_t*)dx;
+  p.B = B; p.H = H; p.W = W; p.lddy = lddy; p.ldy = ldy; p.lddx = lddx; p.alpha = alpha;
+  p.x = x; p.ldx = ldx; p.x_f32 = x_is_f32 ? 1 : 0;
+  p.tiles_x = (W + 15) / 16;
+  const int64_t total = (int64_t)p.tiles_x * ((H + 15) / 16) * B;
+  USSEG_CHECK_ARG(total < (1ll << 31), "conv3_dgrad_actbwd_wgrad1: too many tiles");
+  p.ntiles = (int)total;
+  constexpr int DG_GRID = 512;
+  static_assert(DG_GRID <= USSEG_REDUCE_MAX_BLOCKS, "one partial row per workgroup");
+  const int grid = p.ntiles < DG_GRID ? p.ntiles : DG_GRID;
+  hipStream_t s = (hipStream_t)stream;
+  const int64_t need[2] = {(int64_t)grid * 3 * Co, (int64_t)grid * WN};
+  float* reg[2];
+  usseg_defer_reduce_ws_n(s, ws, need, 2, reg);
+  p.ws = reg[0]; p.wws = reg[1];
+  const int slot = usseg_prof_start(4, s);
+  hipLaunchKernelGGL(dgrad_actbwd_wgrad1_kernel, dim3(grid), dim3(256), 0, s, p);
+  usseg_prof_stop(4, slot, s);
+  usseg_launch_reduce_finish(p.ws + 2 * Co, 1, grid, 1, 3 * Co, Co, 1.f, dbias, nullptr, nullptr, s, 0);
+  usseg_launch_reduce_finish(p.wws, 1, grid, 1, WN, WN, 1.f, dw, nullptr, nullptr, s, 0);
+  return usseg_check_launch("conv3_dgrad_actbwd_wgrad1");
+}
diff --git a/ultrasound_modeling_amd/csrc/stem_dgrad_body.inc b/ultrasound_modeling_amd/csrc/stem_dgrad_body.inc
--- /dev/null
+++ b/ultrasound_modeling_amd/csrc/stem_dgrad_body.inc
@@ -0,0 +1,244 @@
+#if defined(__HIP_DEVICE_COMPILE__)
+  constexpr int TW = 16, HWD = TW + 2, NT = CO / 16, NIT = (HWD * HWD * 4 + 255) / 256, CL = 4 * NT;
+  static_assert(!WG1 || (CO == 16 && MODE == 0), "the weight-gradient epilogue belongs to the 16-channel activation pass");
+  __shared__ __attribute__((aligned(16))) bf16_t DT[2][HWD * HWD * DG_S];
+  __shared__ float RED[4][4][NT * 4 * 3];
+  const int tid = threadIdx.x, lane = tid & 63, wv = tid >> 6, r = lane & 15, q = lane >> 4;
+  constexpr bool WREG = NT == 1;
+  __shared__ __attribute__((aligned(16))) bf16_t WL[WREG ? 8 : 9 * NT * 64 * 8];
+  __shared__ __attribute__((aligned(16))) float CST[3][CO];
+  auto wrow = [&](int t, int nt) { return p.wd + (int64_t)(CL * (r >> 2) + 4 * nt + (r & 3)) * 288 + (8 - t) * 32 + q * 8; };
+  bf16x8_t a[WREG ? 9 : 1][NT];
+  if constexpr (WREG) {
+#pragma unroll
+    for (int t = 0; t < 9; ++t) a[t][0] = *reinterpret_cast<const bf16x8_t*>(wrow(t, 0));
+  } else if (wv == 0) {
+#pragma unroll
+    for (int t = 0; t < 9; ++t)
+#pragma unroll
+      for (int nt = 0; nt < NT; ++nt) *reinterpret_cast<bf16x8_t*>(WL + ((t * NT + nt) * 64 + lane) * 8) = *reinterpret_cast<const bf16x8_t*>(wrow(t, nt));
+  }
+  if (MODE == 2 && tid < CO) {
+    const float g = p.gamma[tid];
+    CST[0][tid] = g * rsqrtf(p.var[tid] + p.eps);
+    CST[1][tid] = p.beta[tid];
+    CST[2][tid] = fabsf(g) > 1e-20f ? 1.f / g : 0.f;
+  }
+  const float inv_neg = p.alpha != 0.f ? 1.f / p.alpha : 1.f;
+  float sga[NT][4], sbe[NT][4], sbi[NT][4];
+#pragma unroll
+  for (int nt = 0; nt < NT; ++nt)
+#pragma unroll
+    for (int j = 0; j < 4; ++j) sga[nt][j] = sbe[nt][j] = sbi[nt][j] = 0.f;
+  const int tiles_img = p.tiles_x * ((p.H + TW - 1) / TW);
+  uint4 dv[NIT];
+  auto load_dy = [&](int t) -> uint32_t {
+    const int b = t / tiles_img, tile = t - b * tiles_img;
+    const int tyi = tile / p.tiles_x, txi = tile - tyi * p.tiles_x;
+    const int64_t img = (int64_t)b * p.H * p.W;
+    uint32_t m = 0;
+#pragma unroll
+    for (int i = 0; i < NIT; ++i) {
+      const int it = tid + i * 256;
+      const int hp = min(it >> 2, HWD * HWD - 1), c = it & 3;
+      const int hy = hp / HWD, hx = hp - hy * HWD;
+      const int gy = tyi * TW - 1 + hy, gx = txi * TW - 1 + hx;
+      m |= (uint32_t)(gy >= 0 && gy < p.H && gx >= 0 && gx < p.W) << i;
+      const int cy = min(max(gy, 0), p.H - 1), cx = min(max(gx, 0), p.W - 1);
+      dv[i] = *reinterpret_cast<const uint4*>(p.dy + (img + (int64_t)cy * p.W + cx) * p.lddy + c * 8);
+    }
+    return m;
+  };
+  auto stage = [&](int buf, uint32_t m) {
+#pragma unroll
+    for (int i = 0; i < NIT; ++i) {
+      const int it = tid + i * 256;
+      const uint4 v = (m >> i) & 1u ? dv[i] : make_uint4(0, 0, 0, 0);
+      if (it < HWD * HWD * 4) *reinterpret_cast<uint4*>(DT[buf] + (it >> 2) * DG_S + (it & 3) * 8) = v;
+    }
+  };
+  constexpr int NXI = (HWD * HWD + 255) / 256;
+  __shared__ float XL[WG1 ? 2 : 1][WG1 ? HWD * HWD : 1];
+  [[maybe_unused]] uint32_t xv[NXI];
+  [[maybe_unused]] const int xes = p.x_f32 ? 4 : 2;
+  [[maybe_unused]] float wacc[WG1 ? 9 : 1][4];
+  if constexpr (WG1) {
+#pragma unroll
+    for (int tp = 0; tp < 9; ++tp)
+#pragma unroll
+      for (int j = 0; j < 4; ++j) wacc[tp][j] = 0.f;
+  }
+  [[maybe_unused]] auto load_x = [&](int t) -> uint32_t {
+    const int b = t / tiles_img, tile = t - b * tiles_img;
+    const int tyi = tile / p.tiles_x, txi = tile - tyi * p.tiles_x;
+    const int64_t img = (int64_t)b * p.H * p.W;
+    uint32_t m = 0;
+#pragma unroll
+    for (int i = 0; i < NXI; ++i) {
+      const int hp = min(tid + i * 256, HWD * HWD - 1);
+      const int hy = hp / HWD, hx = hp - hy * HWD;
+      const int gy = tyi * TW - 1 + hy, gx = txi * TW - 1 + hx;
+      m |= (uint32_t)(gy >= 0 && gy < p.H && gx >= 0 && gx < p.W) << i;
+      const int cy = min(max(gy, 0), p.H - 1), cx = min(max(gx, 0), p.W - 1);
+      const int64_t e = (img + (int64_t)cy * p.W + cx) * p.ldx;
+      xv[i] = *reinterpret_cast<const uint32_t*>(reinterpret_cast<const char*>(p.x) + e * xes);
+    }
+    return m;
+  };
+  [[maybe_unused]] auto stage_x = [&](int buf, uint32_t m) {
+#pragma unroll
+    for (int i = 0; i < NXI; ++i) {
+      const int hp = tid + i * 256;
+      const float f = p.x_f32 ? bf2f(f2bf(__uint_as_float(xv[i]))) : __uint_as_float(xv[i] << 16);
+      if (hp < HWD * HWD) XL[buf][hp] = (m >> i) & 1u ? f : 0.f;
+    }
+  };
+  int t = blockIdx.x, buf = 0;
+  if (t < p.ntiles) {
+    const uint32_t m = load_dy(t);
+    [[maybe_unused]] uint32_t mx = 0;
+    if constexpr (WG1) mx = load_x(t);
+    stage(0, m);
+    if constexpr (WG1) stage_x(0, mx);
+  }
+  __syncthreads();
+  for (; t < p.ntiles; t += gridDim.x) {
+    const int b = t / tiles_img, tile = t - b * tiles_img;
+    const int tyi = tile / p.tiles_x, txi = tile - tyi * p.tiles_x;
+    const int ty0 = tyi * TW, tx0 = txi * TW;
+    const int64_t img = (int64_t)b * p.H * p.W;
+    uint32_t yv[4][CL / 2];
+#pragma unroll
+    for (int i = 0; i < 4; ++i) {
+      const int gy = min(ty0 + wv + 4 * i, p.H - 1), gx = min(tx0 + r, p.W - 1);
+      const bf16_t* yp = p.yact + (img + (int64_t)gy * p.W + gx) * p.ldy + CL * q;
+      if constexpr (NT == 2) {
+        const uint4 v = *reinterpret_cast<const uint4*>(yp);
+        yv[i][0] = v.x; yv[i][1] = v.y; yv[i][CL / 2 - 2] = v.z; yv[i][CL / 2 - 1] = v.w;
+      } else {
+        const uint2 v = *reinterpret_cast<const uint2*>(yp);
+        yv[i][0] = v.x; yv[i][1] = v.y;
+      }
+    }
+    const int tn = t + (int)gridDim.x;
+    const uint32_t mnext = load_dy(tn < p.ntiles ? tn : t);
+    [[maybe_unused]] uint32_t mxnext = 0;
+    if constexpr (WG1) mxnext = load_x(tn < p.ntiles ? tn : t);
+    f32x4_t acc[4][NT];
+#pragma unroll
+    for (int i = 0; i < 4; ++i)
+#pragma unroll
+      for (int nt = 0; nt < NT; ++nt) acc[i][nt] = f32x4_t{0.f, 0.f, 0.f, 0.f};
+#pragma unroll
+    for (int tp = 0; tp < 9; ++tp) {
+      const int ty = tp / 3, tx = tp - ty * 3;
+      bf16x8_t at[NT];
+#pragma unroll
+      for (int nt = 0; nt < NT; ++nt) {
+        if constexpr (WREG) at[nt] = a[tp][nt];
+        else at[nt] = *reinterpret_cast<const bf16x8_t*>(WL + ((tp * NT + nt) * 64 + lane) * 8);
+      }
+#pragma unroll
+      for (int i = 0; i < 4; ++i) {
+        const bf16x8_t bx = *reinterpret_cast<const bf16x8_t*>(DT[buf] + ((wv + 4 * i + ty) * HWD + (r + tx)) * DG_S + q * 8);
+#pragma unroll
+        for (int nt = 0; nt < NT; ++nt) acc[i][nt] = __builtin_amdgcn_mfma_f32_16x16x32_bf16(at[nt], bx, acc[i][nt], 0, 0, 0);
+      }
+    }
+#pragma unroll
+    for (int i = 0; i < 4; ++i) {
+      const int gy = ty0 + wv + 4 * i, gx = tx0 + r;
+      const bool ok = gy < p.H && gx < p.W;
+      uint32_t o2[CL / 2];
+#pragma unroll
+      for (int nt = 0; nt < NT; ++nt) {
+        const uint32_t y01 = yv[i][2 * nt], y23 = yv[i][2 * nt + 1];
+        const float y[4] = {__uint_as_float(y01 << 16), __uint_as_float(y01 & 0xffff0000u), __uint_as_float(y23 << 16), __uint_as_float(y23 & 0xffff0000u)};
+        float o[4];
+        float4 gr = make_float4(1.f, 1.f, 1.f, 1.f), be = gr, ig = gr;
+        if (MODE == 2) {
+          gr = *reinterpret_cast<const float4*>(&CST[0][CL * q + 4 * nt]);
+          be = *reinterpret_cast<const float4*>(&CST[1][CL * q + 4 * nt]);
+          ig = *reinterpret_cast<const float4*>(&CST[2][CL * q + 4 * nt]);
+        }
+        const float grj[4] = {gr.x, gr.y, gr.z, gr.w}, bej[4] = {be.x, be.y, be.z, be.w}, igj[4] = {ig.x, ig.y, ig.z, ig.w};
+#pragma unroll
+        for (int j = 0; j < 4; ++j) {
+          const float d = ok ? acc[i][nt][j] : 0.f;
+          if (MODE == 2) {
+            const float xh = ((y[j] >= 0.f ? y[j] : y[j] * inv_neg) - bej[j]) * igj[j];
+            const float dh = d * (y[j] > 0.f ? 1.f : p.alpha);
+            sga[nt][j] = fmaf(dh, xh, sga[nt][j]);
+            sbe[nt][j] += dh;
+            o[j] = dh * grj[j];
+            sbi[nt][j] += o[j];
+          } else {
+            o[j] = d * (y[j] >= 0.f ? 1.f : p.alpha);
+          }
+        }
+        o2[2 * nt] = pack2bf(o[0], o[1]); o2[2 * nt + 1] = pack2bf(o[2], o[3]);
+        if (MODE == 0) {
+          sbi[nt][0] += __uint_as_float(o2[2 * nt] << 16); sbi[nt][1] += __uint_as_float(o2[2 * nt] & 0xffff0000u);
+          sbi[nt][2] += __uint_as_float(o2[2 * nt + 1] << 16); sbi[nt][3] += __uint_as_float(o2[2 * nt + 1] & 0xffff0000u);
+        }
+      }
+      if constexpr (WG1) {
+        const float g[4] = {__uint_as_float(o2[0] << 16), __uint_as_float(o2[0] & 0xffff0000u), __uint_as_float(o2[1] << 16), __uint_as_float(o2[1] & 0xffff0000u)};
+#pragma unroll
+        for (int tp = 0; tp < 9; ++tp) {
+          const float xs = XL[buf][(wv + 4 * i + tp / 3) * HWD + r + tp % 3];
+#pragma unroll
+          for (int j = 0; j < 4; ++j) wacc[tp][j] = fmaf(xs, g[j], wacc[tp][j]);
+        }
+      }
+      if (ok && (!WG1 || p.dx)) {
+        bf16_t* xp = p.dx + (img + (int64_t)gy * p.W + gx) * p.lddx + CL * q;
+        if constexpr (NT == 2) *reinterpret_cast<uint4*>(xp) = make_uint4(o2[0], o2[1], o2[CL / 2 - 2], o2[CL / 2 - 1]);
+        else *reinterpret_cast<uint2*>(xp) = make_uint2(o2[0], o2[1]);
+      }
+    }
+    stage(buf ^ 1, mnext);
+    if constexpr (WG1) stage_x(buf ^ 1, mxnext);
+    __syncthreads();
+    buf ^= 1;
+  }
+#pragma unroll
+  for (int nt = 0; nt < NT; ++nt)
+#pragma unroll
+    for (int j = 0; j < 4; ++j) {
+      float v0 = sga[nt][j], v1 = sbe[nt][j], v2 = sbi[nt][j];
+#pragma unroll
+      for (int msk = 1; msk < 16; msk <<= 1) {
+        v0 += __shfl_xor(v0, msk, 64); v1 += __shfl_xor(v1, msk, 64); v2 += __shfl_xor(v2, msk, 64);
+      }
+      if (r == 0) { RED[wv][q][(nt * 4 + j) * 3 + 0] = v0; RED[wv][q][(nt * 4 + j) * 3 + 1] = v1; RED[wv][q][(nt * 4 + j) * 3 + 2] = v2; }
+    }
+  if constexpr (WG1) {
+    static_assert(sizeof(DT) >= 64 * 9 * 16 * sizeof(float), "the lanes' sums must fit the dy tiles");
+    float* const RB = reinterpret_cast<float*>(&DT[0][0]);
+#pragma unroll
+    for (int tp = 0; tp < 9; ++tp)
+      *reinterpret_cast<float4*>(RB + (wv * 16 + r) * (9 * 16) + tp * 16 + 4 * q) = make_float4(wacc[tp][0], wacc[tp][1], wacc[tp][2], wacc[tp][3]);
+  }
+  __syncthreads();
+  if (tid < CO * 3) {
+    const int k = tid / CO, c = tid - k * CO;
+    const int qq = c / CL, nt = (c % CL) >> 2, j = c & 3;
+    float s = 0.f;
+#pragma unroll
+    for (int w = 0; w < 4; ++w) s += RED[w][qq][(nt * 4 + j) * 3 + k];
+    p.ws[((int64_t)blockIdx.x * 3 + k) * CO + c] = s;
+  }
+  if constexpr (WG1) {
+    if (tid < 9 * 16) {
+      const float* const RB = reinterpret_cast<const float*>(&DT[0][0]);
+      float s0 = 0.f, s1 = 0.f, s2 = 0.f, s3 = 0.f;
+#pragma unroll
+      for (int row = 0; row < 64; row += 4) {
+        s0 += RB[row * (9 * 16) + tid]; s1 += RB[(row + 1) * (9 * 16) + tid];
+        s2 += RB[(row + 2) * (9 * 16) + tid]; s3 += RB[(row + 3) * (9 * 16) + tid];
+      }
+      p.wws[(int64_t)blockIdx.x * (9 * 16) + tid] = (s0 + s1) + (s2 + s3);
+    }
+  }
+#endif
diff --git a/ultrasound_modeling_amd/csrc/stem_fwd_body.inc b/ultrasound_modeling_amd/csrc/stem_fwd_body.inc
--- a/ultrasound_modeling_amd/csrc/stem_fwd_body.inc
+++ b/ultrasound_modeling_amd/csrc/stem_fwd_body.inc
@@ -22,8 +22,13 @@
       const int hp = tid + 256 * i;
       const int hy = hp / XW, hx = hp - hy * XW;
       const int gy = ty0 - 3 + hy, gx = tx0 - 3 + hx;
-      v[i] = (hp < XW * XH && gy >= 0 && gy < p.H && gx >= 0 && gx < p.W)
-                 ? *reinterpret_cast<const uint4*>(p.x + (img + (int64_t)gy * p.W + gx) * p.ldx) : make_uint4(0, 0, 0, 0);
+      if constexpr (XF32) {
+        const float f = (hp < XW * XH && gy >= 0 && gy < p.H && gx >= 0 && gx < p.W) ? p.xf[img + (int64_t)gy * p.W + gx] : 0.f;
+        v[i] = make_uint4((uint32_t)f2bf(f), 0, 0, 0);
+      } else {
+        v[i] = (hp < XW * XH && gy >= 0 && gy < p.H && gx >= 0 && gx < p.W)
+                   ? *reinterpret_cast<const uint4*>(p.x + (img + (int64_t)gy * p.W + gx) * p.ldx) : make_uint4(0, 0, 0, 0);
+      }
     }
 #pragma unroll
     for (int i = 0; i < 2; ++i) {
diff --git a/ultrasound_modeling_amd/knobs.py b/ultrasound_modeling_amd/knobs.py
--- a/ultrasound_modeling_amd/knobs.py
+++ b/ultrasound_modeling_amd/knobs.py
@@ -16,6 +16,7 @@
     "USSEG_LN_PAIR":            ("flag",   1,     "shortcut norm backward + conv2_bn backward of the large stages in one launch"),
     "USSEG_FUSED_STEM_BWD":     ("flag",   1,     "stem backward-data fused with the norm / activation backward in front"),
     "USSEG_STEM_WGRAD_MERGE":   ("flag",   1,     "the stem's three weight gradients in one multi-job launch"),
+    "USSEG_STEM_LEAN_BWD":      ("flag",   1,     "one-channel stem: conv1's weight gradient in the backward-data epilogue, no 16-channel gradient, no input cast"),
     "USSEG_FUSED_STEM":         ("flag",   1,     "the stem (three convs, two norms, pool) as one launch"),
     "USSEG_MERGED_DGRAD":       ("flag",   1,     "one backward-data GEMM for a stage's grouped 1x1 and shortcut 1x1"),
     "USSEG_FUSED_DGRAD":        ("flag",   1,     "the DecoderBlock's four branch backward-data passes as one launch"),
diff --git a/ultrasound_modeling_amd/ops.py b/ultrasound_modeling_amd/ops.py
--- a/ultrasound_modeling_amd/ops.py
+++ b/ultrasound_modeling_amd/ops.py
@@ -772,6 +772,18 @@
     return y1, t1, c2, pooled
 
 
+def stem_fwd_f32(x, w1, b1, w2, b2, w3, b3, gamma, beta, mean, var, eps, alpha):
+    assert x.dtype == torch.float32 and x.is_contiguous() and x.dim() == 4 and x.shape[3] == 1
+    B, H, W, _ = x.shape
+    dev = x.device
+    y1, t1, c2 = new_act(B, H, W, 16, dev), new_act(B, H, W, 32, dev), new_act(B, H, W, 32, dev)
+    pooled = new_act(B, H // 2, W // 2, 32, dev)
+    L.check(L.load().usseg_stem_fwd_f32(B, H, W, x.data_ptr(), w1.data_ptr(), b1.data_ptr(), w2.data_ptr(), b2.data_ptr(), w3.data_ptr(),
+                                        b3.data_ptr(), gamma.data_ptr(), beta.data_ptr(), mean.data_ptr(), var.data_ptr(), eps, alpha,
+                                        y1.data_ptr(), t1.data_ptr(), c2.data_ptr(), pooled.data_ptr(), _stream()), "stem_fwd_f32")
+    return y1, t1, c2, pooled
+
+
 def stem_fwd_infer(x, w1, b1, w2, b2, w3, b3, gamma, beta, mean, var, eps, alpha):
     B, H, W, Cin, ldx = geom(x)
     assert Cin == 8 and x.dtype == BF16
@@ -793,6 +805,18 @@
     if rc == -2:
         return False
     L.check(rc, "conv3_dgrad_actbwd")
+    return True
+
+
+def conv3_dgrad_actbwd_wgrad1(dy, wd, yact, x, alpha, dbias, dw, dx=None) -> bool:
+    B, H, W, Cdy, lddy = geom(dy)
+    if Cdy != 32 or yact.shape[-1] != 16 or tuple(wd.shape) != (16, 9 * 32) or tuple(dw.shape) != (3, 3, 1, 16):
+        return False
+    assert x.dtype in (BF16, torch.float32) and tuple(x.shape[:3]) == (B, H, W) and dw.dtype == torch.float32 and dw.is_contiguous()
+    L.check(L.load().usseg_conv3_dgrad_actbwd_wgrad1(B, H, W, dy.data_ptr(), lddy, wd.data_ptr(), yact.data_ptr(), geom(yact)[4], x.data_ptr(),
+                                                     geom(x)[4], 1 if x.dtype == torch.float32 else 0, alpha, _ptr(dx),
+                                                     geom(dx)[4] if dx is not None else 0, dbias.data_ptr(), dw.data_ptr(),
+                                                     reduce_ws(dy.device).data_ptr(), _stream()), "conv3_dgrad_actbwd_wgrad1")
     return True
 
 
```

New measurement: 5842 (median of 5 runs). Within noise of the previous version (+0.5%).
